# tsnorri/founder-sequences

Hardware: AMD Instinct MI355X
Metric: alignment cells/s (m*n/T) through pBWT+DP (higher is better)
Workload: dtype u32

## Files before the change

### founder-sequences_amd/__init__.py

```python
import ctypes as C
import os

import numpy as np

_HERE = os.path.dirname(os.path.abspath(__file__))
LIB_PATH = os.path.join(_HERE, "libfseq_hip.so")

FSEQ_OK, FSEQ_E_ARG, FSEQ_E_NO_REDUCTION, FSEQ_E_HIP, FSEQ_E_OOM, FSEQ_E_UNSUPPORTED = range(6)


class FseqError(RuntimeError):
    def __init__(self, code, msg):
        super().__init__("fseq error %d: %s" % (code, msg))
        self.code = code


class NoReduction(FseqError):
    """generate_context.cc:192-200: max segment size equals the number of input sequences."""


class Params(C.Structure):
    _fields_ = [("m", C.c_uint32), ("n", C.c_uint64), ("segment_length", C.c_uint64),
                ("pbwt_sample_rate", C.c_uint64), ("block_len", C.c_uint32), ("list_cap", C.c_uint32),
                ("device", C.c_int32)]


class SynthSpec(C.Structure):
    _fields_ = [("seed", C.c_uint64), ("n_founders", C.c_uint32), ("block_len", C.c_uint32),
                ("mut_threshold", C.c_uint64), ("kind", C.c_uint32)]


class Segment(C.Structure):
    _fields_ = [("lb", C.c_uint64), ("rb", C.c_uint64), ("segment_size", C.c_uint32), ("reserved", C.c_uint32)]


class DpArg(C.Structure):
    _fields_ = [("lb", C.c_uint64), ("rb", C.c_uint64), ("segment_max_size", C.c_uint32), ("segment_size", C.c_uint32)]


class Result(C.Structure):
    _fields_ = [("max_segment_size", C.c_uint32), ("short_path", C.c_uint32),
                ("dp_segment_count", C.c_uint64), ("segment_count", C.c_uint64)]


class Timings(C.Structure):
    _fields_ = [("ms_total", C.c_double), ("ms_phase_a", C.c_double), ("ms_phase_b", C.c_double),
                ("ms_phase_c", C.c_double), ("ms_dp", C.c_double), ("ms_pass2", C.c_double), ("ms_host", C.c_double),
                ("ms_colstep_kernels", C.c_double), ("colstep_launches", C.c_uint64), ("colstep_cells", C.c_uint64),
                ("pass2_cells", C.c_uint64), ("list_cap_used", C.c_uint32), ("retries", C.c_uint32),
                ("block_len", C.c_uint32), ("n_blocks", C.c_uint32),
                ("dp_chunks", C.c_uint32), ("dp_sweeps", C.c_uint32), ("phase_a_fallbacks", C.c_uint32), ("phase_a_given_up", C.c_uint32), ("phase_a_trie_given_up", C.c_uint32),
                ("reduced_blocks", C.c_uint32), ("reduced_rows_mean", C.c_uint32), ("reduced_redone", C.c_uint32)]


class JoinProfile(C.Structure):
    _fields_ = [("ms_d2h", C.c_double), ("ms_classes", C.c_double), ("ms_edges", C.c_double), ("ms_draw", C.c_double), ("ms_total", C.c_double),
                ("bytes_d2h", C.c_uint64)]


class MatchPiece(C.Structure):
    _fields_ = [("lb", C.c_uint64), ("rb", C.c_uint64), ("row", C.c_uint32), ("n_founders", C.c_uint32)]


class MatchSummary(C.Structure):
    _fields_ = [("pieces", C.c_uint64), ("uncovered_cells", C.c_uint64), ("short_pieces", C.c_uint64), ("max_pieces_per_row", C.c_uint64),
                ("n_founders", C.c_uint32), ("set_words", C.c_uint32), ("ms_device", C.c_double)]


class IdentitySummary(C.Structure):
    _fields_ = [("n", C.c_uint64), ("identity", C.c_uint64), ("kept", C.c_uint64), ("ms_device", C.c_double)]


MATCH_PIECE_DTYPE = np.dtype([("lb", "<u8"), ("rb", "<u8"), ("row", "<u4"), ("n_founders", "<u4")])
MATCH_MAX_FOUNDERS = 2048

SEGMENT_DTYPE = np.dtype([("lb", "<u8"), ("rb", "<u8"), ("segment_size", "<u4"), ("reserved", "<u4")])
DPARG_DTYPE = np.dtype([("lb", "<u8"), ("rb", "<u8"), ("segment_max_size", "<u4"), ("segment_size", "<u4")])

EXPORTS = [
    "fseq_abi_version", "fseq_strerror", "fseq_create", "fseq_destroy", "fseq_last_error",
    "fseq_set_rows", "fseq_set_matrix", "fseq_set_device_columns", "fseq_generate_synthetic", "fseq_get_matrix",
    "fseq_run_segmentation", "fseq_get_traceback", "fseq_get_segments", "fseq_boundary_state",
    "fseq_short_path_runs", "fseq_join_greedy", "fseq_greedy_match_host", "fseq_write_founders", "fseq_write_founders_device", "fseq_debug_dp", "fseq_debug_block_state", "fseq_debug_column_list", "fseq_get_timings",
    "fseq_rowshard_xbuf_words", "fseq_rowshard_rows", "fseq_rowshard_pbwt",
    "fseq_debug_rmq", "fseq_shard_xbuf_words", "fseq_set_shard", "fseq_shard_columns", "fseq_shard_owner",
    "fseq_set_device_columns_packed", "fseq_debug_dp_schedule", "fseq_run_segmentation_batch", "fseq_join_bipartite", "fseq_join_random", "fseq_bipartite_match_host", "fseq_random_join_host", "fseq_write_segments",
    "fseq_set_progress", "fseq_step_max", "fseq_current_step", "fseq_set_memory_budget", "fseq_write_segments_host", "fseq_get_join_profile", "fseq_debug_set_tuning",
    "fseq_shard_abort", "fseq_debug_dp_owned", "fseq_debug_clock", "fseq_debug_ranges",
    "fseq_set_list_memory", "fseq_debug_list_windows",
    "fseq_match_founders", "fseq_match_founder_rows", "fseq_get_match", "fseq_write_match",
    "fseq_identity_columns", "fseq_create_without_identity_columns", "fseq_get_identity_columns", "fseq_write_identity_columns", "fseq_write_founders_restored", "fseq_match_founders_restored",
    "fseq_input_begin", "fseq_input_chunk_columns", "fseq_input_scan", "fseq_input_columns", "fseq_input_end", "fseq_set_rows_streamed", "fseq_debug_device_bytes", "fseq_debug_packed_columns",
    "fseq_debug_join_path", "fseq_debug_pass2_paths", "fseq_debug_class_columns", "fseq_debug_bipartite_path",
    "fseq_debug_pass2_step", "fseq_debug_chain_launch", "fseq_debug_red_plan", "fseq_debug_column_sources", "fseq_debug_red_cls_direct",
    "fseq_write_segments_device", "fseq_random_join_classes_host", "fseq_debug_segments_file", "fseq_debug_random_path",
]
DEBUG_EXPORTS = ["fseq_debug_dp", "fseq_debug_dp_owned", "fseq_debug_clock", "fseq_debug_ranges", "fseq_debug_block_state", "fseq_debug_column_list", "fseq_debug_rmq", "fseq_debug_dp_schedule", "fseq_debug_set_tuning",
                 "fseq_debug_list_windows", "fseq_debug_device_bytes", "fseq_debug_packed_columns", "fseq_debug_join_path", "fseq_debug_pass2_paths",
                 "fseq_debug_class_columns", "fseq_debug_bipartite_path", "fseq_debug_pass2_step", "fseq_debug_chain_launch", "fseq_debug_red_plan", "fseq_debug_column_sources", "fseq_debug_red_cls_direct",
                 "fseq_debug_segments_file", "fseq_debug_random_path"]

FSEQ_E_PEER = 6
P2_RUN_CAP = 8832
STAGE_TRACEBACK, STAGE_MERGE, STAGE_SAMPLES = 0, 1, 2
PROGRESS_FN = C.CFUNCTYPE(None, C.c_void_p, C.c_int, C.c_uint64, C.c_uint64)

JOIN_GREEDY, JOIN_BIPARTITE, JOIN_RANDOM = 0, 1, 2

ALLREDUCE_FN = C.CFUNCTYPE(C.c_int, C.c_void_p, C.c_uint64, C.c_uint64, C.c_int)

_lib = None


def load_library():
    global _lib
    if _lib is not None:
        return _lib
    if not os.path.exists(LIB_PATH):
        raise ImportError("%s is missing: run `python __graft_entry__.py build` (hipcc --offload-arch=gfx950); "
                          "there is no CPU fallback for the segmentation path" % LIB_PATH)
    L = C.CDLL(LIB_PATH)
    vp, u64, sz = C.c_void_p, C.c_uint64, C.c_size_t
    L.fseq_abi_version.restype = C.c_uint32
    L.fseq_strerror.restype = C.c_char_p
    L.fseq_strerror.argtypes = [C.c_int]
    L.fseq_create.argtypes = [C.POINTER(Params), C.POINTER(vp)]
    L.fseq_destroy.argtypes = [vp]
    L.fseq_destroy.restype = None
    L.fseq_last_error.restype = C.c_char_p
    L.fseq_last_error.argtypes = [vp]
    L.fseq_set_rows.argtypes = [vp, C.POINTER(vp)]
    L.fseq_set_matrix.argtypes = [vp, vp, sz, sz]
    L.fseq_set_device_columns.argtypes = [vp, vp, sz, C.c_uint32]
    L.fseq_set_device_columns_packed.argtypes = [vp, vp, sz, C.c_uint32, C.c_uint32]
    L.fseq_generate_synthetic.argtypes = [vp, C.POINTER(SynthSpec)]
    L.fseq_get_matrix.argtypes = [vp, u64, u64, vp, sz, sz]
    L.fseq_run_segmentation.argtypes = [vp, C.POINTER(Result)]
    L.fseq_get_traceback.argtypes = [vp, vp]
    L.fseq_get_segments.argtypes = [vp, vp]
    L.fseq_boundary_state.argtypes = [vp, u64, vp, vp]
    L.fseq_short_path_runs.argtypes = [vp, vp, vp]
    L.fseq_join_greedy.argtypes = [vp, vp]
    L.fseq_greedy_match_host.argtypes = [C.c_uint32, C.c_uint32, u64, vp, vp, vp, vp, vp]
    L.fseq_write_founders.argtypes = [vp, C.POINTER(vp), vp, C.c_char_p]
    L.fseq_write_founders_device.argtypes = [vp, vp, C.c_char_p]
    L.fseq_run_segmentation_batch.argtypes = [vp, sz, vp, vp]
    L.fseq_debug_dp_schedule.argtypes = [u64, u64, u64, vp, vp, vp, vp]
    L.fseq_join_bipartite.argtypes = [vp, vp]
    L.fseq_join_random.argtypes = [vp, C.c_uint32, vp]
    L.fseq_bipartite_match_host.argtypes = [C.c_uint32, C.c_uint32, u64, vp, vp, vp, vp, vp, vp]
    L.fseq_random_join_host.argtypes = [C.c_uint32, C.c_uint32, u64, vp, vp, vp, vp, C.c_uint32, vp]
    L.fseq_write_segments.argtypes = [vp, C.POINTER(vp), C.c_int, C.c_char_p]
    L.fseq_debug_dp.argtypes = [vp, vp, vp, vp]
    L.fseq_debug_block_state.argtypes = [vp, u64, vp, vp]
    L.fseq_debug_column_list.argtypes = [vp, u64, vp, vp, vp, vp, vp]
    L.fseq_get_timings.argtypes = [vp, C.POINTER(Timings)]
    L.fseq_debug_rmq.argtypes = [C.c_int, vp, C.c_uint32, vp, vp, C.c_uint32, vp, vp]
    L.fseq_shard_xbuf_words.restype = u64
    L.fseq_shard_xbuf_words.argtypes = [vp, C.c_uint32]
    L.fseq_set_shard.argtypes = [vp, C.c_uint32, C.c_uint32, vp, u64, ALLREDUCE_FN, vp]
    L.fseq_shard_columns.argtypes = [vp, C.POINTER(u64), C.POINTER(u64)]
    L.fseq_shard_owner.argtypes = [vp, u64, C.POINTER(C.c_uint32)]
    L.fseq_rowshard_xbuf_words.restype = u64
    L.fseq_rowshard_xbuf_words.argtypes = [C.c_uint32, C.c_uint32, C.c_uint32]
    L.fseq_rowshard_rows.argtypes = [C.c_uint32, C.c_uint32, C.c_uint32, C.c_uint32, C.POINTER(C.c_uint32), C.POINTER(C.c_uint32)]
    L.fseq_rowshard_pbwt.argtypes = [vp, vp, vp, C.POINTER(C.c_uint32), C.POINTER(C.c_uint32), C.POINTER(C.c_double), C.POINTER(u64)]
    L.fseq_write_segments_host.argtypes = [vp, C.POINTER(vp), C.c_int, vp, vp, C.c_char_p]
    L.fseq_get_join_profile.argtypes = [vp, C.POINTER(JoinProfile)]
    L.fseq_debug_set_tuning.argtypes = [vp, C.c_char_p, C.c_char_p]
    L.fseq_set_progress.argtypes = [vp, PROGRESS_FN, vp]
    L.fseq_step_max.restype = u64
    L.fseq_step_max.argtypes = [vp]
    L.fseq_current_step.restype = u64
    L.fseq_current_step.argtypes = [vp]
    L.fseq_set_memory_budget.argtypes = [vp, u64]
    L.fseq_set_list_memory.argtypes = [vp, u64]
    L.fseq_debug_list_windows.argtypes = [vp, C.POINTER(u64), C.POINTER(u64), C.POINTER(C.c_uint32), C.POINTER(C.c_uint32)]
    L.fseq_shard_abort.argtypes = [vp, C.c_int]
    L.fseq_debug_dp_owned.argtypes = [vp, C.POINTER(u64), C.POINTER(u64), C.POINTER(C.c_int), C.POINTER(C.c_int)]
    L.fseq_debug_clock.argtypes = [vp, C.POINTER(C.c_double), C.POINTER(C.c_uint32)]
    L.fseq_debug_ranges.argtypes = [C.POINTER(u64), C.POINTER(u64), C.POINTER(C.c_int)]
    L.fseq_match_founders.argtypes = [vp, vp, u64, C.POINTER(MatchSummary)]
    L.fseq_match_founder_rows.argtypes = [vp, C.POINTER(vp), C.c_uint32, u64, C.POINTER(MatchSummary)]
    L.fseq_get_match.argtypes = [vp, vp, vp]
    L.fseq_write_match.argtypes = [vp, C.c_char_p]
    L.fseq_identity_columns.argtypes = [vp, vp, C.POINTER(IdentitySummary)]
    L.fseq_create_without_identity_columns.argtypes = [vp, C.POINTER(Params), C.POINTER(vp), C.POINTER(IdentitySummary)]
    L.fseq_get_identity_columns.argtypes = [vp, vp, vp]
    L.fseq_write_identity_columns.argtypes = [vp, C.c_char_p]
    L.fseq_write_founders_restored.argtypes = [vp, vp, C.c_char_p]
    L.fseq_match_founders_restored.argtypes = [vp, vp, u64, C.POINTER(MatchSummary)]
    L.fseq_input_begin.argtypes = [vp, vp, C.c_uint32, u64]
    L.fseq_input_chunk_columns.restype = u64
    L.fseq_input_chunk_columns.argtypes = [vp]
    L.fseq_input_scan.argtypes = [vp, u64, u64, C.POINTER(vp)]
    L.fseq_input_columns.argtypes = [vp, u64, u64, C.POINTER(vp)]
    L.fseq_input_end.argtypes = [vp]
    L.fseq_set_rows_streamed.argtypes = [vp, C.POINTER(vp), u64]
    L.fseq_debug_device_bytes.argtypes = [vp, C.POINTER(u64), C.POINTER(u64), C.c_int]
    L.fseq_debug_packed_columns.argtypes = [vp, u64, u64, vp, C.POINTER(u64), C.POINTER(C.c_uint32)]
    L.fseq_debug_join_path.argtypes = [vp, C.POINTER(C.c_int)]
    L.fseq_debug_bipartite_path.argtypes = [vp, C.POINTER(C.c_int)]
    L.fseq_debug_pass2_paths.argtypes = [vp] + [C.POINTER(C.c_uint32)] * 4 + [vp]
    L.fseq_debug_class_columns.argtypes = [vp, C.POINTER(C.c_uint32), C.POINTER(C.c_uint32), C.c_uint32, C.POINTER(C.c_uint32), C.POINTER(C.c_uint32), C.POINTER(u64), vp, u64]
    L.fseq_debug_column_sources.argtypes = [vp, C.POINTER(C.c_uint32), C.POINTER(C.c_uint32), C.c_uint32, C.POINTER(C.c_uint32)]
    L.fseq_debug_red_cls_direct.argtypes = [C.c_uint32, C.c_uint32, C.c_uint32, u64, C.c_uint32, C.c_uint32, C.c_uint32, C.POINTER(u64), C.POINTER(u64), C.POINTER(C.c_int)]
    L.fseq_debug_pass2_step.argtypes = [C.c_int, C.c_uint32, C.c_uint32, vp, vp, vp, C.c_uint32, C.c_uint32, vp, vp, vp, vp, C.c_uint32, C.c_uint32, vp, vp, vp]
    L.fseq_debug_chain_launch.argtypes = [C.c_int, C.c_uint32, C.c_uint32, C.c_uint32, u64, vp, vp, vp, C.c_uint32, C.c_uint32, vp, vp, vp, vp, vp, vp, vp]
    L.fseq_debug_red_plan.argtypes = [C.c_uint32, C.c_uint32, C.c_uint32, C.c_int, C.c_uint32, C.c_uint32, C.c_uint32, vp, vp, C.c_int, C.c_int] + [vp] * 11
    L.fseq_write_segments_device.argtypes = [vp, C.c_int, C.c_char_p]
    L.fseq_random_join_classes_host.argtypes = [C.c_uint32, C.c_uint32, u64, vp, vp, vp, C.c_uint32, vp]
    L.fseq_debug_segments_file.argtypes = [vp] + [C.POINTER(u64)] * 4
    L.fseq_debug_random_path.argtypes = [vp, C.POINTER(C.c_int)]
    _lib = L
    return L


def synth_threshold(mu):
    if mu <= 0.0:
        return 0
    if mu >= 1.0:
        return 0xFFFFFFFFFFFFFFFF
    return int(mu * 18446744073709551616.0)


def greedy_match_host(m, max_segment_size, lb, rb, a, d):
    L = load_library()
    lb = np.ascontiguousarray(lb, dtype=np.uint64)
    rb = np.ascontiguousarray(rb, dtype=np.uint64)
    a = np.ascontiguousarray(a, dtype=np.uint32)
    d = np.ascontiguousarray(d, dtype=np.uint32)
    perm = np.zeros((len(lb), max_segment_size), dtype=np.uint32)
    rc = L.fseq_greedy_match_host(m, max_segment_size, len(lb), lb.ctypes.data, rb.ctypes.data, a.ctypes.data, d.ctypes.data, perm.ctypes.data)
    if rc != FSEQ_OK:
        raise FseqError(rc, L.fseq_strerror(rc).decode())
    return perm


def debug_ranges():
    a, b, w = C.c_uint64(), C.c_uint64(), C.c_int()
    load_library().fseq_debug_ranges(C.byref(a), C.byref(b), C.byref(w))
    return a.value, b.value, bool(w.value)


def debug_rmq(keys, beg, end, device=0):
    L = load_library()
    keys = np.ascontiguousarray(keys, dtype=np.uint32)
    beg = np.ascontiguousarray(beg, dtype=np.uint32)
    end = np.ascontiguousarray(end, dtype=np.uint32)
    a = np.zeros(len(beg), dtype=np.uint32)
    b = np.zeros(len(beg), dtype=np.uint32)
    rc = L.fseq_debug_rmq(device, keys.ctypes.data, len(keys), beg.ctypes.data, end.ctypes.data, len(beg), a.ctypes.data, b.ctypes.data)
    if rc != FSEQ_OK:
        raise FseqError(rc, L.fseq_strerror(rc).decode())
    return a, b


P2_STATS = 23
NOT_WRITTEN = 0xFFFFFFFF


def pass2_step(a0, d0, rank, task_blk, cls, headd, ncls, run_cap=P2_RUN_CAP, workgroups=1, device=0):
    L = load_library()
    a0 = np.ascontiguousarray(np.atleast_2d(a0), dtype=np.uint32)
    d0 = np.ascontiguousarray(np.atleast_2d(d0), dtype=np.uint32)
    rank = np.ascontiguousarray(np.atleast_2d(rank), dtype=np.uint32)
    task_blk = np.ascontiguousarray(task_blk, dtype=np.uint32)
    ncls = np.ascontiguousarray(ncls, dtype=np.uint32)
    cls = np.ascontiguousarray(np.atleast_2d(cls), dtype=np.uint32)
    headd = np.ascontiguousarray(np.atleast_2d(headd), dtype=np.uint32)
    nblocks, m = a0.shape
    ntasks, cap = cls.shape
    if d0.shape != a0.shape or rank.shape != a0.shape or headd.shape != cls.shape or task_blk.shape != (ntasks,) or ncls.shape != (ntasks,):
        raise FseqError(FSEQ_E_ARG, "pass2_step: shapes disagree")
    snap_a = np.zeros((ntasks, m), dtype=np.uint32)
    snap_d = np.zeros((ntasks, m), dtype=np.uint32)
    stats = np.zeros(P2_STATS, dtype=np.uint32)
    rc = L.fseq_debug_pass2_step(device, m, nblocks, a0.ctypes.data, d0.ctypes.data, rank.ctypes.data, cap, ntasks, task_blk.ctypes.data, cls.ctypes.data,
                                 headd.ctypes.data, ncls.ctypes.data, run_cap, workgroups, snap_a.ctypes.data, snap_d.ctypes.data, stats.ctypes.data)
    if rc != FSEQ_OK:
        raise FseqError(rc, L.fseq_strerror(rc).decode())
    return snap_a, snap_d, stats


def chain_launch(rank, keyd, nkeys, G, cols_per_block, first_chain=0, chains=None, start_a=None, start_d=None, states=True, keys=False, device=0):
    L = load_library()
    rank = np.ascontiguousarray(np.atleast_2d(rank), dtype=np.uint32)
    keyd = np.ascontiguousarray(np.atleast_2d(keyd), dtype=np.uint32)
    nkeys = np.ascontiguousarray(nkeys, dtype=np.uint32)
    nb_total, m = rank.shape
    if keyd.shape != rank.shape or nkeys.shape != (nb_total,):
        raise FseqError(FSEQ_E_ARG, "chain_launch: shapes disagree")
    if chains is None:
        chains = max(0, (nb_total + G - 1) // G - first_chain) if G else 0
    if (start_a is None) != (start_d is None):
        raise FseqError(FSEQ_E_ARG, "chain_launch: start_a and start_d go together")
    if start_a is not None:
        start_a = np.ascontiguousarray(np.atleast_2d(start_a), dtype=np.uint32)
        start_d = np.ascontiguousarray(np.atleast_2d(start_d), dtype=np.uint32)
        if start_a.shape != (chains, m) or start_d.shape != (chains, m):
            raise FseqError(FSEQ_E_ARG, "chain_launch: start states are [chains][m]")
    out = {}
    if states:
        out["state_a"] = np.zeros((nb_total + 1, m), dtype=np.uint32)
        out["state_d"] = np.zeros((nb_total + 1, m), dtype=np.uint32)
    if keys:
        out["rank"] = np.zeros((chains, m), dtype=np.uint32)
        out["keyd"] = np.zeros((chains, m), dtype=np.uint32)
        out["nkeys"] = np.zeros(chains, dtype=np.uint32)
    ptr = lambda name: out[name].ctypes.data if name in out else None
    rc = L.fseq_debug_chain_launch(device, m, nb_total, G, cols_per_block, rank.ctypes.data, keyd.ctypes.data, nkeys.ctypes.data, first_chain, chains,
                                   None if start_a is None else start_a.ctypes.data, None if start_a is None else start_d.ctypes.data,
                                   ptr("state_a"), ptr("state_d"), ptr("rank"), ptr("keyd"), ptr("nkeys"))
    if rc != FSEQ_OK:
        raise FseqError(rc, L.fseq_strerror(rc).decode())
    return out


RED_NONE = 0xFFFFFFFF
RED_FORCE_FULL, RED_FORCE_WIDE = 1, 2
RED_USE, RED_DECLINED, RED_NO_BLOCK_LIST = 0, 1, 2
RED_CONFIGS_MAX = 64


def red_cls_direct_host(m, B, bits, cls_ld, config, resident_rows, resident_cls):
    a, b, d = C.c_uint64(), C.c_uint64(), C.c_int()
    rc = load_library().fseq_debug_red_cls_direct(m, B, bits, cls_ld, config, resident_rows, resident_cls, C.byref(a), C.byref(b), C.byref(d))
    if rc != FSEQ_OK:
        raise FseqError(rc, "red_cls_direct_host")
    return a.value, b.value, bool(d.value)


def red_plan_host(m, B, bits, direct, cnt, force=None, b_lo=0, b_hi=None, reduced_always=False, no_block_list=False):
    L = load_library()
    cnt = np.ascontiguousarray(cnt, dtype=np.uint32)
    if cnt.ndim != 1:
        raise FseqError(FSEQ_E_ARG, "red_plan_host: cnt is one count per block")
    nb = len(cnt)
    if force is not None:
        force = np.ascontiguousarray(force, dtype=np.uint8)
        if force.shape != cnt.shape:
            raise FseqError(FSEQ_E_ARG, "red_plan_host: one force mark per block")
    configs = np.zeros((RED_CONFIGS_MAX, 6), dtype=np.uint32)
    full = np.zeros(nb, dtype=np.uint8)
    config_of = np.zeros(nb, dtype=np.int32)
    config_snap_of = np.zeros(nb, dtype=np.int32)
    blocks = np.zeros(3 * nb, dtype=np.uint32)
    bins = np.zeros((RED_CONFIGS_MAX, 3), dtype=np.uint32)
    summary = np.zeros(6, dtype=np.uint32)
    n_configs, n_blocks, n_bins, verdict = C.c_uint32(), C.c_uint32(), C.c_uint32(), C.c_int()
    rc = L.fseq_debug_red_plan(m, B, bits, int(bool(direct)), nb, b_lo, nb if b_hi is None else b_hi, cnt.ctypes.data,
                               None if force is None else force.ctypes.data, int(bool(reduced_always)), int(bool(no_block_list)),
                               configs.ctypes.data, C.addressof(n_configs), C.addressof(verdict), full.ctypes.data, config_of.ctypes.data,
                               config_snap_of.ctypes.data, blocks.ctypes.data, C.addressof(n_blocks), bins.ctypes.data, C.addressof(n_bins),
                               summary.ctypes.data)
    if rc != FSEQ_OK:
        raise FseqError(rc, L.fseq_strerror(rc).decode())
    out = dict(zip(("full_at", "nfull", "listed", "max_rows", "reduced_blocks", "rows_mean"), (int(x) for x in summary)))
    out.update(verdict=verdict.value, full=full, config_of=config_of, config_snap_of=config_snap_of, blocks=blocks[:n_blocks.value],
               bins=[tuple(int(x) for x in row) for row in bins[:n_bins.value]],
               configs=[(int(r), int(v), int(T), int(E), bool(ew), bool(fits)) for r, v, T, E, ew, fits in configs[:n_configs.value]])
    return out


class RowShard(C.Structure):
    _fields_ = [("device", C.c_int32), ("rank", C.c_uint32), ("world", C.c_uint32), ("m", C.c_uint32), ("sigma", C.c_uint32),
                ("bits", C.c_uint32), ("ncols", C.c_uint64), ("d_cols", C.c_void_p), ("ld", C.c_size_t), ("xbuf", C.c_void_p),
                ("xbuf_words", C.c_uint64), ("fn", ALLREDUCE_FN), ("user", C.c_void_p)]


def pack_columns(msa_codes, bits):
    m, n = msa_codes.shape
    per = 8 // bits
    ld = ((m + per - 1) // per + 15) // 16 * 16
    cols = np.zeros((n, ld * per), dtype=np.uint8)
    cols[:, :m] = msa_codes.T
    out = np.zeros((n, ld), dtype=np.uint8)
    for j in range(per):
        out |= (cols[:, j::per] << (bits * j)).astype(np.uint8)
    return out, ld


def rowshard_xbuf_words(m, bits, world):
    return int(load_library().fseq_rowshard_xbuf_words(m, bits, world))


def rowshard_rows(m, bits, rank, world):
    lo, hi = C.c_uint32(), C.c_uint32()
    rc = load_library().fseq_rowshard_rows(m, bits, rank, world, C.byref(lo), C.byref(hi))
    if rc != FSEQ_OK:
        raise FseqError(rc, load_library().fseq_strerror(rc).decode())
    return lo.value, hi.value


def rowshard_pbwt(d_cols_ptr, ld, m, sigma, bits, ncols, rank, world, xbuf_ptr, xbuf_words, allreduce=None, device=0):
    L = load_library()

    def _cb(_user, off, cnt, op):
        try:
            return int(allreduce(int(off), int(cnt), int(op)) or 0)
        except Exception:
            import traceback
            traceback.print_exc()
            return 1
    cb = ALLREDUCE_FN(_cb) if allreduce is not None else ALLREDUCE_FN()
    args = RowShard(device, rank, world, m, sigma, bits, ncols, d_cols_ptr, ld, xbuf_ptr, xbuf_words, cb, None)
    a = np.zeros(m, dtype=np.uint32)
    d = np.zeros(m, dtype=np.uint32)
    lo, hi, ms, nex = C.c_uint32(), C.c_uint32(), C.c_double(), C.c_uint64()
    rc = L.fseq_rowshard_pbwt(C.byref(args), a.ctypes.data, d.ctypes.data, C.byref(lo), C.byref(hi), C.byref(ms), C.byref(nex))
    if rc != FSEQ_OK:
        raise FseqError(rc, L.fseq_strerror(rc).decode())
    return a, d, lo.value, hi.value, ms.value, nex.value


def dp_schedule(segment_length, n, col_hi):
    L = load_library()
    a, b, c_, d = C.c_uint32(), C.c_uint32(), C.c_uint32(), C.c_int()
    rc = L.fseq_debug_dp_schedule(segment_length, n, col_hi, C.byref(a), C.byref(b), C.byref(c_), C.byref(d))
    if rc != FSEQ_OK:
        raise FseqError(rc, L.fseq_strerror(rc).decode())
    return a.value, b.value, c_.value, bool(d.value)


def run_batch(contexts):
    L = load_library()
    n = len(contexts)
    handles = (C.c_void_p * n)(*[c.h for c in contexts])
    results = (Result * n)()
    rcs = (C.c_int * n)()
    rc = L.fseq_run_segmentation_batch(handles, n, results, rcs)
    if rc != FSEQ_OK:
        raise FseqError(rc, L.fseq_strerror(rc).decode())
    for i, c in enumerate(contexts):
        r = Result()
        C.memmove(C.byref(r), C.byref(results[i]), C.sizeof(Result))
        c.result = r
    return list(rcs)


def bipartite_match_host(m, max_segment_size, lb, rb, a, d):
    L = load_library()
    lb = np.ascontiguousarray(lb, dtype=np.uint64)
    rb = np.ascontiguousarray(rb, dtype=np.uint64)
    a = np.ascontiguousarray(a, dtype=np.uint32)
    d = np.ascontiguousarray(d, dtype=np.uint32)
    perm = np.zeros((len(lb), max_segment_size), dtype=np.uint32)
    weights = np.zeros(max(1, len(lb) - 1), dtype=np.int64)
    rc = L.fseq_bipartite_match_host(m, max_segment_size, len(lb), lb.ctypes.data, rb.ctypes.data, a.ctypes.data, d.ctypes.data,
                                     perm.ctypes.data, weights.ctypes.data)
    if rc != FSEQ_OK:
        raise FseqError(rc, L.fseq_strerror(rc).decode())
    return perm, weights[:len(lb) - 1]


def random_join_host(m, max_segment_size, lb, rb, a, d, seed):
    L = load_library()
    lb = np.ascontiguousarray(lb, dtype=np.uint64)
    rb = np.ascontiguousarray(rb, dtype=np.uint64)
    a = np.ascontiguousarray(a, dtype=np.uint32)
    d = np.ascontiguousarray(d, dtype=np.uint32)
    perm = np.zeros((len(lb), max_segment_size), dtype=np.uint32)
    rc = L.fseq_random_join_host(m, max_segment_size, len(lb), lb.ctypes.data, rb.ctypes.data, a.ctypes.data, d.ctypes.data, seed, perm.ctypes.data)
    if rc != FSEQ_OK:
        raise FseqError(rc, L.fseq_strerror(rc).decode())
    return perm
# ... 231 lines not shown
        self._check(self.L.fseq_debug_segments_file(self.h, *[C.byref(x) for x in v]))
        return dict(zip(("batches", "bytes", "longest_line", "lines"), (x.value for x in v)))

    def random_path(self):
        path = C.c_int()
        self._check(self.L.fseq_debug_random_path(self.h, C.byref(path)))
        return path.value

    def write_founders_device(self, permutations, path):
        perm = np.ascontiguousarray(permutations, dtype=np.uint32)
        self._check(self.L.fseq_write_founders_device(self.h, perm.ctypes.data, path.encode() if path else None))

    def write_founders(self, msa, permutations, path):
        assert msa.dtype == np.uint8 and msa.flags["C_CONTIGUOUS"] and msa.shape == (self.m, self.n)
        rows = (C.c_void_p * self.m)(*[msa.ctypes.data + r * msa.strides[0] for r in range(self.m)])
        perm = np.ascontiguousarray(permutations, dtype=np.uint32)
        self._check(self.L.fseq_write_founders(self.h, rows, perm.ctypes.data, path.encode() if path else None))

    def match_founders(self, permutations=None, founders=None, min_segment_length=0):
        if (permutations is None) == (founders is None):
            raise ValueError("match_founders: give either permutations or founders")
        sm = MatchSummary()
        if permutations is not None:
            perm = np.ascontiguousarray(permutations, dtype=np.uint32)
            self._check(self.L.fseq_match_founders(self.h, perm.ctypes.data, int(min_segment_length), C.byref(sm)))
        else:
            if not isinstance(founders, np.ndarray):
                founders = np.array([np.frombuffer(bytes(f), dtype=np.uint8) for f in founders], dtype=np.uint8).reshape(len(founders), -1)
            founders = np.ascontiguousarray(founders, dtype=np.uint8)
            if founders.ndim != 2 or founders.shape[1] != self.n:
                raise ValueError("match_founders: founders must be K rows of n = %d bytes" % self.n)
            K = founders.shape[0]
            rows = (C.c_void_p * max(K, 1))(*[founders.ctypes.data + r * founders.strides[0] for r in range(K)])
            self._check(self.L.fseq_match_founder_rows(self.h, rows, K, int(min_segment_length), C.byref(sm)))
        self._match = sm
        return {k: getattr(sm, k) for k, _ in MatchSummary._fields_}

    def match_pieces(self):
        sm = getattr(self, "_match", None)
        n_pieces, words = (sm.pieces, sm.set_words) if sm is not None else (0, 1)
        pieces = np.zeros(n_pieces, dtype=MATCH_PIECE_DTYPE)
        sets = np.zeros((n_pieces, words), dtype=np.uint32)
        self._check(self.L.fseq_get_match(self.h, pieces.ctypes.data, sets.ctypes.data))
        return pieces, sets

    def write_match(self, path):
        self._check(self.L.fseq_write_match(self.h, path.encode() if path else None))

    def identity_columns(self):
        mask = np.zeros(self.n, dtype=np.uint8)
        sm = IdentitySummary()
        self._check(self.L.fseq_identity_columns(self.h, mask.ctypes.data, C.byref(sm)))
        return mask.astype(bool), {k: getattr(sm, k) for k, _ in IdentitySummary._fields_}

    def without_identity_columns(self, segment_length, block_len=0, list_cap=0, list_memory=0):
        p = Params(0, 0, int(segment_length), 0, int(block_len), int(list_cap), int(self._device))
        h = C.c_void_p()
        sm = IdentitySummary()
        self._check(self.L.fseq_create_without_identity_columns(self.h, C.byref(p), C.byref(h), C.byref(sm)))
        new = SegmentationContext.__new__(SegmentationContext)
        new.L, new.h = self.L, h
        new.m, new.n, new.segment_length, new._device = self.m, int(sm.kept), int(segment_length), self._device
        new.result, new._keep = None, None
        new.source_n = int(sm.n)
        new.identity_summary = {k: getattr(sm, k) for k, _ in IdentitySummary._fields_}
        if list_memory:
            new.set_list_memory(list_memory)
        return new

    def identity_mask(self):
        mask = np.zeros(getattr(self, "source_n", 0), dtype=np.uint8)
        self._check(self.L.fseq_get_identity_columns(self.h, mask.ctypes.data, None))
        return mask.astype(bool)

    def kept_columns(self):
        kept = np.zeros(self.n, dtype=np.uint64)
        self._check(self.L.fseq_get_identity_columns(self.h, None, kept.ctypes.data))
        return kept

    def write_identity_columns(self, path):
        self._check(self.L.fseq_write_identity_columns(self.h, path.encode() if path else None))

    def write_founders_restored(self, permutations, path):
        perm = np.ascontiguousarray(permutations, dtype=np.uint32)
        self._check(self.L.fseq_write_founders_restored(self.h, perm.ctypes.data, path.encode() if path else None))

    def match_founders_restored(self, permutations, min_segment_length=0):
        perm = np.ascontiguousarray(permutations, dtype=np.uint32)
        sm = MatchSummary()
        self._check(self.L.fseq_match_founders_restored(self.h, perm.ctypes.data, int(min_segment_length), C.byref(sm)))
        self._match = sm
        return {k: getattr(sm, k) for k, _ in MatchSummary._fields_}

    def debug_dp(self):
        k = self.n - self.segment_length + 1
        lb = np.zeros(k, dtype=np.uint32)
        mx = np.zeros(k, dtype=np.uint32)
        sz = np.zeros(k, dtype=np.uint32)
        self._check(self.L.fseq_debug_dp(self.h, lb.ctypes.data, mx.ctypes.data, sz.ctypes.data))
        return lb, mx, sz

    def debug_dp_owned(self):
        a, b = C.c_uint64(), C.c_uint64()
        f, w = C.c_int(), C.c_int()
        self._check(self.L.fseq_debug_dp_owned(self.h, C.byref(a), C.byref(b), C.byref(f), C.byref(w)))
        return a.value, b.value, bool(f.value), bool(w.value)

    def debug_clock(self):
        g, n = C.c_double(), C.c_uint32()
        self._check(self.L.fseq_debug_clock(self.h, C.byref(g), C.byref(n)))
        return g.value, n.value

    def debug_block_state(self, b):
        a = np.zeros(self.m, dtype=np.uint32)
        d = np.zeros(self.m, dtype=np.uint32)
        self._check(self.L.fseq_debug_block_state(self.h, b, a.ctypes.data, d.ctypes.data))
        return a, d

    def debug_column_list(self, col):
        cap = self.m + 2
        v = np.zeros(cap, dtype=np.uint32)
        c = np.zeros(cap, dtype=np.uint32)
        ne, c0, comp = C.c_uint32(), C.c_uint32(), C.c_uint32()
        self._check(self.L.fseq_debug_column_list(self.h, col, v.ctypes.data, c.ctypes.data,
                                                  C.byref(ne), C.byref(c0), C.byref(comp)))
        return v[:ne.value].copy(), c[:ne.value].copy(), c0.value, bool(comp.value)

    def set_tuning(self, name, value="1"):
        self._check(self.L.fseq_debug_set_tuning(self.h, name.encode(), None if value is None else str(value).encode()))

    def join_profile(self):
        jp = JoinProfile()
        self._check(self.L.fseq_get_join_profile(self.h, C.byref(jp)))
        return {k: getattr(jp, k) for k, _ in JoinProfile._fields_}

    def join_path(self):
        path = C.c_int()
        self._check(self.L.fseq_debug_join_path(self.h, C.byref(path)))
        return path.value

    def bipartite_path(self):
        path = C.c_int()
        self._check(self.L.fseq_debug_bipartite_path(self.h, C.byref(path)))
        return path.value

    def pass2_paths(self):
        v = [C.c_uint32() for _ in range(4)]
        hist = np.zeros(19, dtype=np.uint32)
        self._check(self.L.fseq_debug_pass2_paths(self.h, *[C.byref(x) for x in v], hist.ctypes.data))
        out = dict(zip(("by_runs", "by_sort", "copies", "max_runs"), (x.value for x in v)))
        out["runs_hist"] = [int(x) for x in hist]
        return out

    def class_column_sources(self):
        a, b = C.c_uint32(), C.c_uint32()
        self._check(self.L.fseq_debug_class_columns(self.h, C.byref(a), C.byref(b), 0xFFFFFFFF, None, None, None, None, 0))
        return {"from_classes": a.value, "from_alignment": b.value}

    def column_sources(self, block=None):
        a, b, s = C.c_uint32(), C.c_uint32(), C.c_uint32()
        self._check(self.L.fseq_debug_column_sources(self.h, C.byref(a), C.byref(b), 0xFFFFFFFF if block is None else block, C.byref(s)))
        out = {"staged": a.value, "gathered": b.value}
        if block is not None:
            out["block_staged"] = bool(s.value)
        return out

    def class_columns(self, block):
        have, nkeys, ldc = C.c_uint32(), C.c_uint32(), C.c_uint64()
        self._check(self.L.fseq_debug_class_columns(self.h, None, None, block, C.byref(have), C.byref(nkeys), C.byref(ldc), None, 0))
        if not have.value:
            return None, ldc.value, nkeys.value
        t = self.timings()
        cols = min(t["block_len"], self.n - block * t["block_len"])
        out = np.zeros((cols, ldc.value), dtype=np.uint8)
        self._check(self.L.fseq_debug_class_columns(self.h, None, None, block, C.byref(have), C.byref(nkeys), C.byref(ldc), out.ctypes.data, out.nbytes))
        return out, ldc.value, nkeys.value

    def timings(self):
        t = Timings()
        self._check(self.L.fseq_get_timings(self.h, C.byref(t)))
        return {k: getattr(t, k) for k, _ in Timings._fields_}
```

### founder-sequences_amd/csrc/fseq_api_debug.hip

```cpp
#include "fseq_path.hpp"
#include "fseq_dp.hpp"
#include "fseq_rowshard.hpp"

using namespace fseq;

extern "C" {

int fseq_debug_set_tuning(fseq_ctx *c, char const *name, char const *value)
{
	if (!c || !name) return FSEQ_E_ARG;
	if (c->sh.on && c->have_input) return fail(c, FSEQ_E_ARG, "sharded run: set tuning knobs before the input is set (identically on every rank)");
	if (!c->tune.set(name, value)) return fail(c, FSEQ_E_ARG, "unknown tuning knob");
	(void) hipSetDevice(c->p.device);
	if (c->stream) (void) hipStreamSynchronize(c->stream);
	free_work(c);
	forget_run_history(c);
	return FSEQ_OK;
}

int fseq_debug_pass2_paths(fseq_ctx *c, uint32_t *by_runs, uint32_t *by_sort, uint32_t *copies, uint32_t *max_runs, uint32_t *runs_hist)
{
	if (!c) return FSEQ_E_ARG;
	if (int const rc = need_result(c)) return rc;
	uint32_t const none[P2_STATS] = {};
	uint32_t const *s = c->p2_stats_have ? c->p2_stats : none;
	if (by_runs) *by_runs = s[0];
	if (by_sort) *by_sort = s[1];
	if (copies) *copies = s[2];
	if (max_runs) *max_runs = s[3];
	if (runs_hist) std::copy(s + 4, s + 4 + P2_HIST, runs_hist);
	return FSEQ_OK;
}

int fseq_debug_class_columns(fseq_ctx *c, uint32_t *from_classes, uint32_t *from_alignment, uint32_t block, uint32_t *have, uint32_t *nkeys, uint64_t *ldc,
                             uint8_t *out, uint64_t out_bytes)
{
	if (!c) return FSEQ_E_ARG;
	if (int const rc = need_result(c)) return rc;
	(void) hipSetDevice(c->p.device);
	uint32_t const b_lo = c->sh.on ? c->sh.b_lo : 0u, b_hi = c->sh.on ? c->sh.b_hi : c->nblocks;
	std::vector<uint32_t> flags;
	if (c->cls_read)
	{
		flags.assign(c->nblocks, 0u);
		if (b_hi > b_lo) HIP_TRY(c, hipMemcpy(flags.data() + b_lo, c->d_cls_have + b_lo, (size_t) (b_hi - b_lo) * 4, hipMemcpyDeviceToHost));
	}
	uint32_t n_cls = 0, n_msa = 0;
	if (c->red_active && !c->red_direct && c->red.plan.cnt.size() == c->nblocks)
		for (uint32_t b = b_lo; b < b_hi; ++b)
			if (c->red.plan.cnt[b] != RED_NONE) ++(c->cls_read && flags[b] ? n_cls : n_msa);
	if (from_classes) *from_classes = n_cls;
	if (from_alignment) *from_alignment = n_msa;
	if (block == UINT32_MAX) return FSEQ_OK;
	if (block < b_lo || block >= b_hi) return fail(c, FSEQ_E_ARG, "fseq_debug_class_columns: not a block of this context");
	uint32_t h = 0;
	if (c->cls_on && c->d_cls && c->d_cls_have) HIP_TRY(c, hipMemcpy(&h, c->d_cls_have + block, 4, hipMemcpyDeviceToHost));
	if (have) *have = h;
	if (nkeys) { *nkeys = 0; if (c->d_nkeys) HIP_TRY(c, hipMemcpy(nkeys, c->d_nkeys + block, 4, hipMemcpyDeviceToHost)); }
	if (ldc) *ldc = c->cls_on ? c->cls_ld : 0;
	if (out && h)
	{
		uint64_t const k0 = (uint64_t) block * c->B, k1 = std::min<uint64_t>(c->p.n, k0 + c->B);
		if (out_bytes < (k1 - k0) * c->cls_ld) return fail(c, FSEQ_E_ARG, "fseq_debug_class_columns: the buffer is smaller than the block's class columns");
		HIP_TRY(c, hipMemcpy(out, c->d_cls + (size_t) k0 * c->cls_ld, (size_t) (k1 - k0) * c->cls_ld, hipMemcpyDeviceToHost));
	}
	return FSEQ_OK;
}

int fseq_debug_column_sources(fseq_ctx *c, uint32_t *staged, uint32_t *gathered, uint32_t block, uint32_t *block_staged)
{
	if (!c) return FSEQ_E_ARG;
	if (int const rc = need_result(c)) return rc;
	(void) hipSetDevice(c->p.device);
	uint32_t const b_lo = c->sh.on ? c->sh.b_lo : 0u, b_hi = c->sh.on ? c->sh.b_hi : c->nblocks;
	uint32_t n_staged = 0, n_gathered = 0, mine = 0;
	RedPlan const &P = c->red.plan;
	if (c->red_active && !c->red_direct && P.cnt.size() == c->nblocks)
	{
		std::vector<uint32_t> have(c->nblocks, 0u);
		if (c->cls_staged && b_hi > b_lo) HIP_TRY(c, hipMemcpy(have.data() + b_lo, c->d_cls_have + b_lo, (size_t) (b_hi - b_lo) * 4, hipMemcpyDeviceToHost));
		for (uint32_t b = b_lo; b < b_hi; ++b)
		{
			if (P.cnt[b] == RED_NONE) continue;
			bool const st = c->cls_staged && P.from_cls[b] && have[b];
			++(st ? n_staged : n_gathered);
			if (b == block) mine = st ? 1u : 0u;
		}
	}
	if (staged) *staged = n_staged;
	if (gathered) *gathered = n_gathered;
	if (block_staged) *block_staged = mine;
	return FSEQ_OK;
}

int fseq_debug_dp(fseq_ctx *c, uint32_t *lb, uint32_t *max_size, uint32_t *size)
{
	if (!c) return FSEQ_E_ARG;
	if (int const rc = need_result(c)) return rc;
	(void) hipSetDevice(c->p.device);
	if (lb) HIP_TRY(c, hipMemcpy(lb, c->dp.LB, c->dp_size * 4, hipMemcpyDeviceToHost));
	if (max_size) HIP_TRY(c, hipMemcpy(max_size, c->dp.M, c->dp_size * 4, hipMemcpyDeviceToHost));
	if (size) HIP_TRY(c, hipMemcpy(size, c->dp.SZ, c->dp_size * 4, hipMemcpyDeviceToHost));
	return FSEQ_OK;
}

int fseq_debug_dp_owned(fseq_ctx *c, uint64_t *first, uint64_t *last, int *final_cell, int *whole_arrays)
{
	if (!c || !c->have_result || c->res.short_path) return FSEQ_E_ARG;
	uint64_t lo = 0, hi = c->dp_size;
	int fin = 1, whole = 1;
	if (c->sh.on)
	{
		Shard const &sh = c->sh;
		bool const have = sh.rank < sh.active && sh.rank < c->own_lo.size();
		lo = have ? c->own_lo[sh.rank] : 0; hi = have ? c->own_hi[sh.rank] : 0;
		fin = have && sh.rank + 1u == sh.active ? 1 : 0;
		whole = c->dp_window_mode ? 0 : 1;
	}
	if (first) *first = lo;
	if (last) *last = hi;
	if (final_cell) *final_cell = fin;
	if (whole_arrays) *whole_arrays = whole;
	return FSEQ_OK;
}

int fseq_debug_ranges(uint64_t *pushes, uint64_t *pops, int *with_roctx)
{
	if (pushes) *pushes = g_range_pushes.load(std::memory_order_relaxed);
	if (pops) *pops = g_range_pops.load(std::memory_order_relaxed);
#ifdef FSEQ_WITH_ROCTX
	if (with_roctx) *with_roctx = 1;
#else
	if (with_roctx) *with_roctx = 0;
#endif
	return FSEQ_OK;
}

int fseq_debug_clock(fseq_ctx *c, double *ghz, uint32_t *workgroups)
{
	if (!c || !ghz) return FSEQ_E_ARG;
#ifdef FSEQ_CLOCK_STAMPS
	(void) hipSetDevice(c->p.device);
	std::vector<unsigned long long> st((size_t) FSEQ_CLOCK_SLOTS * 4);
	HIP_TRY(c, hipMemcpyFromSymbol(st.data(), HIP_SYMBOL(g_clock_stamps), st.size() * 8));
	std::vector<double> f;
	for (uint32_t i = 0; i < FSEQ_CLOCK_SLOTS; ++i)
	{
		unsigned long long const t0 = st[4 * i], r0 = st[4 * i + 1], t1 = st[4 * i + 2], r1 = st[4 * i + 3];
		if (t1 > t0 && r1 > r0) f.push_back((double) (t1 - t0) / (double) (r1 - r0) * 0.1);
	}
	if (f.empty()) return fail(c, FSEQ_E_ARG, "no clock stamps: run a long-path segmentation first");
	std::nth_element(f.begin(), f.begin() + f.size() / 2, f.end());
	*ghz = f[f.size() / 2];
	if (workgroups) *workgroups = (uint32_t) f.size();
	return FSEQ_OK;
#else
	(void) workgroups;
	*ghz = 0.0;
	return fail(c, FSEQ_E_UNSUPPORTED, "built without -DFSEQ_CLOCK_STAMPS (the product kernels execute no stamp)");
#endif
}

int fseq_debug_block_state(fseq_ctx *c, uint64_t block_idx, uint32_t *a_out, uint32_t *d_out)
{
	if (!c || !c->have_result || c->res.short_path || block_idx > c->nblocks) return FSEQ_E_ARG;
	if (c->sh.on && (block_idx < c->sh.b_lo || block_idx > c->sh.b_hi)) return fail(c, FSEQ_E_ARG, "block state held by another rank");
	(void) hipSetDevice(c->p.device);
	size_t const m = c->p.m;
	if (a_out) HIP_TRY(c, hipMemcpy(a_out, c->d_bstate_a + block_idx * m, m * 4, hipMemcpyDeviceToHost));
	if (d_out) HIP_TRY(c, hipMemcpy(d_out, c->d_bstate_d + block_idx * m, m * 4, hipMemcpyDeviceToHost));
	return FSEQ_OK;
}

int fseq_debug_column_list(fseq_ctx *c, uint64_t col, uint32_t *values, uint32_t *counts,
                           uint32_t *n_entries, uint32_t *cnt0, uint32_t *complete)
{
	if (!c || !c->have_result || c->res.short_path || col >= c->p.n) return FSEQ_E_ARG;
	if (c->lw.on && (col < c->lw.col_lo || col >= c->lw.col_hi)) return fail(c, FSEQ_E_ARG, "the list of this column is not held: the run kept its lists in windows (fseq_set_list_memory)");
	(void) hipSetDevice(c->p.device);
	uint4 h;
	HIP_TRY(c, hipMemcpy(&h, c->d_hdr + col, sizeof(h), hipMemcpyDeviceToHost));
	std::vector<uint2> e(h.x);
	if (h.x) HIP_TRY(c, hipMemcpy(e.data(), c->d_ent + col * (size_t) c->stride, h.x * sizeof(uint2), hipMemcpyDeviceToHost));
// ... 150 lines not shown
```

### founder-sequences_amd/csrc/fseq_chainsort.hpp

```cpp
#pragma once

#include <type_traits>

#include "fseq_stream.hpp"
#include "fseq_types.hpp"

namespace fseq {

constexpr uint32_t CS_MAX_DIGIT_BITS = 9;
constexpr uint32_t CS_BINS = 1u << CS_MAX_DIGIT_BITS;
constexpr uint32_t CS_LEVELS = 16;

__host__ __device__ inline size_t chainsort_ws_words(uint32_t m)
{
	size_t const nblk = ((size_t) m + 63) / 64;
	return 8 * (size_t) m + CS_LEVELS * nblk + 64;
}

__device__ __forceinline__ uint64_t cs_match(uint32_t dg, bool in, uint32_t nbits)
{
	uint64_t mask = __ballot(in);
#pragma unroll
	for (uint32_t b = 0; b < CS_MAX_DIGIT_BITS; ++b)
		if (b < nbits)
		{
			uint64_t const bal = __ballot(in && ((dg >> b) & 1u));
			mask &= ((dg >> b) & 1u) ? bal : ~bal;
		}
	return mask;
}

__device__ __forceinline__ uint32_t cs_below(uint64_t mask)
{
	return (uint32_t) __builtin_amdgcn_mbcnt_hi((uint32_t) (mask >> 32), __builtin_amdgcn_mbcnt_lo((uint32_t) mask, 0u));
}

constexpr uint32_t P2_CLS_CAP = 11264;

constexpr uint32_t P2_RUN_CAP = 8832;
constexpr uint32_t P2_CLS_BITS = 14;
static_assert(P2_CLS_CAP <= (1u << P2_CLS_BITS), "a class of a reduced block fits a descriptor");

struct Pass2Lds {
	uint32_t scan[ST / WAVE + 1];
	uint32_t grp;
	union {
		struct {
			uint32_t hist[ST / WAVE][CS_BINS];
			uint32_t total[CS_BINS];
			uint16_t cls[P2_CLS_CAP];
		};
		struct {
			uint32_t off[P2_RUN_CAP + 1];
			uint32_t dsc[P2_RUN_CAP];
		};
	};
};

__host__ __device__ inline size_t pass2_lds_bytes() { return carve_bytes(1, sizeof(Pass2Lds)); }

__host__ __device__ inline size_t pass2_ws_r(uint32_t m) { return (((size_t) m + 1) / 2 + 3) & ~size_t(3); }
__host__ __device__ inline size_t pass2_ws_words(uint32_t m)
{
	size_t const nblk = ((size_t) m + 63) / 64;
	return pass2_ws_r(m) + 2 * (size_t) m + 2 * (size_t) m + 4 * (size_t) m + ((CS_LEVELS * nblk + 64 + 3) & ~size_t(3));
}
struct Pass2Ws {
	uint16_t *r;
	uint32_t *bufB, *bufA;
	uint4 *rec;
	uint32_t *tab;
};
__device__ __forceinline__ Pass2Ws pass2_ws(uint32_t *w, uint32_t m)
{
	Pass2Ws W;
	W.r = reinterpret_cast<uint16_t *>(w);
	W.bufB = w + pass2_ws_r(m);
	W.bufA = W.bufB + 2u * (size_t) m;
	W.rec = reinterpret_cast<uint4 *>(W.bufA + 2u * (size_t) m);
	W.tab = W.bufA + 6u * (size_t) m;
	return W;
}

__device__ __forceinline__ void pass2_digits(uint32_t D, uint32_t &npass, uint32_t &db)
{
	uint32_t bits = 1;
	while (bits < 32u && ((D - 1u) >> bits) != 0u) ++bits;
	npass = (bits + CS_MAX_DIGIT_BITS - 1u) / CS_MAX_DIGIT_BITS;
	db = (bits + npass - 1u) / npass;
}

template <typename PairT, typename Load0, typename KeyOf>
__device__ __forceinline__ void pass2_sort(uint32_t cnt, uint32_t npass, uint32_t db, Load0 load0, KeyOf key_of, PairT none, PairT *bufA, PairT *bufB, Pass2Lds &S)
{
	uint32_t const tid = threadIdx.x, lane = lane_id();
	uint32_t const wave = __builtin_amdgcn_readfirstlane(tid >> 6);
	constexpr uint32_t NW = ST / WAVE;
	uint32_t const nbins = 1u << db;
	uint32_t const per = ((cnt + NW - 1u) / NW + 63u) & ~63u;
	uint32_t const c_lo = min(cnt, wave * per), c_hi = min(cnt, c_lo + per);
	for (uint32_t p = 0; p < npass; ++p)
	{
		uint32_t const shift = p * db;
		bool const first = p == 0;
		PairT const *src = ((npass - p) & 1u) ? bufA : bufB;
		PairT *dst = ((npass - p) & 1u) ? bufB : bufA;
		auto load = [&](uint32_t i) -> PairT { return first ? load0(i) : src[i]; };
		for (uint32_t b = lane; b < nbins; b += 64u) S.hist[wave][b] = 0;
		constexpr uint32_t U = 4;
		for (uint32_t i0 = c_lo; i0 < c_hi; i0 += 64u * U)
		{
			PairT pr[U];
#pragma unroll
			for (uint32_t u = 0; u < U; ++u) { uint32_t const i = i0 + u * 64u + lane; pr[u] = i < c_hi ? load(i) : none; }
#pragma unroll
			for (uint32_t u = 0; u < U; ++u)
				if (i0 + u * 64u + lane < c_hi) atomicAdd(&S.hist[wave][(key_of(pr[u]) >> shift) & (nbins - 1u)], 1u);
		}
		__syncthreads();
		uint32_t tot = 0;
		if (tid < nbins)
			for (uint32_t v = 0; v < NW; ++v) { uint32_t const c = S.hist[v][tid]; S.hist[v][tid] = tot; tot += c; }
		uint32_t all;
		uint32_t const start = block_excl_add<ST>(tid < nbins ? tot : 0u, S.scan, &all);
		if (tid < nbins) S.total[tid] = start;
		__syncthreads();
		for (uint32_t b = lane; b < nbins; b += 64u) S.hist[wave][b] += S.total[b];
		for (uint32_t i0 = c_lo; i0 < c_hi; i0 += 64u * U)
		{
			PairT pr[U];
#pragma unroll
			for (uint32_t u = 0; u < U; ++u) { uint32_t const i = i0 + u * 64u + lane; pr[u] = i < c_hi ? load(i) : none; }
#pragma unroll
			for (uint32_t u = 0; u < U; ++u)
			{
				bool const in = i0 + u * 64u + lane < c_hi;
				uint32_t const dg = (key_of(pr[u]) >> shift) & (nbins - 1u);
				uint64_t const same = cs_match(dg, in, db);
				uint32_t const below = cs_below(same);
				uint32_t const base = S.hist[wave][dg];
				if (in) dst[base + below] = pr[u];
				if (in && below == 0u) S.hist[wave][dg] = base + (uint32_t) __popcll(same);
			}
		}
		__syncthreads();
	}
}

__device__ __forceinline__ void pass2_records(uint32_t m, uint32_t const *__restrict__ a0, uint32_t const *__restrict__ d0, uint4 *rec, uint32_t *tab)
{
	uint32_t const tid = threadIdx.x, lane = lane_id();
	uint32_t const wave = __builtin_amdgcn_readfirstlane(tid >> 6);
	constexpr uint32_t NW = ST / WAVE;
	uint32_t const nblk = (m + 63u) / 64u;
	constexpr uint32_t UB = 4;
	for (uint32_t b0 = wave; b0 < nblk; b0 += NW * UB)
	{
		uint32_t v[UB], a[UB];
#pragma unroll
		for (uint32_t u = 0; u < UB; ++u)
		{
			uint32_t const i = (b0 + u * NW) * 64u + lane;
			v[u] = i < m ? d0[i] : 0u;
			a[u] = i < m ? a0[i] : 0u;
		}
#pragma unroll
		for (uint32_t u = 0; u < UB; ++u)
		{
			uint32_t const blk = b0 + u * NW, i = blk * 64u + lane;
			if (blk >= nblk) break;
			uint32_t const pre = wave_incl_max(v[u]);
			uint32_t const rev = (uint32_t) __builtin_amdgcn_ds_bpermute((int) ((63u - lane) << 2), (int) v[u]);
			uint32_t const sufr = wave_incl_max(rev);
			uint32_t const sufn = (uint32_t) __builtin_amdgcn_ds_bpermute((int) ((62u - min(lane, 62u)) << 2), (int) sufr);
			if (i < m) rec[i] = make_uint4(a[u], v[u], pre, lane == 63u ? 0u : sufn);
			if (lane == 63u) tab[blk] = pre;
		}
	}
	__syncthreads();
	for (uint32_t j = tid; j + 1u < nblk; j += ST) rec[j * 64u + 63u].w = tab[j + 1u];
	for (uint32_t k = 1; k < CS_LEVELS && (1u << k) <= nblk; ++k)
	{
		uint32_t const *lo = tab + (size_t) (k - 1u) * nblk;
		uint32_t *hi = tab + (size_t) k * nblk;
		for (uint32_t j = tid; j + (1u << k) <= nblk; j += ST) hi[j] = max(lo[j], lo[j + (1u << (k - 1u))]);
		__syncthreads();
	}
	__syncthreads();
}

__device__ __forceinline__ uint32_t pass2_range_max(uint32_t lo, uint32_t hi, uint4 const *rec, uint32_t const *tab, uint32_t nblk, uint32_t const *__restrict__ d0)
{
	uint32_t const bl = lo >> 6, bh = hi >> 6;
	uint4 const rc = rec[hi], q = rec[lo - 1u];
	uint32_t const pz = q.z, sv = q.w;
	uint32_t dv = max(sv, rc.z);
	if (bh > bl + 1u)
	{
		uint32_t const k = 31u - (uint32_t) __builtin_clz(bh - bl - 1u);
		uint32_t const *t = tab + (size_t) k * nblk;
		dv = max(dv, max(t[bl + 1u], t[bh - (1u << k)]));
	}
	if (bl == bh)
	{
		if ((lo & 63u) == 0u || rc.z > pz) dv = rc.z;
		else if ((hi & 63u) == 63u || sv > rc.w) dv = sv;
		else
		{
			dv = rc.y;
			for (uint32_t i = lo; i < hi; ++i) dv = max(dv, d0[i]);
		}
	}
	return dv;
}

__device__ __forceinline__ bool pass2_runs(
	uint32_t m, uint32_t const *__restrict__ kd, uint32_t D, Pass2Ws const &W, Pass2Lds &S, uint32_t run_cap, uint32_t *nrun,
	uint32_t const *__restrict__ a0, uint32_t const *__restrict__ d0, uint32_t *__restrict__ a1, uint32_t *__restrict__ d1)
{
	uint32_t const tid = threadIdx.x, lane = lane_id();
	uint32_t const wave = __builtin_amdgcn_readfirstlane(tid >> 6);
	constexpr uint32_t NW = ST / WAVE;
	uint16_t const *__restrict__ r = W.r;
	uint32_t pb = 1;
	while (pb < 32u && ((m - 1u) >> pb) != 0u) ++pb;
	uint32_t const pmask = (1u << pb) - 1u;
	uint32_t const nblk = (m + 63u) / 64u;
	uint32_t const per = ((m + NW - 1u) / NW + 63u) & ~63u;
	uint32_t const c_lo = min(m, wave * per), c_hi = min(m, c_lo + per);
	constexpr uint32_t U = 4;

	uint32_t npass, db;
	pass2_digits(D, npass, db);
	uint2 *const bufA = reinterpret_cast<uint2 *>(W.bufA), *const bufB = reinterpret_cast<uint2 *>(W.bufB);
	uint32_t *const pos_order = reinterpret_cast<uint32_t *>((npass & 1u) ? bufA : bufB);
	uint32_t R = 0, wbase = 0;
	for (uint32_t sweep = 0; sweep < 2u; ++sweep)
	{
		uint32_t prev = 0xFFFFFFFFu;
		if (c_lo > 0u && c_lo < c_hi) prev = (uint32_t) S.cls[r[c_lo - 1u]];
		uint32_t k0 = wbase;
		for (uint32_t i0 = c_lo; i0 < c_hi; i0 += 64u * U)
		{
			uint32_t rv[U];
#pragma unroll
			for (uint32_t u = 0; u < U; ++u) { uint32_t const i = i0 + u * 64u + lane; rv[u] = i < c_hi ? (uint32_t) r[i] : 0u; }
// ... 101 lines not shown
	                  reinterpret_cast<PairT *>(W.bufA), reinterpret_cast<PairT *>(W.bufB), S);
	PairT const *perm = reinterpret_cast<PairT const *>(W.bufB);


	{
		constexpr uint32_t U = 4;
		for (uint32_t p0 = tid; p0 < m; p0 += ST * U)
		{
			uint2 me[U], pv[U];
#pragma unroll
			for (uint32_t u = 0; u < U; ++u)
			{
				uint32_t const p = min(p0 + u * ST, m - 1u);
				PairT const pm_ = perm[p], pp_ = perm[p ? p - 1u : 0u];
				me[u] = make_uint2(key_of(pm_), pos_of(pm_));
				pv[u] = make_uint2(key_of(pp_), pos_of(pp_));
			}
			uint4 rc[U];
			uint32_t z0[U], w0[U], kdv[U], t0[U], t1[U];
#pragma unroll
			for (uint32_t u = 0; u < U; ++u)
			{
				uint32_t const p = p0 + u * ST;
				bool const first = p == 0u || pv[u].x != me[u].x;
				uint32_t const lo = pv[u].y + 1u, hi = me[u].y;
				uint32_t const bl = lo >> 6, bh = hi >> 6;
				rc[u] = rec[hi];
				z0[u] = 0u; w0[u] = 0u; kdv[u] = 0u; t0[u] = 0u; t1[u] = 0u;
				if (lane == 0u && !first) { uint4 const q = rec[pv[u].y]; z0[u] = q.z; w0[u] = q.w; }
				if (p < m && first) kdv[u] = kd[me[u].x];
				if (p < m && !first && bh > bl + 1u)
				{
					uint32_t const k = 31u - (uint32_t) __builtin_clz(bh - bl - 1u);
					uint32_t const *t = tab + (size_t) k * nblk;
					t0[u] = t[bl + 1u];
					t1[u] = t[bh - (1u << k)];
				}
			}
#pragma unroll
			for (uint32_t u = 0; u < U; ++u)
			{
				uint32_t const p = p0 + u * ST;
				uint32_t const bz = (uint32_t) __builtin_amdgcn_ds_bpermute((int) ((lane - 1u) << 2), (int) rc[u].z);
				uint32_t const bw = (uint32_t) __builtin_amdgcn_ds_bpermute((int) ((lane - 1u) << 2), (int) rc[u].w);
				if (p < m)
				{
					bool const first = p == 0u || pv[u].x != me[u].x;
					uint32_t const lo = pv[u].y + 1u, hi = me[u].y;
					uint32_t const bl = lo >> 6, bh = hi >> 6;
					uint32_t const pz = lane ? bz : z0[u], sv = lane ? bw : w0[u];
					uint32_t dv = max(sv, rc[u].z);
					if (bh > bl + 1u) dv = max(dv, max(t0[u], t1[u]));
					if (!first && bl == bh)
					{
						if ((lo & 63u) == 0u || rc[u].z > pz) dv = rc[u].z;
						else if ((hi & 63u) == 63u || sv > rc[u].w) dv = sv;
						else
						{
							dv = rc[u].y;
							for (uint32_t i = lo; i < hi; i += 4u)
							{
								uint32_t const x0 = d0[i], x1 = i + 1u < hi ? d0[i + 1u] : 0u;
								uint32_t const x2 = i + 2u < hi ? d0[i + 2u] : 0u, x3 = i + 3u < hi ? d0[i + 3u] : 0u;
								dv = max(dv, max(max(x0, x1), max(x2, x3)));
							}
						}
					}
					a1[p] = rc[u].x;
					d1[p] = first ? kdv[u] : dv;
				}
			}
		}
	}
	__syncthreads();
}

__global__ __launch_bounds__(ST) void k_chain_snap_grouped(
	uint32_t const *__restrict__ bstate_a, uint32_t const *__restrict__ bstate_d, uint32_t const *__restrict__ rank, uint32_t m,
	uint32_t const *__restrict__ task_blk, uint32_t const *__restrict__ cls, uint32_t const *__restrict__ headd, uint32_t const *__restrict__ ncls,
	uint32_t cap, uint2 const *__restrict__ grps, uint32_t ngrp, uint32_t *__restrict__ grp_next, uint32_t *__restrict__ snap_a,
	uint32_t *__restrict__ snap_d, uint32_t *ws, uint32_t run_cap, uint32_t *__restrict__ stats)
{
	extern __shared__ __attribute__((aligned(16))) char smem[];
	Pass2Lds &S = *reinterpret_cast<Pass2Lds *>(smem);
	uint32_t const tid = threadIdx.x;
	Pass2Ws const W = pass2_ws(ws + (size_t) blockIdx.x * pass2_ws_words(m), m);
	uint16_t *const r = W.r;
	uint32_t pbits = 1;
	while (pbits < 32u && ((m - 1u) >> pbits) != 0u) ++pbits;
	for (;;)
	{
		if (tid == 0) S.grp = atomicAdd(grp_next, 1u);
		__syncthreads();
		uint32_t const g = S.grp;
		__syncthreads();
		if (g >= ngrp) break;
		uint2 const gr = grps[g];
		size_t const sb = (size_t) task_blk[gr.x] * m;
		uint32_t const *a0 = bstate_a + sb, *d0 = bstate_d + sb;
		bool have_r = false;
		for (uint32_t task = gr.x; task < gr.x + gr.y; ++task)
		{
			uint32_t const D = ncls[task];
			if (D == 0xFFFFFFFFu) continue;
			size_t const ob = (size_t) task * m;
			if (D == 0u)
			{
				for (uint32_t i = tid; i < m; i += ST) { snap_a[ob + i] = a0[i]; snap_d[ob + i] = d0[i]; }
				if (tid == 0) atomicAdd(stats + 2, 1u);
				continue;
			}
			if (!have_r)
			{
				constexpr uint32_t U = 4;
				for (uint32_t i0 = tid; i0 < m; i0 += ST * U)
				{
					uint32_t rv[U];
#pragma unroll
					for (uint32_t u = 0; u < U; ++u) { uint32_t const i = i0 + u * ST; rv[u] = i < m ? rank[sb + a0[i]] : 0u; }
#pragma unroll
					for (uint32_t u = 0; u < U; ++u) { uint32_t const i = i0 + u * ST; if (i < m) r[i] = (uint16_t) rv[u]; }
				}
				pass2_records(m, a0, d0, W.rec, W.tab);
				have_r = true;
			}
			for (uint32_t j = tid; j < cap; j += ST) S.cls[j] = (uint16_t) cls[(size_t) task * cap + j];
			__syncthreads();
			uint32_t kb = 1;
			while (kb < 32u && ((D - 1u) >> kb) != 0u) ++kb;
			bool const p4 = kb + pbits <= 32u;
			uint32_t const *kd = headd + (size_t) task * cap;
			uint32_t nrun = 0;
			bool const by_runs = run_cap != 0u && P2_CLS_BITS + pbits <= 32u && pass2_runs(m, kd, D, W, S, run_cap, &nrun, a0, d0, snap_a + ob, snap_d + ob);
			if (!by_runs)
			{
				if (p4) pass2_step<true>(m, kd, D, W, S, d0, snap_a + ob, snap_d + ob);
				else pass2_step<false>(m, kd, D, W, S, d0, snap_a + ob, snap_d + ob);
			}
			if (tid == 0)
			{
				atomicAdd(stats + (by_runs ? 0 : 1), 1u);
				if (nrun)
				{
					atomicMax(stats + 3, nrun);
					atomicAdd(stats + 4 + min(P2_HIST - 1u, nrun > 1u ? 32u - (uint32_t) __builtin_clz(nrun - 1u) : 0u), 1u);
				}
			}
		}
	}
}

constexpr uint32_t CM_PART = 1024;
constexpr uint32_t CM_WG = 256;


struct CmWg { uint32_t x, chain; bool ok; };
__device__ __forceinline__ CmWg cm_wg(ChainMultiArgs const &A)
{
	CmWg w;
	uint32_t const nx = gridDim.x, L = blockIdx.y * nx + blockIdx.x;
	uint32_t const xcd = L & 7u, slot = L >> 3;
	w.chain = (slot / nx) * 8u + xcd;
	w.x = slot % nx;
	w.ok = w.chain < A.nchains;
	return w;
}

__host__ __device__ inline uint32_t chainmulti_parts(uint32_t m) { return (m + CM_PART - 1u) / CM_PART; }
__host__ __device__ inline uint32_t chainmulti_passes(uint32_t m)
{
	uint32_t bits = 1;
	while (bits < 32u && ((m - 1u) >> bits) != 0u) ++bits;
	return (bits + CS_MAX_DIGIT_BITS - 1u) / CS_MAX_DIGIT_BITS;
}

struct ChainMultiGeom {
	uint32_t b, npass, db, nbins;
	uint32_t pb;
	bool p4;
	bool active;
	uint32_t *w;
	uint32_t const *a0, *d0;
	uint32_t *a1, *d1;
	uint2 *pairA, *pairB;
	uint32_t *pm, *sm, *tab;
	uint32_t *hist;
};

__device__ __forceinline__ ChainMultiGeom chainmulti_geom(ChainMultiArgs const &A, uint32_t chain)
{
	ChainMultiGeom g;
	uint32_t const grp = chain + A.grp0;
	uint32_t const b0 = grp * A.G, b1 = min(A.nb_total, b0 + A.G);
	g.b = b0 + A.step;
	g.active = g.b < b1 && (A.out_rank != nullptr || g.b + 1u < b1 || g.b + 1u == A.nb_total);
	uint32_t const nk = g.active ? A.nkeys[g.b] : 1u;
	uint32_t bits = 1;
	while (bits < 32u && ((nk - 1u) >> bits) != 0u) ++bits;
	g.npass = (bits + CS_MAX_DIGIT_BITS - 1u) / CS_MAX_DIGIT_BITS;
	g.db = (bits + g.npass - 1u) / g.npass;
	g.nbins = 1u << g.db;
	uint32_t const cur = A.step & 1u, m = A.m;
	g.pb = 1;
	while (g.pb < 32u && ((m - 1u) >> g.pb) != 0u) ++g.pb;
	g.p4 = bits + g.pb <= 32u;
	g.w = A.ws + (size_t) chain * chainsort_ws_words(m);
	g.a0 = g.w + (size_t) cur * 2u * m; g.d0 = g.a0 + m;
	g.a1 = g.w + (size_t) (cur ^ 1u) * 2u * m; g.d1 = g.a1 + m;
	g.pairA = reinterpret_cast<uint2 *>(g.a1);
	g.pairB = reinterpret_cast<uint2 *>(g.w + 4u * (size_t) m);
	g.pm = g.w + 6u * (size_t) m; g.sm = g.w + 7u * (size_t) m; g.tab = g.w + 8u * (size_t) m;
	g.hist = A.hist + (size_t) chain * chainmulti_parts(m) * CS_BINS;
	return g;
}

__device__ __forceinline__ uint2 cm_pack(uint32_t key, uint32_t pos, uint32_t row) { return make_uint2(key | (row << 20), pos | ((row >> 12) << 20)); }
__device__ __forceinline__ uint32_t cm_key(uint2 p) { return p.x & 0xFFFFFu; }
__device__ __forceinline__ uint32_t cm_pos(uint2 p) { return p.y & 0xFFFFFu; }
__device__ __forceinline__ uint32_t cm_row(uint2 p) { return (p.x >> 20) | ((p.y >> 20) << 12); }

template <bool P4>
struct CmPair {
	using T = std::conditional_t<P4, uint32_t, uint2>;
	static __device__ __forceinline__ T pack(ChainMultiGeom const &g, uint32_t key, uint32_t pos, uint32_t row)
	{
		if constexpr (P4) { (void) row; return (key << g.pb) | pos; } else { (void) g; return cm_pack(key, pos, row); }
	}
	static __device__ __forceinline__ T none() { if constexpr (P4) return 0u; else return make_uint2(0u, 0u); }
	static __device__ __forceinline__ uint32_t key(ChainMultiGeom const &g, T p) { if constexpr (P4) return p >> g.pb; else { (void) g; return cm_key(p); } }
	static __device__ __forceinline__ uint32_t pos(ChainMultiGeom const &g, T p) { if constexpr (P4) return p & ((1u << g.pb) - 1u); else { (void) g; return cm_pos(p); } }
	static __device__ __forceinline__ uint32_t row(ChainMultiGeom const &g, T p) { if constexpr (P4) return g.a0[pos(g, p)]; else { (void) g; return cm_row(p); } }
	static __device__ __forceinline__ T *bufA(ChainMultiGeom const &g) { return reinterpret_cast<T *>(g.pairA); }
	static __device__ __forceinline__ T *bufB(ChainMultiGeom const &g) { return reinterpret_cast<T *>(g.pairB); }
	static __device__ __forceinline__ T *stage(ChainMultiGeom const &g) { return (g.npass & 1u) ? bufA(g) : bufB(g); }
	static __device__ __forceinline__ T load(ChainMultiGeom const &g, uint32_t const *rk, uint32_t pass, uint32_t i)
	{
		if (pass == 0u) { uint32_t const r = g.a0[i]; return pack(g, rk[r], i, r); }
		T const *src = ((g.npass - pass) & 1u) ? bufA(g) : bufB(g);
		return src[i];
	}
};


__global__ __launch_bounds__(CM_WG) void k_cm_init(ChainMultiArgs const A)
{
	CmWg const wg = cm_wg(A);
	if (!wg.ok) return;
	uint32_t const chain = wg.chain, grp = chain + A.grp0, m = A.m;
	uint32_t const b0 = grp * A.G;
	if (b0 >= A.nb_total) return;
	uint32_t const kstart = (uint32_t) ((uint64_t) b0 * A.cols_per_block);
	uint32_t *w = A.ws + (size_t) chain * chainsort_ws_words(m);
	uint32_t const i = wg.x * CM_WG + threadIdx.x;
	if (i >= m) return;
	uint32_t const av = A.start_a ? A.start_a[(size_t) grp * m + i] : i;
	uint32_t const dv = A.start_d ? A.start_d[(size_t) grp * m + i] : kstart;
	w[i] = av; w[(size_t) m + i] = dv;
	if (A.out_state_a) { A.out_state_a[(size_t) b0 * m + i] = av; A.out_state_d[(size_t) b0 * m + i] = dv; }
}

__global__ __launch_bounds__(CM_WG) void k_cm_count(ChainMultiArgs const A)
{
	__shared__ uint32_t hist[CM_WG / WAVE][CS_BINS];
	CmWg const wg = cm_wg(A);
	if (!wg.ok) return;
	ChainMultiGeom const g = chainmulti_geom(A, wg.chain);
	if (!g.active || A.pass >= g.npass) return;
	uint32_t const lane = lane_id(), wave = __builtin_amdgcn_readfirstlane(threadIdx.x >> 6);
	uint32_t const part = wg.x * (CM_WG / WAVE) + wave, m = A.m;
	uint32_t const lo = part * CM_PART;
	if (lo >= m) return;
	uint32_t const hi = min(m, lo + CM_PART);
	uint32_t const *rk = A.rank + (size_t) g.b * m;
	uint32_t const shift = A.pass * g.db;
	for (uint32_t b = lane; b < g.nbins; b += 64u) hist[wave][b] = 0;
	auto sweep = [&](auto p4_) {
		using P = CmPair<decltype(p4_)::value>;
		constexpr uint32_t U = 4;
		for (uint32_t i0 = lo; i0 < hi; i0 += 64u * U)
		{
			typename P::T pr[U];
#pragma unroll
			for (uint32_t u = 0; u < U; ++u) { uint32_t const i = i0 + u * 64u + lane; pr[u] = i < hi ? P::load(g, rk, A.pass, i) : P::none(); }
			if (A.pass == 0u)
			{
				typename P::T *const stage = P::stage(g);
#pragma unroll
				for (uint32_t u = 0; u < U; ++u) { uint32_t const i = i0 + u * 64u + lane; if (i < hi) stage[i] = pr[u]; }
			}
#pragma unroll
			for (uint32_t u = 0; u < U; ++u)
				if (i0 + u * 64u + lane < hi) atomicAdd(&hist[wave][(P::key(g, pr[u]) >> shift) & (g.nbins - 1u)], 1u);
		}
	};
	if (g.p4) sweep(std::true_type{}); else sweep(std::false_type{});
	if (A.pass == 0u)
	{
		uint32_t const nblk = (m + 63u) / 64u;
		for (uint32_t i0 = lo; i0 < hi; i0 += 64u)
		{
			uint32_t const i = i0 + lane;
			uint32_t const v = i < m ? g.d0[i] : 0u;
			uint32_t const pre = wave_incl_max(v);
			uint32_t const rev = (uint32_t) __builtin_amdgcn_ds_bpermute((int) ((63u - lane) << 2), (int) v);
			uint32_t const sufr = wave_incl_max(rev);
			uint32_t const suf = (uint32_t) __builtin_amdgcn_ds_bpermute((int) ((63u - lane) << 2), (int) sufr);
			if (i < m) { g.pm[i] = pre; g.sm[i] = suf; }
			if (lane == 63u && (i0 >> 6) < nblk) g.tab[i0 >> 6] = pre;
		}
	}
	uint32_t *out = g.hist + (size_t) part * CS_BINS;
	for (uint32_t b = lane; b < g.nbins; b += 64u) out[b] = hist[wave][b];
}

__global__ __launch_bounds__(ST) void k_cm_offsets(ChainMultiArgs const A)
{
	__shared__ uint32_t scan[ST / WAVE + 1];
	__shared__ uint32_t start_of[CS_BINS];
	ChainMultiGeom const g = chainmulti_geom(A, blockIdx.x);
	if (!g.active || A.pass >= g.npass) return;
	uint32_t const tid = threadIdx.x, m = A.m;
	uint32_t const nparts = chainmulti_parts(m);
	constexpr uint32_t PB = 16;
	uint32_t tot = 0;
	if (tid < g.nbins)
		for (uint32_t p0 = 0; p0 < nparts; p0 += PB)
		{
			uint32_t c[PB];
#pragma unroll
			for (uint32_t q = 0; q < PB; ++q) c[q] = p0 + q < nparts ? g.hist[(size_t) (p0 + q) * CS_BINS + tid] : 0u;
#pragma unroll
			for (uint32_t q = 0; q < PB; ++q) tot += c[q];
		}
	uint32_t all;
	uint32_t const start = block_excl_add<ST>(tid < g.nbins ? tot : 0u, scan, &all);
	(void) start_of;
	if (tid < g.nbins)
	{
		uint32_t run = start;
		for (uint32_t p0 = 0; p0 < nparts; p0 += PB)
		{
			uint32_t c[PB];
#pragma unroll
			for (uint32_t q = 0; q < PB; ++q) c[q] = p0 + q < nparts ? g.hist[(size_t) (p0 + q) * CS_BINS + tid] : 0u;
#pragma unroll
			for (uint32_t q = 0; q < PB; ++q)
			{
				if (p0 + q < nparts) g.hist[(size_t) (p0 + q) * CS_BINS + tid] = run;
				run += c[q];
			}
		}
	}
	if (A.pass == 0u)
	{
		uint32_t const nblk = (m + 63u) / 64u;
		for (uint32_t k = 1; k < CS_LEVELS && (1u << k) <= nblk; ++k)
		{
			__syncthreads();
			uint32_t const *lo = g.tab + (size_t) (k - 1u) * nblk;
			uint32_t *hi = g.tab + (size_t) k * nblk;
			for (uint32_t j = tid; j + (1u << k) <= nblk; j += ST) hi[j] = max(lo[j], lo[j + (1u << (k - 1u))]);
		}
	}
}

__global__ __launch_bounds__(CM_WG) void k_cm_scatter(ChainMultiArgs const A)
{
	__shared__ uint32_t offs[CM_WG / WAVE][CS_BINS];
	CmWg const wg = cm_wg(A);
	if (!wg.ok) return;
	ChainMultiGeom const g = chainmulti_geom(A, wg.chain);
	if (!g.active || A.pass >= g.npass) return;
	uint32_t const lane = lane_id(), wave = __builtin_amdgcn_readfirstlane(threadIdx.x >> 6);
	uint32_t const part = wg.x * (CM_WG / WAVE) + wave, m = A.m;
	uint32_t const lo = part * CM_PART;
	if (lo >= m) return;
	uint32_t const hi = min(m, lo + CM_PART);
	uint32_t const *rk = A.rank + (size_t) g.b * m;
	uint32_t const shift = A.pass * g.db;
	uint32_t const *in_offs = g.hist + (size_t) part * CS_BINS;
	for (uint32_t b = lane; b < g.nbins; b += 64u) offs[wave][b] = in_offs[b];
	auto sweep = [&](auto p4_) {
		using P = CmPair<decltype(p4_)::value>;
		typename P::T *dst = ((g.npass - A.pass) & 1u) ? P::bufB(g) : P::bufA(g);
		constexpr uint32_t U = 4;
		for (uint32_t i0 = lo; i0 < hi; i0 += 64u * U)
		{
			typename P::T pr[U];
#pragma unroll
			for (uint32_t u = 0; u < U; ++u)
			{
				uint32_t const i = i0 + u * 64u + lane;
				pr[u] = i < hi ? (A.pass == 0u ? P::stage(g)[i] : P::load(g, rk, A.pass, i)) : P::none();
			}
#pragma unroll
			for (uint32_t u = 0; u < U; ++u)
			{
				bool const in = i0 + u * 64u + lane < hi;
				uint32_t const dg = (P::key(g, pr[u]) >> shift) & (g.nbins - 1u);
				uint64_t const same = cs_match(dg, in, g.db);
				uint32_t const below = cs_below(same);
				uint32_t const base = offs[wave][dg];
				if (in) dst[base + below] = pr[u];
				if (in && below == 0u) offs[wave][dg] = base + (uint32_t) __popcll(same);
			}
		}
	};
	if (g.p4) sweep(std::true_type{}); else sweep(std::false_type{});
}

__global__ __launch_bounds__(CM_WG) void k_cm_output(ChainMultiArgs const A)
{
	CmWg const wg = cm_wg(A);
	if (!wg.ok) return;
	ChainMultiGeom const g = chainmulti_geom(A, wg.chain);
	if (!g.active) return;
	uint32_t const m = A.m, p = wg.x * CM_WG + threadIdx.x;
	if (p >= m) return;
	uint32_t const nblk = (m + 63u) / 64u;
	uint32_t const *kd = A.keyd + (size_t) g.b * m;
	uint32_t key_me, key_pv, pos_me, pos_pv, row;
	if (g.p4)
	{
		using P = CmPair<true>;
		P::T const me = P::bufB(g)[p], pv = P::bufB(g)[p ? p - 1u : 0u];
		key_me = P::key(g, me); key_pv = P::key(g, pv); pos_me = P::pos(g, me); pos_pv = P::pos(g, pv); row = P::row(g, me);
	}
	else
	{
		using P = CmPair<false>;
		P::T const me = P::bufB(g)[p], pv = P::bufB(g)[p ? p - 1u : 0u];
		key_me = P::key(g, me); key_pv = P::key(g, pv); pos_me = P::pos(g, me); pos_pv = P::pos(g, pv); row = P::row(g, me);
	}
	bool const first = p == 0u || key_pv != key_me;
	uint32_t dv;
	if (first) dv = kd[key_me];
	else
	{
		uint32_t const lo = pos_pv + 1u, hi = pos_me;
		uint32_t const bl = lo >> 6, bh = hi >> 6;
		if (bl == bh)
		{
			dv = g.d0[hi];
			for (uint32_t i = lo; i < hi; ++i) dv = max(dv, g.d0[i]);
		}
		else
		{
			dv = max(g.sm[lo], g.pm[hi]);
			if (bh > bl + 1u)
			{
				uint32_t const k = 31u - (uint32_t) __builtin_clz(bh - bl - 1u);
				uint32_t const *t = g.tab + (size_t) k * nblk;
				dv = max(dv, max(t[bl + 1u], t[bh - (1u << k)]));
			}
		}
	}
	g.a1[p] = row; g.d1[p] = dv;
	uint32_t const grp = wg.chain + A.grp0;
	uint32_t const b1 = min(A.nb_total, grp * A.G + A.G);
	if (A.out_state_a && (g.b + 1u < b1 || g.b + 1u == A.nb_total))
	{
		A.out_state_a[(size_t) (g.b + 1u) * m + p] = row; A.out_state_d[(size_t) (g.b + 1u) * m + p] = dv;
	}
}

__global__ __launch_bounds__(ST) void k_cm_emit(ChainMultiArgs const A, uint32_t steps_done)
{
	extern __shared__ __attribute__((aligned(16))) char smem[];
	Carver cv{smem};
	StreamLds &L = *cv.take<StreamLds>(1);
	uint32_t const chain = blockIdx.x, grp = chain + A.grp0, m = A.m;
	uint32_t const b0 = grp * A.G;
	if (b0 >= A.nb_total) return;
	uint32_t const b1 = min(A.nb_total, b0 + A.G);
	uint32_t const cur = (b1 - b0) & 1u;
	(void) steps_done;
	uint32_t const *w = A.ws + (size_t) chain * chainsort_ws_words(m);
	uint32_t const *a = w + (size_t) cur * 2u * m, *d = a + m;
	uint32_t const kstart = (uint32_t) ((uint64_t) b0 * A.cols_per_block);
	stream_emit_ranks(m, a, d, kstart, A.out_rank + (size_t) grp * m, A.out_keyd + (size_t) grp * m, A.out_nkeys + grp, L);
}

}
```

### founder-sequences_amd/csrc/fseq_ctx.hpp

```cpp
#pragma once

#include "../../include/fseq.h"
#include "../../include/fseq_debug.h"
#include "fseq_types.hpp"

#include <hip/hip_runtime.h>

#include <algorithm>
#include <array>
#include <atomic>
#include <chrono>
#include <climits>
#include <cmath>
#include <cstdio>
#include <cstring>
#include <string>
#include <thread>
#include <unordered_map>
#include <vector>

namespace fseq {

struct KernelSet {
	uint32_t T, E, sigma, cap;
	size_t lds_colblock, lds_snap;
	uint32_t scan_shift;
	void (*rank)(hipStream_t st, uint32_t grid, size_t lds, PhaseAArgs const &keys);
	void (*snap)(hipStream_t st, uint32_t grid, size_t lds, SnapArgs const &tasks);
	size_t (*columns_lds)(uint32_t B);
	void (*columns)(hipStream_t st, uint32_t grid, size_t lds, ColumnsArgs const &cols);
	uint32_t (*columns_resident)(size_t lds);
	size_t lds_chain;
	void (*chain)(hipStream_t st, uint32_t grid, size_t lds, ChainMultiArgs const &chains, uint32_t keyed);
	hipError_t (*prepare)();
	hipError_t (*prepare_columns)(size_t lds_columns);
};

template <typename K>
inline hipError_t allow_lds(K kernel, size_t bytes)
{
	if (bytes <= 64 * 1024) return hipSuccess;
	return hipFuncSetAttribute(reinterpret_cast<void const *>(kernel), hipFuncAttributeMaxDynamicSharedMemorySize, (int) bytes);
}

struct Stream2Config { uint32_t T, E, key_shift; size_t (*lds)(uint32_t colbytes); hipError_t (*prepare)(size_t lds);
	void (*launch)(hipStream_t st, uint32_t grid, size_t lds, ColumnsArgs const &cols);
	uint32_t (*resident)(size_t lds);
	void (*launch_snap)(hipStream_t st, uint32_t grid, size_t lds, SnapArgs const &tasks); };
struct ReducedSet {
	uint32_t T, E, rows, values;
	bool pk, ew;
	size_t (*lds)(uint32_t B, uint32_t symcap);
	hipError_t (*prepare)(size_t lds);
	void (*launch)(hipStream_t st, uint32_t grid, size_t lds, ColumnsArgs const &cols, RedArgs const &red);
	uint32_t (*resident)(size_t lds);
};
int reduced_config_count();
bool reduced_config(int index, ReducedSet *out);
struct ChainSnapSet {
	size_t lds;
	hipError_t (*prepare)();
	void (*launch)(hipStream_t st, uint32_t grid, size_t lds, SnapArgs const &tasks, RedArgs const &red);
};
bool select_chain_snap(uint32_t T, uint32_t E, ChainSnapSet *out);

bool select_kernels(uint32_t m, uint32_t sigma, KernelSet *out);
Stream2Config stream2_config();
void launch_blockkeys(hipStream_t st, uint32_t grid, size_t lds, PhaseAArgs const &keys);
hipError_t prepare_blockkeys(uint32_t T, size_t lds, bool debug);
uint32_t blocktrie_threads(uint32_t m, bool stream);
size_t blocktrie_lds(uint32_t T);
hipError_t launch_blocktrie(hipStream_t st, uint32_t groups, PhaseAArgs const &keys);
hipError_t launch_reduce_prep(hipStream_t, uint32_t grid, RedPrepArgs const &);
void launch_reduce_check(hipStream_t, uint32_t const *cnt, uint32_t const *planned, uint32_t count, uint32_t *flags);
void launch_reduce_msa(hipStream_t st, MsaArgs const &A, ReducedMsaArgs const &red, bool gather_only);
bool launch_reduce_cls(hipStream_t st, MsaArgs const &A, ReducedMsaArgs const &red, ClassColumnArgs const &classes);

inline double now_ms()
{
	using namespace std::chrono;
	return duration<double, std::milli>(steady_clock::now().time_since_epoch()).count();
}


}

struct Tuning {
	bool debug = false;
	bool dp_serial = false;
	int  dp_spec_win = 0, dp_spec_rounds = 0, dp_spec_max_sweeps = 0;
	bool stream_plain_scan = false;
	bool plain_scan = false;
	bool occurrence_keys = false;
	bool phase_a_classic = false;
	int  chain_fan = 0;
	bool blockkeys_wide = false;
	bool blockkeys_single = false;
	bool no_dense_columns = false;
	bool no_blocktrie = false;
	bool blocktrie_always = false;
	int  blockkeys_cap = 0;
	bool ss_unpacked = false;
	bool ss_absolute = false;
	bool poison_lists = false;
	bool join_host = false;
	bool join_wide = false;
	bool join_bip_wide = false;
	int  join_bip_slabs = 0;
	int  segfile_batch = 0;
	bool shard_dp_full = false;
	int  shard_dp_window = 0;
	int  inject_failure_rank = -1;
	std::string sync_phases;
	bool check_phase_a = false;
	bool no_reduced = false;
	int  reduced_margin = -1;
	bool reduced_always = false;
	bool reduced_msa_gather = false;
	int  reduced_cap = 0;
	bool class_gather = false;
	int  class_columns = 1;
	int  p2_run_cap = -1;

	struct Knob {
		char const *name;
		bool Tuning::*flag;
		int Tuning::*num;
		int lo, off;
		std::string Tuning::*str;
	};
	static std::vector<Knob> const &knobs()
	{
		static std::vector<Knob> const table = {
			{"FSEQ_DEBUG", &Tuning::debug, nullptr, 0, 0, nullptr},
			{"FSEQ_DP_SERIAL", &Tuning::dp_serial, nullptr, 0, 0, nullptr},
			{"FSEQ_DP_SPEC_WIN", nullptr, &Tuning::dp_spec_win, 1, 0, nullptr},
			{"FSEQ_DP_SPEC_ROUNDS", nullptr, &Tuning::dp_spec_rounds, 1, 0, nullptr},
			{"FSEQ_DP_SPEC_MAX_SWEEPS", nullptr, &Tuning::dp_spec_max_sweeps, 1, 0, nullptr},
			{"FSEQ_STREAM_PLAIN_SCAN", &Tuning::stream_plain_scan, nullptr, 0, 0, nullptr},
			{"FSEQ_PLAIN_SCAN", &Tuning::plain_scan, nullptr, 0, 0, nullptr},
			{"FSEQ_OCCURRENCE_KEYS", &Tuning::occurrence_keys, nullptr, 0, 0, nullptr},
			{"FSEQ_PHASE_A_CLASSIC", &Tuning::phase_a_classic, nullptr, 0, 0, nullptr},
			{"FSEQ_CHAIN_FAN", nullptr, &Tuning::chain_fan, 2, 0, nullptr},
			{"FSEQ_BLOCKKEYS_WIDE", &Tuning::blockkeys_wide, nullptr, 0, 0, nullptr},
			{"FSEQ_BLOCKKEYS_SINGLE", &Tuning::blockkeys_single, nullptr, 0, 0, nullptr},
			{"FSEQ_NO_DENSE_COLUMNS", &Tuning::no_dense_columns, nullptr, 0, 0, nullptr},
			{"FSEQ_NO_BLOCKTRIE", &Tuning::no_blocktrie, nullptr, 0, 0, nullptr},
			{"FSEQ_BLOCKTRIE_ALWAYS", &Tuning::blocktrie_always, nullptr, 0, 0, nullptr},
			{"FSEQ_BLOCKKEYS_CAP", nullptr, &Tuning::blockkeys_cap, 2048, 0, nullptr},
			{"FSEQ_SS_UNPACKED", &Tuning::ss_unpacked, nullptr, 0, 0, nullptr},
			{"FSEQ_SS_ABSOLUTE", &Tuning::ss_absolute, nullptr, 0, 0, nullptr},
			{"FSEQ_POISON_LISTS", &Tuning::poison_lists, nullptr, 0, 0, nullptr},
			{"FSEQ_JOIN_HOST", &Tuning::join_host, nullptr, 0, 0, nullptr},
			{"FSEQ_JOIN_WIDE", &Tuning::join_wide, nullptr, 0, 0, nullptr},
			{"FSEQ_JOIN_BIP_WIDE", &Tuning::join_bip_wide, nullptr, 0, 0, nullptr},
			{"FSEQ_JOIN_BIP_SLABS", nullptr, &Tuning::join_bip_slabs, 1, 0, nullptr},
			{"FSEQ_SEGFILE_BATCH", nullptr, &Tuning::segfile_batch, 1, 0, nullptr},
			{"FSEQ_SHARD_DP_FULL", &Tuning::shard_dp_full, nullptr, 0, 0, nullptr},
			{"FSEQ_SHARD_DP_WINDOW", nullptr, &Tuning::shard_dp_window, 64, 0, nullptr},
			{"FSEQ_INJECT_FAILURE_RANK", nullptr, &Tuning::inject_failure_rank, INT_MIN, -1, nullptr},
			{"FSEQ_SYNC_PHASES", nullptr, nullptr, 0, 0, &Tuning::sync_phases},
			{"FSEQ_CHECK_PHASE_A", &Tuning::check_phase_a, nullptr, 0, 0, nullptr},
			{"FSEQ_NO_REDUCED", &Tuning::no_reduced, nullptr, 0, 0, nullptr},
			{"FSEQ_REDUCED_MARGIN", nullptr, &Tuning::reduced_margin, 0, -1, nullptr},
			{"FSEQ_REDUCED_ALWAYS", &Tuning::reduced_always, nullptr, 0, 0, nullptr},
			{"FSEQ_REDUCED_MSA_GATHER", &Tuning::reduced_msa_gather, nullptr, 0, 0, nullptr},
			{"FSEQ_REDUCED_CAP", nullptr, &Tuning::reduced_cap, 1, 0, nullptr},
			{"FSEQ_P2_RUN_CAP", nullptr, &Tuning::p2_run_cap, 0, -1, nullptr},
			{"FSEQ_CLASS_COLUMNS", nullptr, &Tuning::class_columns, 0, 1, nullptr},
			{"FSEQ_CLASS_GATHER", &Tuning::class_gather, nullptr, 0, 0, nullptr},
		};
		return table;
	}

	void apply(Knob const &k, char const *value)
	{
		bool const on = value != nullptr;
		if (k.flag) this->*k.flag = on;
		else if (k.num) this->*k.num = on ? std::max(k.lo, atoi(value)) : k.off;
		else this->*k.str = on ? value : "";
	}

	bool set(char const *name, char const *value)
	{
		for (Knob const &k : knobs())
			if (!strcmp(k.name, name)) { apply(k, value); return true; }
		return false;
	}

	void from_environment()
	{
		for (Knob const &k : knobs())
			if (char const *v = getenv(k.name)) apply(k, v);
	}
};

struct fseq_ctx;

namespace fseq {

template <typename T>
struct DevBuf {
	T *base = nullptr;
	size_t cap = 0;
	ptrdiff_t shift = 0;
	operator T *() const { return base ? reinterpret_cast<T *>(reinterpret_cast<char *>(base) - shift) : nullptr; }
	template <typename U> U *as() const { return reinterpret_cast<U *>(static_cast<T *>(*this)); }
	void rebase(ptrdiff_t elements) { shift = elements * (ptrdiff_t) sizeof(T); }
	int alloc(fseq_ctx *c, size_t count);
	bool try_alloc(fseq_ctx *c, size_t count);
	int ensure(fseq_ctx *c, size_t count) { return cap >= count ? FSEQ_OK : alloc(c, count); }
	int alloc_range(fseq_ctx *c, size_t lo, size_t hi, size_t per)
	{
		int const rc = alloc(c, (hi > lo ? hi - lo : 0) * per);
		rebase((ptrdiff_t) (lo * per));
		return rc;
	}
	void release(fseq_ctx *c);
};

template <typename T>
struct DevTemp : DevBuf<T> {
	fseq_ctx *const c;
	explicit DevTemp(fseq_ctx *c_) : c(c_) {}
	DevTemp(DevTemp const &) = delete;
	~DevTemp() { this->release(c); }
	int alloc(size_t count) { return DevBuf<T>::alloc(c, count); }
};

template <typename... B>
inline void release_all(fseq_ctx *c, B &...bufs) { (bufs.release(c), ...); }

}

struct Shard {
	bool on = false;
	uint32_t rank = 0, world = 1;
	uint32_t *xbuf = nullptr;
	uint64_t xwords = 0;
	fseq_allreduce_fn fn = nullptr;
	void *user = nullptr;
	uint32_t bpr = 0;
	uint32_t active = 1;
	uint32_t b_lo = 0, b_hi = 0;
	uint64_t c_lo = 0, c_hi = 0, c_end = 0;
	bool posted = false;
	bool closed = false;
};

struct fseq_ctx {
	fseq_params p{};
	Tuning tune;
	template <typename T> using DevBuf = fseq::DevBuf<T>;
	std::unordered_map<void *, size_t> alloc_sizes;
	size_t alloc_total = 0;
	size_t alloc_peak = 0;
	uint64_t mem_budget = 0;
	struct ListWindows {
		uint64_t budget = 0;
		bool on = false;
		uint32_t wb = 0, H = 0, nwin = 0;
		uint32_t merge_windows = 0;
		uint64_t bytes = 0;
		uint64_t col_lo = 0, col_hi = 0;
		std::vector<hipEvent_t> ev;
	} lw;
	std::atomic<uint64_t> step_max{0}, current_step{0};
	fseq_join_profile jp{};
	int join_path = -1;
	int bip_path = -1;
	int rand_path = -1;
	struct SegFileStats { bool have = false; uint64_t batches = 0, bytes = 0, longest_line = 0, lines = 0; } segfile;
	fseq_progress_fn progress_fn = nullptr;
	void *progress_user = nullptr;
	hipStream_t stream = nullptr;
	std::string err;
	Shard sh;
	DevBuf<uint8_t> d_msa_own;
	DevBuf<uint32_t> d_bkws;
	DevBuf<uint16_t> d_bk;
	size_t bk_per_block = 0;
	uint32_t bk_cap_words = 0;
	uint32_t bk_T = 0;
	DevBuf<uint32_t> d_todo;
	int bk_given_up = -1;
	size_t bk_lds = 0;
	DevBuf<uint32_t> d_colmask;
	bool colmask_ready = false, colmask_use = false;
	DevBuf<uint32_t> d_btws;
	DevBuf<uint32_t> d_only;
	int bt_given_up = -1;
	DevBuf<uint32_t> d_chunk_r0;
	DevBuf<uint2> d_tau;
	std::vector<int64_t> snap_slot;
	std::vector<uint32_t> own_lo, own_hi;
	bool dp_window_mode = false;
	bool shard_dp_full_sticky = false;
	uint64_t dp_exchange_words = 0;

	uint8_t *d_msa = nullptr;
	size_t ld = 0;
	bool have_input = false;
	uint32_t sigma = 0;
	uint8_t code_to_byte[256]{};

	uint32_t B = 0, nblocks = 0, N2 = 0, npass = 1;
	uint32_t auto_B = 0;
	fseq::Stream2Config s2{};
	size_t s2_lds = 0;
	bool stream_staged = false;
	uint32_t bsh = 0;
	fseq::KernelSet ks{};
	bool kernels_ready = false;
	bool use_stream = false;
	size_t tb_guess = 0;
	std::vector<uint2> tau_host;
	DevBuf<uint32_t> d_ws;
	size_t lds_columns = 0;

	DevBuf<uint32_t> d_rank, d_keyd, d_nkeys;
	DevBuf<uint32_t> d_bstate_a, d_bstate_d;
	DevBuf<uint32_t> d_cshist;
	DevBuf<uint32_t> d_hrank, d_hkeyd, d_hnkeys, d_hstate_a, d_hstate_d;
	struct ChainLevel { uint32_t count = 0; uint64_t cols = 0; DevBuf<uint32_t> rank, keyd, nkeys, state_a, state_d; };
	std::vector<ChainLevel> levels;
	uint32_t chain_fan = 0;
	uint32_t shard_k = 0, shard_q = 0;
	uint32_t chain_G = 0, n_super = 0;
	uint32_t chain_G2 = 0, n_hyper = 0;
	DevBuf<uint2> d_ent;
	DevBuf<uint4> d_hdr;
	uint32_t X = 0, stride = 0;
	uint32_t X_hint = 0;
	struct Dp {
		DevBuf<uint32_t> M, LB, SZ, Tb, Tbv;
		DevBuf<unsigned long long> K;
		uint32_t tstride = 0;
		operator fseq::DpArrays() const { return fseq::DpArrays{M, LB, SZ, Tb, Tbv, K, tstride}; }
	} dp;
	DevBuf<uint32_t> d_Mprev;
	DevBuf<uint32_t> d_spec;
	DevBuf<fseq::PathWords> d_flags;
	DevBuf<uint32_t> d_recent;
	uint64_t dp_size = 0;
	DevBuf<uint64_t> d_cols;
	DevBuf<uint2> d_grp;
	DevBuf<uint64_t> d_src;
	uint32_t snap_stride = 16;
	DevBuf<uint32_t> d_ss_a, d_ss_d;
	uint32_t ss_pack = 0;
	bool ss_ids = false;
	DevBuf<uint32_t> d_bs_w;
	DevBuf<uint8_t> d_bs_h;
	DevBuf<uint32_t> d_wgblk;
	DevBuf<uint2> d_wggrp;
	DevBuf<uint32_t> d_snap_a, d_snap_d;

	DevBuf<uint32_t> d_red_cnt, d_red_vmin, d_red_rows, d_red_leaf, d_red_a, d_red_d;
	DevBuf<uint32_t> d_red_invalid, d_red_blocks;
	uint32_t red_cap = 0;
	DevBuf<uint8_t> d_red_msa;
	size_t red_ld = 0;
	DevBuf<uint8_t> d_cls;
	DevBuf<uint32_t> d_cls_have;
	size_t cls_ld = 0;
	bool cls_on = false;
	bool cls_every = false;
	bool cls_read = false;
	DevBuf<uint32_t> d_red_src;
	bool cls_staged = false;
	struct Red {
		fseq::RedPlan plan;
		std::vector<uint8_t> cls_config;
		struct Memory {
			std::vector<uint8_t> force;
			bool plan_holds = false;
			uint32_t plan_X = 0;
			bool declined = false;
			uint32_t declined_X = 0;
			bool cls_unread = false;
			void forget_plan() { plan_holds = false; }
			void forget_verdicts() { plan_holds = false; declined = false; cls_unread = false; }
			void forget_input() { forget_verdicts(); force.clear(); }
		} memory;
	} red;
	bool red_active = false;
	DevBuf<uint32_t> d_red_cls, d_red_headd, d_red_ncls, d_red_taskblk, d_red_wgtasks;
	DevBuf<uint32_t> d_red_p2grp;
	uint32_t p2_stats[fseq::P2_STATS]{};
	bool p2_stats_have = false;
	DevBuf<uint32_t> d_red_ss_a, d_red_ss_d;
	uint32_t red_ss_stride = 0, red_ss_cap = 0;
	uint32_t *h_red_pin = nullptr;
	size_t red_pin_words = 0;
	bool red_direct = false;
	DevBuf<uint32_t> d_red_cnt_plan;
	hipStream_t red_st[2]{};
	struct RedEvents {
		hipEvent_t fork = nullptr;
		hipEvent_t join_stream2 = nullptr, join_side0 = nullptr, join_side1 = nullptr;
		std::array<hipEvent_t *, 3> joins() { return {&join_stream2, &join_side0, &join_side1}; }
		std::array<hipEvent_t *, 4> all() { return {&fork, &join_stream2, &join_side0, &join_side1}; }
	} red_ev;
	uint8_t *h_red_pin2 = nullptr;
	size_t red_pin2_bytes = 0;

	bool have_result = false;
	fseq_result res{};
	DevBuf<uint4> d_tb;
	std::vector<fseq_dp_arg> traceback;
	std::vector<fseq_segment> segments;
	std::vector<uint32_t> sp_first, sp_len;
	fseq_timings tm{};
	struct PathEvents {
		hipEvent_t a_begin = nullptr, a_end_b_begin = nullptr, b_end = nullptr;
		hipEvent_t c_begin = nullptr, c_end = nullptr, dp_begin = nullptr, dp_end = nullptr;
		hipEvent_t pass2_begin = nullptr, pass2_end = nullptr;
		hipEvent_t dp_reset = nullptr;
		std::array<hipEvent_t *, 9> timed() { return {&a_begin, &a_end_b_begin, &b_end, &c_begin, &c_end, &dp_begin, &dp_end, &pass2_begin, &pass2_end}; }
	} ev;
	hipStream_t stream2 = nullptr;
	uint8_t *h_pin = nullptr;
	size_t pin_cap = 0, pin_used = 0;

	struct Match {
		DevBuf<uint8_t> fcols;
		DevBuf<uint32_t> cnt;
		DevBuf<uint64_t> off;
		DevBuf<fseq_match_piece> pieces;
		DevBuf<uint32_t> sets;
		bool have = false;
		fseq_match_summary sum{};
		hipEvent_t ev[4]{};
	} match;
	void free_match()
	{
		fseq::release_all(this, match.fcols, match.cnt, match.off, match.pieces, match.sets);
		for (auto &e : match.ev) if (e) { (void) hipEventDestroy(e); e = nullptr; }
		match.have = false;
	}

	struct Identity {
		bool have = false;
		uint64_t n_src = 0, identity = 0;
		DevBuf<uint8_t> mask;
		DevBuf<uint32_t> kept;
		DevBuf<uint8_t> ref;
	} idn;
	void free_identity()
	{
		fseq::release_all(this, idn.mask, idn.kept, idn.ref);
		idn.have = false;
	}

	struct Input {
		bool open = false;
		bool given = false;
		bool table_ready = false;
		uint64_t half_bytes = 0, chunk_cols = 0;
		uint64_t scanned = 0, encoded = 0;
		uint64_t calls = 0;
		uint32_t present[8]{};
		DevBuf<uint8_t> stage;
		DevBuf<uint32_t> words;
		DevBuf<uint8_t> table;
		hipEvent_t copied[2]{}, used[2]{};
	} in;
	void free_input()
	{
		fseq::release_all(this, in.stage, in.words, in.table);
		for (auto &e : in.copied) if (e) { (void) hipEventDestroy(e); e = nullptr; }
		for (auto &e : in.used) if (e) { (void) hipEventDestroy(e); e = nullptr; }
		in.open = false;
	}
};
// ... 96 lines not shown
```

### founder-sequences_amd/csrc/fseq_path_pass1.hip

```cpp
#include "fseq_path.hpp"
#include "fseq_kernels.hpp"
#include "fseq_stream.hpp"
#include "fseq_stream2.hpp"
#include "fseq_chainsort.hpp"
#include "fseq_blockkeys.hpp"
#include "fseq_blocktrie.hpp"

namespace fseq {

std::atomic<uint64_t> g_range_pushes{0}, g_range_pops{0};

uint32_t scan_keyed(fseq_ctx const *c)
{
	if (c->use_stream || c->tune.plain_scan) return 0u;
	return (c->p.n < (1ull << c->ks.scan_shift) && !c->tune.occurrence_keys) ? 1u : c->p.n < (1ull << 25) ? 2u : 0u;
}

namespace {

bool stream_keyed(fseq_ctx const *c) { return c->p.n < (1ull << 25) && !c->tune.plain_scan; }

template <int MODE>
void launch_colblock_stream(fseq_ctx *c, uint32_t grid, MsaArgs const &A, PhaseAArgs const &K, SnapArgs const &S)
{
	hipLaunchKernelGGL((stream_keyed(c) ? k_colblock_stream<MODE, true> : k_colblock_stream<MODE, false>), dim3(grid), dim3(ST), stream_lds_bytes(sym_bytes(A.m, A.bsh), c->stream_staged), c->stream,
	                   A.msa, A.ld, A.m, A.n, A.B, A.nblocks, A.npass, A.bsh, c->d_ws.base, (uint32_t) c->stream_staged, K.rank, K.keyd, K.nkeys, MODE == MODE_RANK ? K.only : S.bstate_a, S.bstate_d,
	                   S.task_rb, S.task_grp, S.snap_a, S.snap_d, S.task_src, S.ss.snap_stride, (uint32_t const *) S.ss.ss_a, (uint32_t const *) S.ss.ss_d, K.col0, S.ss.ss_pack);
}

void launch_rank(fseq_ctx *c, PhaseAArgs const &K)
{
	if (!K.nblk) return;
	if (c->use_stream) launch_colblock_stream<MODE_RANK>(c, K.nblk, K.A, K, SnapArgs{});
	else c->ks.rank(c->stream, K.nblk, c->ks.lds_colblock, K);
}

void launch_blockkeys_stream(fseq_ctx *c, uint32_t groups, PhaseAArgs const &K)
{
	MsaArgs const &A = K.A;
	hipLaunchKernelGGL(k_blockkeys_stream, dim3(groups), dim3(1024), c->bk_lds, c->stream, A.msa, A.ld, A.m, A.n, A.B, A.bsh, K.nblk, K.rank, K.keyd, K.nkeys, K.col0,
	                   static_cast<uint32_t *>(K.work), K.work_per, K.cap_words, K.counters, K.wide, K.todo, K.only);
}

}

void launch_replay_stream(fseq_ctx *c, size_t groups, SnapArgs const &tasks)
{
	size_t const cap = std::max<size_t>(1, c->d_ws.cap / (4 * (size_t) c->p.m));
	SnapArgs S = tasks;
	for (size_t g0 = 0; g0 < groups; g0 += cap)
	{
		S.task_grp = tasks.task_grp + g0; S.task_src = tasks.task_src + g0;
		launch_colblock_stream<MODE_SNAP>(c, (uint32_t) std::min(cap, groups - g0), S.A, PhaseAArgs{}, S);
	}
}

namespace {

void launch_chain_stream(hipStream_t st, uint32_t grid, ChainMultiArgs A)
{
	uint32_t const m = A.m, nparts = chainmulti_parts(m), npass = chainmulti_passes(m);
	A.step = 0; A.pass = 0;
	A.nchains = grid;
	uint32_t const grid_y = (grid + 7u) & ~7u;
	dim3 const by_row((m + CM_WG - 1u) / CM_WG, grid_y), by_part((nparts + CM_WG / WAVE - 1u) / (CM_WG / WAVE), grid_y);
	hipLaunchKernelGGL(k_cm_init, by_row, dim3(CM_WG), 0, st, A);
	for (uint32_t s_ = 0; s_ < A.G; ++s_)
	{
		A.step = s_;
		for (uint32_t ps = 0; ps < npass; ++ps)
		{
			A.pass = ps;
			hipLaunchKernelGGL(k_cm_count, by_part, dim3(CM_WG), 0, st, A);
			hipLaunchKernelGGL(k_cm_offsets, dim3(grid), dim3(ST), 0, st, A);
			hipLaunchKernelGGL(k_cm_scatter, by_part, dim3(CM_WG), 0, st, A);
		}
		hipLaunchKernelGGL(k_cm_output, by_row, dim3(CM_WG), 0, st, A);
	}
	if (A.out_rank) hipLaunchKernelGGL(k_cm_emit, dim3(grid), dim3(ST), stream_lds_bytes(0, false), st, A, A.G);
}

void launch_chain(fseq_ctx *c, uint32_t grid, ChainMultiArgs A)
{
	if (!grid) return;
	A.m = c->p.m;
	if (c->use_stream)
	{
		A.ws = c->d_ws.base; A.hist = c->d_cshist;
		launch_chain_stream(c->stream, grid, A);
	}
	else
		c->ks.chain(c->stream, grid, c->ks.lds_chain, A, scan_keyed(c));
}

}

int prepare_stream_kernels(fseq_ctx *c, size_t lds)
{
	HIP_TRY(c, allow_lds(k_colblock_stream<MODE_RANK>, lds));
	HIP_TRY(c, allow_lds(k_colblock_stream<MODE_SNAP>, lds));
	HIP_TRY(c, allow_lds(k_colblock_stream<MODE_RANK, true>, lds));
	HIP_TRY(c, allow_lds(k_colblock_stream<MODE_SNAP, true>, lds));
	HIP_TRY(c, allow_lds(k_columns_stream<19>, lds));
	HIP_TRY(c, allow_lds(k_columns_stream<0>, lds));
	HIP_TRY(c, allow_lds(k_chain_snap_grouped, pass2_lds_bytes()));
	HIP_TRY(c, allow_lds(k_cm_emit, stream_lds_bytes(0, false)));
	return FSEQ_OK;
}
int prepare_stream2_prologue(fseq_ctx *c)
{
	HIP_TRY(c, allow_lds(k_columns_stream2_prologue, stream_lds_bytes(0, true)));
	return FSEQ_OK;
}
int prepare_blockkeys_stream(fseq_ctx *c)
{
	HIP_TRY(c, allow_lds(k_blockkeys_stream, c->bk_lds));
	return FSEQ_OK;
}
size_t chain_hist_words(uint32_t m) { return (size_t) chainmulti_parts(m) * CS_BINS; }

uint32_t pass2_run_cap(fseq_ctx const *c)
{
	return c->tune.p2_run_cap < 0 ? P2_RUN_CAP : std::min<uint32_t>((uint32_t) c->tune.p2_run_cap, P2_RUN_CAP);
}

int launch_chain_snap_grouped(fseq_ctx *c, uint32_t ngrp, uint32_t *stats)
{
	uint32_t const m = c->p.m;
	hipStream_t st = c->stream;
	if (c->red_cap > P2_CLS_CAP) return fail(c, FSEQ_E_UNSUPPORTED, "pass 2: more representatives a block than the class table in LDS holds");
	int ncu = 0;
	(void) hipDeviceGetAttribute(&ncu, hipDeviceAttributeMultiprocessorCount, c->p.device);
	size_t const fit = c->d_ws.cap / pass2_ws_words(m);
	uint32_t const grid = (uint32_t) std::min<size_t>(std::min<size_t>(ngrp, fit), (size_t) std::max(ncu, 1) * 2u);
	if (!grid) return fail(c, FSEQ_E_OOM, "pass 2: the workspace holds no chain step");
	if (c->tune.debug)
	{
		int resident = 0;
		(void) hipOccupancyMaxActiveBlocksPerMultiprocessor(&resident, k_chain_snap_grouped, (int) ST, pass2_lds_bytes());
		fprintf(stderr, "[fseq] pass 2 chain steps: %u groups on %u workgroups (the workspace holds %zu, a CU %d), %zu bytes of LDS, at most %u runs\n", ngrp, grid, fit,
		        resident, pass2_lds_bytes(), pass2_run_cap(c));
	}
	hipLaunchKernelGGL(k_chain_snap_grouped, dim3(grid), dim3(ST), pass2_lds_bytes(), st, c->d_bstate_a, c->d_bstate_d, c->d_rank, m, c->d_red_taskblk, c->d_red_cls,
	                   c->d_red_headd, c->d_red_ncls, c->red_cap, c->d_red_p2grp.as<uint2 const>(), ngrp, c->d_red_p2grp + 2 * (size_t) ngrp,
	                   c->d_snap_a, c->d_snap_d, c->d_ws.base, pass2_run_cap(c), stats);
	return FSEQ_OK;
}

int long_phase_a(fseq_ctx *c, LongRun &R)
{
	FSEQ_LONG_LOCALS(c);
	if (c->bsh == 1u && c->npass == 2u && !c->use_stream && !c->tune.no_dense_columns && !c->colmask_ready && held_hi(c) > held_lo(c)
	    && c->d_msa_own && (c->ld & 3u) == 0)
	{
		uint64_t const lo = held_lo(c), hi = held_hi(c);
		if ((rc = c->d_colmask.alloc_range(c, (size_t) lo, (size_t) hi, 1))) return rc;
		HIP_TRY(c, hipMemsetAsync(&path_words(c)->dense_columns, 0, 4, st));
		hipLaunchKernelGGL(k_column_presence, dim3((uint32_t) std::min<uint64_t>(hi - lo, 8192)), dim3(256), 0, st, c->d_msa, c->ld, sym_bytes(m, c->bsh), lo, hi, c->d_colmask,
		                   &path_words(c)->dense_columns);
		uint32_t n_dense = 0;
		HIP_TRY(c, hipMemcpyAsync(&n_dense, &path_words(c)->dense_columns, 4, hipMemcpyDeviceToHost, st));
		HIP_TRY(c, hipStreamSynchronize(st));
		c->colmask_use = (uint64_t) n_dense * 20u >= hi - lo;
		c->colmask_ready = true;
	}
	HIP_TRY(c, hipEventRecord(c->ev.a_begin, st));
	progress(c, FSEQ_STAGE_TRACEBACK, 0, n);
	FSEQ_RANGE_PUSH("fseq pass 1: phases A + B (block keys, boundary states)");
	R.range_ab_open = true;
	bool const keyspace = R.keyspace = c->bk_cap_words && my_blocks && !c->tune.phase_a_classic;
	bool const limited = keyspace && !c->tune.blockkeys_cap;
	bool const tree = keyspace && !(limited && c->bk_given_up >= 0 && 2u * (uint32_t) c->bk_given_up > my_blocks);
	bool const sweep_after = limited && !(tree && c->bk_given_up == 0);
	R.tree_alone = tree && limited && !sweep_after;
	R.tree_ran = tree;
	uint32_t *todo = nullptr;
	if (limited)
	{
		if ((rc = c->d_todo.ensure(c, my_blocks))) return rc;
		todo = c->d_todo;
		HIP_TRY(c, hipMemsetAsync(todo, tree ? 0 : 0x01, (size_t) my_blocks * 4, st));
	}
	if (keyspace) HIP_TRY(c, hipMemsetAsync(&path_words(c)->phase_a, 0, sizeof(PhaseACounters), st));
	uint32_t const bt_bits = 8u >> c->bsh, bt_T = blocktrie_threads(m, c->use_stream);
	bool const trie = tree && limited && (uint64_t) m <= (uint64_t) (32u / bt_bits) * bt_T * 32u && c->B < 65536u && !c->tune.no_blocktrie
	                  && (c->use_stream || m > 12u * 512u || c->tune.blocktrie_always)
	                  && (c->ld & 3u) == 0 && (reinterpret_cast<uintptr_t>(c->d_msa) & 3u) == 0
	                  && !(c->bt_given_up >= 0 && 2u * (uint32_t) c->bt_given_up > my_blocks);
	bool const tree_after = tree && !(trie && c->bt_given_up == 0);
	c->cls_on = c->cls_every = c->cls_read = c->cls_staged = false;
	R.trie_ran = trie;
	R.trie_alone = trie && !tree_after;
	PhaseAArgs keys;
	keys.A = msa_args(c);
	keys.rank = c->d_rank + (size_t) b_lo * m; keys.keyd = c->d_keyd + (size_t) b_lo * m; keys.nkeys = c->d_nkeys + b_lo;
	keys.col0 = (uint64_t) b_lo * c->B; keys.nblk = my_blocks;
	keys.T = c->bk_T; keys.cap_words = c->bk_cap_words; keys.counters = &path_words(c)->phase_a.tree_sliced; keys.todo = todo;
	keys.wide = (c->tune.blockkeys_wide ? 1u : 0u) | (c->tune.blockkeys_single ? 2u : 0u);
	if (trie)
	{
		int ncu = 0;
		(void) hipDeviceGetAttribute(&ncu, hipDeviceAttributeMultiprocessorCount, c->p.device);
		uint32_t const per_cu = (uint32_t) std::max<size_t>(1, std::min<size_t>(2048u / bt_T, (160u * 1024u) / blocktrie_lds(bt_T)));
		uint32_t const groups = std::min<uint32_t>(my_blocks, (uint32_t) std::max(1, ncu) * per_cu);
		size_t const per = (blocktrie_ws_words(m, c->B, bt_bits, bt_T) + 15) & ~size_t(15);
		if ((rc = c->d_btws.ensure(c, per * groups))) return rc;
		if ((rc = c->d_only.ensure(c, my_blocks))) return rc;
		HIP_TRY(c, hipMemsetAsync(c->d_only, 0, (size_t) my_blocks * 4, st));
		PhaseAArgs T = keys;
		T.T = bt_T; T.work = c->d_btws; T.work_per = per; T.counters = &path_words(c)->phase_a.trie_given_up; T.todo = c->d_only;
		if (c->use_stream && c->tune.class_columns && !c->tune.no_reduced && n >= 2 * L && !(c->red.memory.declined && !c->tune.reduced_always) && !c->red.memory.cls_unread)
		{
			size_t const ldc = ((size_t) sym_bytes((uint32_t) BT_PER * bt_T, c->bsh) + 15) & ~size_t(15);
			uint64_t const k_lo = (uint64_t) b_lo * c->B, k_hi = std::min<uint64_t>(n, (uint64_t) b_hi * c->B);
			size_t const need = (size_t) (k_hi - k_lo) * ldc + 64;
			bool ok = c->d_cls.cap >= need;
			if (!ok)
			{
				size_t const held = c->d_cls.base ? c->d_cls.cap : 0;
				size_t free_b = 0, total_b = 0;
				bool fits = hipMemGetInfo(&free_b, &total_b) == hipSuccess && need <= (free_b + held) / 4;
				if (c->mem_budget && c->alloc_total - std::min(c->alloc_total, held) + need > c->mem_budget) fits = false;
				if (fits) ok = c->d_cls.try_alloc(c, need);
				else if (c->d_cls.base) c->d_cls.release(c);
				if (c->tune.debug && !ok) fprintf(stderr, "[fseq] phase A: no room for %zu bytes of class columns: the reduced alignment from the alignment\n", need);
			}
			if (ok && (rc = c->d_cls_have.ensure(c, c->nblocks))) return rc;
			if (ok)
			{
				c->cls_ld = ldc;
				c->d_cls.rebase((ptrdiff_t) ((size_t) k_lo * ldc));
				HIP_TRY(c, hipMemsetAsync(c->d_cls_have + b_lo, 0, (size_t) my_blocks * 4, st));
				T.cls = c->d_cls; T.ldc = ldc; T.cls_have = c->d_cls_have + b_lo;
				c->cls_on = true; c->cls_every = !tree_after;
			}
		}
		HIP_TRY(c, launch_blocktrie(st, groups, T));
		keys.only = c->d_only;
	}
	if (tree_after && c->use_stream)
	{
		int ncu = 0;
		(void) hipDeviceGetAttribute(&ncu, hipDeviceAttributeMultiprocessorCount, c->p.device);
		uint32_t const groups = std::min<uint32_t>(my_blocks, (uint32_t) std::max(1, ncu));
		size_t const per = (blockkeys_stream_ws_words(m, c->B, c->bsh) + 15) & ~size_t(15);
		if ((rc = c->d_bkws.ensure(c, per * groups))) return rc;
		keys.work = c->d_bkws; keys.work_per = per;
		launch_blockkeys_stream(c, groups, keys);
	}
	else if (tree_after)
	{
		size_t const per = (blockkeys_scratch_halfwords(m, c->B, c->bsh) + 7) & ~size_t(7);
		if (c->bk_per_block != per) c->d_bk.release(c);
		if ((rc = c->d_bk.ensure(c, per * my_blocks))) return rc;
		c->bk_per_block = per;
		keys.work = c->d_bk; keys.work_per = per;
		launch_blockkeys(st, my_blocks, c->bk_lds, keys);
	}
	if (!keyspace || sweep_after)
	{
		keys.only = keyspace && tree ? todo : nullptr;
		launch_rank(c, keys);
	}
	HIP_TRY(c, hipEventRecord(c->ev.a_end_b_begin, st));
	if (sharded && c->tune.inject_failure_rank >= 0 && (uint32_t) c->tune.inject_failure_rank == sh.rank)
		return fail(c, FSEQ_E_OOM, "injected failure (FSEQ_INJECT_FAILURE_RANK)");
	if (sync_at(c, 'A')) { fprintf(stderr, "[fseq] phase A queued\n"); HIP_TRY(c, hipStreamSynchronize(st)); fprintf(stderr, "[fseq] phase A done\n"); }
	if (c->tune.check_phase_a)
	{
		HIP_TRY(c, hipStreamSynchronize(st));
		std::vector<uint32_t> rk(m), kd(m);
		for (uint32_t b = b_lo; b < b_hi; ++b)
		{
			uint32_t nk = 0;
			HIP_TRY(c, hipMemcpy(&nk, c->d_nkeys + b, 4, hipMemcpyDeviceToHost));
			HIP_TRY(c, hipMemcpy(rk.data(), c->d_rank + (size_t) b * m, (size_t) m * 4, hipMemcpyDeviceToHost));
			HIP_TRY(c, hipMemcpy(kd.data(), c->d_keyd + (size_t) b * m, (size_t) m * 4, hipMemcpyDeviceToHost));
			uint64_t const k0 = (uint64_t) b * c->B, k1 = std::min<uint64_t>(n, k0 + c->B);
			uint32_t bad_r = 0, bad_k = 0;
			for (uint32_t i = 0; i < m; ++i) if (rk[i] >= nk) ++bad_r;
			for (uint32_t j = 0; j < nk && j < m; ++j) if (kd[j] <= k0 || kd[j] > k1) ++bad_k;
			if (nk == 0 || nk > m || bad_r || bad_k)
			{
				char what[200];
				snprintf(what, sizeof(what), "phase A check: block %u has %u keys (m = %u), %u ranks out of range, %u key divergences outside (%llu, %llu]",
				         b, nk, m, bad_r, bad_k, (unsigned long long) k0, (unsigned long long) k1);
				return fail(c, FSEQ_E_HIP, what);
			}
		}
	}
	return FSEQ_OK;
}

int phase_a_take_counts(fseq_ctx *c, LongRun const &R, PhaseACounters counts)
{
	FSEQ_LONG_LOCALS(c);
	if (!R.keyspace) return FSEQ_OK;
	if (!R.tree_ran) counts.tree_given_up = my_blocks;
	c->tm.phase_a_fallbacks = counts.tree_sliced;
	c->tm.phase_a_given_up = counts.tree_given_up;
	if (R.tree_alone && counts.tree_given_up != 0u) return fail(c, FSEQ_E_HIP, "internal: the key-space tree gave up blocks it ranked in the run before");
	c->bk_given_up = (int) counts.tree_given_up;
	if (R.trie_ran)
	{
		if (R.trie_alone && counts.trie_given_up != 0u) return fail(c, FSEQ_E_HIP, "internal: the block trie gave up blocks it ranked in the run before");
		c->bt_given_up = (int) counts.trie_given_up;
		c->tm.phase_a_trie_given_up = counts.trie_given_up;
	}
	return FSEQ_OK;
}

int short_phase_a(fseq_ctx *c, uint32_t *d_rank, uint32_t *d_keyd, uint32_t *d_nkeys)
{
	fseq_params const &p = c->p;
	uint32_t const m = p.m;
	int rc;
	PhaseAArgs keys;
	keys.A = msa_args(c, p.n, (uint32_t) p.n, 1);
	keys.rank = d_rank; keys.keyd = d_keyd; keys.nkeys = d_nkeys; keys.nblk = 1;
	keys.T = c->bk_T; keys.cap_words = c->bk_cap_words;
	keys.wide = (c->tune.blockkeys_wide ? 1u : 0u) | (c->tune.blockkeys_single ? 2u : 0u);
	if (c->bk_cap_words && !c->tune.phase_a_classic)
	{
		if (c->use_stream)
		{
			size_t const per = (blockkeys_stream_ws_words(m, (uint32_t) p.n, c->bsh) + 15) & ~size_t(15);
			if ((rc = c->d_bkws.ensure(c, per))) return rc;
			keys.work = c->d_bkws; keys.work_per = per;
			launch_blockkeys_stream(c, 1, keys);
		}
		else
		{
			size_t const per = (blockkeys_scratch_halfwords(m, (uint32_t) p.n, c->bsh) + 7) & ~size_t(7);
			if (c->bk_per_block != per) c->d_bk.release(c);
			if ((rc = c->d_bk.ensure(c, per))) return rc;
			c->bk_per_block = per;
			keys.work = c->d_bk; keys.work_per = per;
			launch_blockkeys(c->stream, 1, c->bk_lds, keys);
		}
	}
	else
	{
		if (!c->use_stream && c->ks.cap > 7168u && p.n > 65535u)
			return fail(c, FSEQ_E_UNSUPPORTED, "short path by column sweep: more than 65535 columns with 16-bit LDS state (unset FSEQ_PHASE_A_CLASSIC)");
		launch_rank(c, keys);
	}
	return FSEQ_OK;
}

int long_phase_b(fseq_ctx *c, LongRun &R)
{
	FSEQ_LONG_LOCALS(c);
	(void) R;
	auto rank_of = [&](size_t i) { return i ? c->levels[i - 1].rank : c->d_rank; };
	auto keyd_of = [&](size_t i) { return i ? c->levels[i - 1].keyd : c->d_keyd; };
	auto nkeys_of = [&](size_t i) { return i ? c->levels[i - 1].nkeys : c->d_nkeys; };
	auto sa_of = [&](size_t i) { return i ? c->levels[i - 1].state_a : c->d_bstate_a; };
	auto sd_of = [&](size_t i) { return i ? c->levels[i - 1].state_d : c->d_bstate_d; };
	auto count_of = [&](size_t i) { return i ? c->levels[i - 1].count : c->nblocks; };
	auto chains_of = [&](size_t i, uint32_t G, uint32_t grp0) {
		ChainMultiArgs A{};
		A.rank = rank_of(i); A.keyd = keyd_of(i); A.nkeys = nkeys_of(i); A.nb_total = count_of(i); A.G = G;
		A.cols_per_block = i ? c->levels[i - 1].cols : (uint64_t) c->B; A.grp0 = grp0;
		return A;
	};
	auto compose = [&](size_t i, uint32_t G, uint32_t grp0 = 0) {
		ChainMultiArgs A = chains_of(i, G, grp0);
		A.out_rank = rank_of(i + 1); A.out_keyd = keyd_of(i + 1); A.out_nkeys = nkeys_of(i + 1);
		return A;
	};
	auto expand = [&](size_t i, uint32_t G, uint32_t grp0 = 0) {
		ChainMultiArgs A = chains_of(i, G, grp0);
		if (i < c->levels.size()) { A.start_a = sa_of(i + 1); A.start_d = sd_of(i + 1); }
		A.out_state_a = sa_of(i); A.out_state_d = sd_of(i);
		return A;
	};
	if (!sharded)
	{
		uint32_t const G = c->chain_fan;
		size_t const top = c->levels.size();
		for (size_t i = 0; i < top; ++i) launch_chain(c, count_of(i + 1), compose(i, G));
		launch_chain(c, 1, expand(top, count_of(top)));
		for (size_t i = top; i-- > 0;) launch_chain(c, count_of(i + 1), expand(i, G));
	}
	else
	{
		uint32_t const F = c->chain_fan, NH = c->n_hyper, K = c->shard_k, Q = c->shard_q;
		bool const have = sh.rank < NH;
		std::vector<uint32_t> lo(K + 1), hi(K + 1);
		lo[0] = b_lo; hi[0] = b_hi;
		for (uint32_t i = 1; i <= K; ++i) { lo[i] = lo[i - 1] / F; hi[i] = (hi[i - 1] + F - 1) / F; }
		ChainMultiArgs mine = chains_of(K, Q, sh.rank), hyper{};
		mine.out_rank = c->d_hrank; mine.out_keyd = c->d_hkeyd; mine.out_nkeys = c->d_hnkeys;
		hyper.rank = c->d_hrank; hyper.keyd = c->d_hkeyd; hyper.nkeys = c->d_hnkeys; hyper.nb_total = hyper.G = NH; hyper.cols_per_block = (uint64_t) sh.bpr * c->B;
		hyper.out_state_a = c->d_hstate_a; hyper.out_state_d = c->d_hstate_d;
		for (uint32_t i = 0; have && i < K; ++i) launch_chain(c, hi[i + 1] - lo[i + 1], compose(i, F, lo[i + 1]));
		if (have) launch_chain(c, 1, mine);
		{
			size_t const w = (size_t) NH * m;
			HIP_TRY(c, hipMemsetAsync(sh.xbuf, 0, (2 * w + NH) * 4, st));
			if (have)
			{
				HIP_TRY(c, hipMemcpyAsync(sh.xbuf + (size_t) sh.rank * m, c->d_hrank + (size_t) sh.rank * m, (size_t) m * 4, hipMemcpyDeviceToDevice, st));
				HIP_TRY(c, hipMemcpyAsync(sh.xbuf + w + (size_t) sh.rank * m, c->d_hkeyd + (size_t) sh.rank * m, (size_t) m * 4, hipMemcpyDeviceToDevice, st));
				HIP_TRY(c, hipMemcpyAsync(sh.xbuf + 2 * w + sh.rank, c->d_hnkeys + sh.rank, 4, hipMemcpyDeviceToDevice, st));
			}
			if ((rc = shard_exchange(c, 2 * w + NH, 0))) return rc;
			HIP_TRY(c, hipMemcpyAsync(c->d_hrank, sh.xbuf, w * 4, hipMemcpyDeviceToDevice, st));
			HIP_TRY(c, hipMemcpyAsync(c->d_hkeyd, sh.xbuf + w, w * 4, hipMemcpyDeviceToDevice, st));
			HIP_TRY(c, hipMemcpyAsync(c->d_hnkeys, sh.xbuf + 2 * w, (size_t) NH * 4, hipMemcpyDeviceToDevice, st));
		}
		launch_chain(c, 1, hyper);
		if (have)
		{
			ChainMultiArgs top = expand(K, Q, sh.rank);
			top.start_a = c->d_hstate_a; top.start_d = c->d_hstate_d;
			launch_chain(c, 1, top);
			for (uint32_t i = K; i-- > 0;) launch_chain(c, hi[i + 1] - lo[i + 1], expand(i, F, lo[i + 1]));
			if (b_hi < c->nblocks)
			{
				HIP_TRY(c, hipMemcpyAsync(c->d_bstate_a + (size_t) b_hi * m, c->d_hstate_a + (size_t) (sh.rank + 1u) * m, (size_t) m * 4, hipMemcpyDeviceToDevice, st));
				HIP_TRY(c, hipMemcpyAsync(c->d_bstate_d + (size_t) b_hi * m, c->d_hstate_d + (size_t) (sh.rank + 1u) * m, (size_t) m * 4, hipMemcpyDeviceToDevice, st));
			}
		}
	}
	HIP_TRY(c, hipEventRecord(c->ev.b_end, st));
	HIP_TRY(c, hipGetLastError());
	FSEQ_RANGE_POP();
	R.range_ab_open = false;
	progress(c, FSEQ_STAGE_TRACEBACK, n / 5, n);
	if (sync_at(c, 'B')) { fprintf(stderr, "[fseq] phase B queued\n"); HIP_TRY(c, hipStreamSynchronize(st)); fprintf(stderr, "[fseq] phase B done\n"); }
	return FSEQ_OK;
}

int long_list_capacity(fseq_ctx *c, LongRun &R)
{
	FSEQ_LONG_LOCALS(c);
	uint32_t &X = R.X;
	if (!p.list_cap && !c->X_hint)
	{
		std::vector<uint32_t> recent(my_blocks ? my_blocks + 1 : 0);
		if (my_blocks)
		{
			hipLaunchKernelGGL(k_boundary_recent, dim3(my_blocks + 1), dim3(256), 0, st, c->d_bstate_d, m, n, c->B, (uint32_t) L, c->d_recent, b_lo);
			HIP_TRY(c, hipMemcpyAsync(recent.data(), c->d_recent, recent.size() * 4, hipMemcpyDeviceToHost, st));
		}
		HIP_TRY(c, hipStreamSynchronize(st));
		recent.erase(std::remove(recent.begin(), recent.end(), 0xFFFFFFFFu), recent.end());
		if (!recent.empty())
		{
			std::nth_element(recent.begin(), recent.begin() + recent.size() / 2, recent.end());
			uint64_t const med = recent[recent.size() / 2];
			uint64_t const want = med + med / 4;
			if (X < want) X = (uint32_t) (((want + 63) & ~63ull) - 1);
			if (c->tune.debug)
				fprintf(stderr, "[fseq] list capacity estimate: %zu boundaries, median recent count %llu -> X = %u\n",
				        recent.size(), (unsigned long long) med, X);
		}
	}
	if (sharded)
	{
		HIP_TRY(c, hipMemcpyAsync(sh.xbuf, &X, 4, hipMemcpyHostToDevice, st));
		if ((rc = shard_exchange(c, 1, 1))) return rc;
		HIP_TRY(c, hipMemcpy(&X, sh.xbuf, 4, hipMemcpyDeviceToHost));
	}
	if (X >= m) X = m;

	return FSEQ_OK;
}

namespace {

template <int KS>
void launch_columns_stream(fseq_ctx *c, uint32_t grid, ColumnsArgs const &C)
{
	MsaArgs const &A = C.A;
	hipLaunchKernelGGL(k_columns_stream<KS>, dim3(grid), dim3(ST), stream_lds_bytes(sym_bytes(A.m, A.bsh), c->stream_staged), c->stream, A.msa, A.ld, A.m, A.n, A.B, A.npass, A.bsh, C.ws, (uint32_t) c->stream_staged,
	                   C.bstate_a, C.bstate_d, C.lists.L, C.lists.X, C.lists.stride, C.lists.ent, C.lists.hdr, C.ss.snap_stride, C.ss.ss_a, C.ss.ss_d, C.block0, C.done_host, C.epoch, C.ss.ss_pack);
}

}

void launch_columns(fseq_ctx *c, uint32_t b0, uint32_t nb, uint32_t const *list)
{
	FSEQ_LONG_LOCALS(c);
	ColumnsArgs C;
	C.A = msa_args(c, sharded ? sh.c_end : n, c->B, c->nblocks);
	C.bstate_a = c->d_bstate_a; C.bstate_d = c->d_bstate_d; C.lists = list_args(c); C.ss = stride_states(c); C.ws = c->d_ws;
	C.block0 = b0; C.blocklist = list;
	if (c->colmask_ready && c->colmask_use) C.colmask = c->d_colmask;
	if (c->use_stream && c->s2.T)
	{
		uint32_t pack_abits = 1;
		while ((1u << pack_abits) < m) ++pack_abits;
		hipLaunchKernelGGL(k_columns_stream2_prologue, dim3(nb), dim3(ST), stream_lds_bytes(0, true), st, m, C.A.n, C.A.B, C.ws, C.bstate_a, C.bstate_d, b0, pack_abits,
		                   c->ss_ids ? c->d_bs_w : (uint32_t *) nullptr, c->ss_ids ? c->d_bs_h : (uint8_t *) nullptr, list);
		c->s2.launch(st, nb, c->s2_lds, C);
	}
	else if (c->use_stream && (uint64_t) m + c->B < (1u << 19) && !c->tune.stream_plain_scan) launch_columns_stream<19>(c, nb, C);
	else if (c->use_stream) launch_columns_stream<0>(c, nb, C);
	else ks.columns(st, nb, c->lds_columns, C);
}

}

using namespace fseq;

namespace {

struct DebugBuffers {
	std::vector<void *> held;
	~DebugBuffers() { for (void *p : held) (void) hipFree(p); }
	uint32_t *words(size_t words, int fill)
	{
		void *p = nullptr;
		if (hipMalloc(&p, std::max<size_t>(1, words) * 4) != hipSuccess) return nullptr;
		held.push_back(p);
		if (hipMemset(p, fill, std::max<size_t>(1, words) * 4) != hipSuccess) return nullptr;
		return static_cast<uint32_t *>(p);
	}
	uint32_t *copy(uint32_t const *src, size_t n, size_t at = 0, size_t total = 0)
	{
		uint32_t *p = words(std::max(total, at + n), 0);
		if (p && n && hipMemcpy(p + at, src, n * 4, hipMemcpyHostToDevice) != hipSuccess) return nullptr;
		return p;
	}
};

constexpr uint32_t DEBUG_M_MIN = 11265, DEBUG_M_MAX = 589824;

bool rows_are_permutations(uint32_t const *a, size_t count, uint32_t m)
{
	std::vector<uint8_t> seen(m);
	for (size_t b = 0; b < count; ++b)
	{
		std::fill(seen.begin(), seen.end(), 0);
		for (uint32_t i = 0; i < m; ++i)
		{
			uint32_t const v = a[b * m + i];
			if (v >= m || seen[v]) return false;
			seen[v] = 1;
		}
	}
	return true;
}

}

extern "C" {

int fseq_debug_pass2_step(int device, uint32_t m, uint32_t nblocks, uint32_t const *a0, uint32_t const *d0, uint32_t const *rank, uint32_t cap,
                          uint32_t ntasks, uint32_t const *task_blk, uint32_t const *cls, uint32_t const *headd, uint32_t const *ncls,
                          uint32_t run_cap, uint32_t workgroups, uint32_t *snap_a, uint32_t *snap_d, uint32_t *stats)
{
	if (!a0 || !d0 || !rank || !task_blk || !cls || !headd || !ncls || !snap_a || !snap_d || !stats) return FSEQ_E_ARG;
	if (m < DEBUG_M_MIN || m > DEBUG_M_MAX || !nblocks || nblocks > 4096u || !ntasks || ntasks > 4096u) return FSEQ_E_ARG;
	if (!cap || cap > P2_CLS_CAP || run_cap > P2_RUN_CAP || !workgroups || workgroups > 1024u) return FSEQ_E_ARG;
	if (!rows_are_permutations(a0, nblocks, m)) return FSEQ_E_ARG;
	for (size_t i = 0; i < (size_t) nblocks * m; ++i)
		if (rank[i] >= cap) return FSEQ_E_ARG;
	std::vector<uint2> groups;
	{
		std::vector<uint8_t> block_seen(nblocks);
		for (uint32_t t = 0; t < ntasks; ++t)
		{
			if (task_blk[t] >= nblocks) return FSEQ_E_ARG;
			if (t && task_blk[t] == task_blk[t - 1]) { ++groups.back().y; continue; }
			if (block_seen[task_blk[t]]) return FSEQ_E_ARG;
			block_seen[task_blk[t]] = 1;
			groups.push_back(make_uint2(t, 1u));
		}
	}
	for (uint32_t t = 0; t < ntasks; ++t)
	{
		uint32_t const D = ncls[t];
		if (D == 0u || D == 0xFFFFFFFFu) continue;
		if (D > cap) return FSEQ_E_ARG;
		for (uint32_t j = 0; j < cap; ++j)
			if (cls[(size_t) t * cap + j] >= D) return FSEQ_E_ARG;
	}
	std::stable_sort(groups.begin(), groups.end(), [](uint2 x, uint2 y) { return x.y > y.y; });
	uint32_t const ngrp = (uint32_t) groups.size();
	std::vector<uint32_t> grp_words(2 * (size_t) ngrp + 1, 0u);
	for (uint32_t g = 0; g < ngrp; ++g) { grp_words[2 * g] = groups[g].x; grp_words[2 * g + 1] = groups[g].y; }

	if (hipSetDevice(device) != hipSuccess) return FSEQ_E_HIP;
	DebugBuffers B;
	size_t const states = (size_t) nblocks * m, outs = (size_t) ntasks * m, tables = (size_t) ntasks * cap;
	uint32_t *d_a0 = B.copy(a0, states), *d_d0 = B.copy(d0, states), *d_rank = B.copy(rank, states);
	uint32_t *d_blk = B.copy(task_blk, ntasks), *d_cls = B.copy(cls, tables), *d_headd = B.copy(headd, tables), *d_ncls = B.copy(ncls, ntasks);
	uint32_t *d_grp = B.copy(grp_words.data(), grp_words.size());
	uint32_t *d_sa = B.words(outs, 0xFF), *d_sd = B.words(outs, 0xFF), *d_stats = B.words(P2_STATS, 0);
	uint32_t *d_ws = B.words((size_t) workgroups * pass2_ws_words(m), 0);
	if (!d_a0 || !d_d0 || !d_rank || !d_blk || !d_cls || !d_headd || !d_ncls || !d_grp || !d_sa || !d_sd || !d_stats || !d_ws) return FSEQ_E_OOM;
	if (allow_lds(k_chain_snap_grouped, pass2_lds_bytes()) != hipSuccess) return FSEQ_E_HIP;
	hipLaunchKernelGGL(k_chain_snap_grouped, dim3(workgroups), dim3(ST), pass2_lds_bytes(), 0, d_a0, d_d0, d_rank, m, d_blk, d_cls, d_headd, d_ncls, cap,
	                   reinterpret_cast<uint2 const *>(d_grp), ngrp, d_grp + 2 * (size_t) ngrp, d_sa, d_sd, d_ws, run_cap, d_stats);
	if (hipGetLastError() != hipSuccess || hipDeviceSynchronize() != hipSuccess) return FSEQ_E_HIP;
	if (hipMemcpy(snap_a, d_sa, outs * 4, hipMemcpyDeviceToHost) != hipSuccess || hipMemcpy(snap_d, d_sd, outs * 4, hipMemcpyDeviceToHost) != hipSuccess
	    || hipMemcpy(stats, d_stats, P2_STATS * 4, hipMemcpyDeviceToHost) != hipSuccess)
		return FSEQ_E_HIP;
	return FSEQ_OK;
}

int fseq_debug_chain_launch(int device, uint32_t m, uint32_t nb_total, uint32_t G, uint64_t cols_per_block, uint32_t const *rank, uint32_t const *keyd,
                            uint32_t const *nkeys, uint32_t first_chain, uint32_t chains, uint32_t const *start_a, uint32_t const *start_d,
                            uint32_t *out_state_a, uint32_t *out_state_d, uint32_t *out_rank, uint32_t *out_keyd, uint32_t *out_nkeys)
{
	bool const want_states = out_state_a != nullptr, want_keys = out_rank != nullptr;
	if (!rank || !keyd || !nkeys || (!want_states && !want_keys)) return FSEQ_E_ARG;
	if (want_states != (out_state_d != nullptr) || want_keys != (out_keyd != nullptr) || want_keys != (out_nkeys != nullptr)) return FSEQ_E_ARG;
	if ((start_a != nullptr) != (start_d != nullptr)) return FSEQ_E_ARG;
	if (m < DEBUG_M_MIN || m > DEBUG_M_MAX || !nb_total || nb_total > 4096u) return FSEQ_E_ARG;
	if (!G || G > nb_total) return FSEQ_E_ARG;
	uint32_t const nchains_all = (nb_total + G - 1u) / G;
	if (!chains || first_chain >= nchains_all || chains > nchains_all - first_chain) return FSEQ_E_ARG;
	for (uint32_t b = 0; b < nb_total; ++b)
	{
		if (!nkeys[b] || nkeys[b] > m) return FSEQ_E_ARG;
		for (uint32_t i = 0; i < m; ++i)
			if (rank[(size_t) b * m + i] >= nkeys[b]) return FSEQ_E_ARG;
	}
	if (start_a && !rows_are_permutations(start_a, chains, m)) return FSEQ_E_ARG;

	if (hipSetDevice(device) != hipSuccess) return FSEQ_E_HIP;
	DebugBuffers B;
	size_t const blocks = (size_t) nb_total * m, per_chain = (size_t) (first_chain + chains) * m, at = (size_t) first_chain * m;
	ChainMultiArgs A{};
	A.m = m; A.nb_total = nb_total; A.G = G; A.cols_per_block = cols_per_block; A.grp0 = first_chain;
	A.rank = B.copy(rank, blocks); A.keyd = B.copy(keyd, blocks); A.nkeys = B.copy(nkeys, nb_total);
	A.ws = B.words((size_t) chains * chainsort_ws_words(m), 0);
	A.hist = B.words((size_t) chains * chainmulti_parts(m) * CS_BINS, 0);
	if (!A.rank || !A.keyd || !A.nkeys || !A.ws || !A.hist) return FSEQ_E_OOM;
	if (start_a)
	{
		A.start_a = B.copy(start_a, (size_t) chains * m, at); A.start_d = B.copy(start_d, (size_t) chains * m, at);
		if (!A.start_a || !A.start_d) return FSEQ_E_OOM;
	}
	if (want_states)
	{
		A.out_state_a = B.words(blocks + m, 0xFF); A.out_state_d = B.words(blocks + m, 0xFF);
		if (!A.out_state_a || !A.out_state_d) return FSEQ_E_OOM;
	}
	if (want_keys)
	{
		A.out_rank = B.words(per_chain, 0xFF); A.out_keyd = B.words(per_chain, 0xFF); A.out_nkeys = B.words(first_chain + chains, 0xFF);
		if (!A.out_rank || !A.out_keyd || !A.out_nkeys) return FSEQ_E_OOM;
		if (allow_lds(k_cm_emit, stream_lds_bytes(0, false)) != hipSuccess) return FSEQ_E_HIP;
	}
	launch_chain_stream(0, chains, A);
	if (hipGetLastError() != hipSuccess || hipDeviceSynchronize() != hipSuccess) return FSEQ_E_HIP;
	if (want_states && (hipMemcpy(out_state_a, A.out_state_a, (blocks + m) * 4, hipMemcpyDeviceToHost) != hipSuccess
	                    || hipMemcpy(out_state_d, A.out_state_d, (blocks + m) * 4, hipMemcpyDeviceToHost) != hipSuccess))
		return FSEQ_E_HIP;
	if (want_keys && (hipMemcpy(out_rank, A.out_rank + at, (size_t) chains * m * 4, hipMemcpyDeviceToHost) != hipSuccess
	                  || hipMemcpy(out_keyd, A.out_keyd + at, (size_t) chains * m * 4, hipMemcpyDeviceToHost) != hipSuccess
	                  || hipMemcpy(out_nkeys, A.out_nkeys + first_chain, (size_t) chains * 4, hipMemcpyDeviceToHost) != hipSuccess))
		return FSEQ_E_HIP;
	return FSEQ_OK;
}

}
```

### founder-sequences_amd/csrc/fseq_path_setup.hip

```cpp
#include "fseq_path.hpp"
#include "fseq_kernels.hpp"
#include "fseq_dp.hpp"
#include "fseq_stream.hpp"
#include "fseq_blockkeys.hpp"

namespace fseq {

int pin_reserve(fseq_ctx *c, size_t bytes)
{
	c->pin_used = 0;
	if (c->pin_cap >= bytes) return FSEQ_OK;
	if (c->h_pin) (void) hipHostFree(c->h_pin);
	c->h_pin = nullptr; c->pin_cap = 0;
	size_t const cap = std::max<size_t>((bytes + 4095) & ~size_t(4095), size_t(1) << 20);
	hipError_t const e = hipHostMalloc(reinterpret_cast<void **>(&c->h_pin), cap, hipHostMallocDefault);
	if (e != hipSuccess) { c->h_pin = nullptr; return fail(c, FSEQ_E_OOM, "hipHostMalloc of the staging buffer", e); }
	c->pin_cap = cap;
	return FSEQ_OK;
}

void free_msa(fseq_ctx *c)
{
	c->d_msa_own.release(c);
	c->d_msa = nullptr;
// ... 168 lines not shown
			                           (unsigned long long) rounds, (unsigned long long) b);
			if (b >= 256 && b < c->B)
			{
				c->auto_B = (uint32_t) b;
				block_geometry(c);
			}
		}
		c->bk_cap_words = 12288;
		if (c->tune.blockkeys_cap) c->bk_cap_words = (uint32_t) c->tune.blockkeys_cap;
		c->bk_lds = blockkeys_stream_lds_bytes(c->bk_cap_words, 1024);
		if (c->bk_lds <= LDS_LIMIT && (uint64_t) p.m <= (uint64_t) c->bk_cap_words * 32u)
		{
			if (int const rc = prepare_blockkeys_stream(c)) return rc;
		}
		else c->bk_cap_words = 0;
	}
	else
	{
		c->lds_columns = c->ks.columns_lds(c->B);
		if (c->lds_columns > LDS_LIMIT || c->ks.lds_chain > LDS_LIMIT || c->ks.lds_colblock > LDS_LIMIT || c->ks.lds_snap > LDS_LIMIT)
			return fail(c, FSEQ_E_UNSUPPORTED, "block state does not fit the 160 KiB LDS of one CU");
		if ((uint64_t) p.m + c->B > 65535u) return fail(c, FSEQ_E_UNSUPPORTED, "block length too large for the 16-bit value ids of phase C");
		HIP_TRY(c, c->ks.prepare());
		HIP_TRY(c, c->ks.prepare_columns(c->lds_columns));
		if (!p.block_len && !c->sh.on && !c->auto_B)
		{
			int ncu = 0;
			(void) hipDeviceGetAttribute(&ncu, hipDeviceAttributeMultiprocessorCount, p.device);
			uint64_t const slots = (uint64_t) std::max(ncu, 1) * c->ks.columns_resident(c->lds_columns);
			if (c->tune.debug) fprintf(stderr, "[fseq] phase C: %u blocks of %u columns on %llu workgroup slots (%zu bytes of LDS each)\n", c->nblocks, c->B, (unsigned long long) slots, c->lds_columns);
			if (c->nblocks > slots && c->nblocks < 3 * slots)
			{
				uint64_t const rounds = (c->nblocks + slots / 2) / slots;
				uint64_t const b = (p.n + rounds * slots - 1) / (rounds * slots);
				if (b >= 16 && b <= 4096 && b != c->B && p.m + b <= 65535u)
				{
					c->auto_B = (uint32_t) b;
					block_geometry(c);
					c->lds_columns = c->ks.columns_lds(c->B);
					if (c->lds_columns > LDS_LIMIT || (uint64_t) std::max(ncu, 1) * c->ks.columns_resident(c->lds_columns) != slots)
					{
						c->auto_B = 0;
						block_geometry(c);
						c->lds_columns = c->ks.columns_lds(c->B);
					}
					HIP_TRY(c, c->ks.prepare_columns(c->lds_columns));
				}
			}
		}
		{
			c->bk_T = blockkeys_threads(p.m);
			size_t const arrays = blockkeys_lds_bytes(p.m, 0, (int) c->bk_T, c->ld, c->bsh);
			size_t budget = 76 * 1024;
			if (arrays + 16 * 2560 > budget) budget = LDS_LIMIT - 1024;
			size_t cap = budget > arrays ? (budget - arrays) / 16 : 0;
			cap = std::min<size_t>(cap & ~size_t(63), 32768);
			if (c->tune.blockkeys_cap) cap = (size_t) c->tune.blockkeys_cap;
			c->bk_cap_words = (uint32_t) cap;
			c->bk_lds = blockkeys_lds_bytes(p.m, c->bk_cap_words, (int) c->bk_T, c->ld, c->bsh);
			if (cap >= 2048 && c->bk_lds <= LDS_LIMIT && (size_t) (8u >> (2u - c->bsh)) * c->ld <= (size_t) c->bk_T * 32) HIP_TRY(c, prepare_blockkeys(c->bk_T, c->bk_lds, c->tune.debug));
			else c->bk_cap_words = 0;
		}
	}
	if (int const rc = prepare_dp_kernels(c)) return rc;
	c->kernels_ready = true;
	return FSEQ_OK;
}

namespace {

void release_levels(fseq_ctx *c)
{
	for (auto &lv : c->levels) release_all(c, lv.rank, lv.keyd, lv.nkeys, lv.state_a, lv.state_d);
	c->levels.clear();
}

int alloc_geometry_buffers(fseq_ctx *c)
{
	fseq_params const &p = c->p;
	size_t const m = p.m;
	int rc;
	size_t const bl = c->sh.on ? c->sh.b_lo : 0, bh = c->sh.on ? std::max(c->sh.b_hi, c->sh.b_lo) : c->nblocks;
	if ((rc = c->d_rank.alloc_range(c, bl, bh, m))) return rc;
	if ((rc = c->d_keyd.alloc_range(c, bl, bh, m))) return rc;
	if ((rc = c->d_nkeys.alloc_range(c, bl, bh, 1))) return rc;
	if ((rc = c->d_bstate_a.alloc_range(c, bl, bh + 1, m))) return rc;
	if ((rc = c->d_bstate_d.alloc_range(c, bl, bh + 1, m))) return rc;
	{
		uint32_t cnt = c->nblocks;
		uint64_t cols = c->B;
		size_t lo = bl, hi = bh;
		for (uint32_t i = 0; c->sh.on ? i < c->shard_k : cnt > c->chain_fan; ++i)
		{
			fseq_ctx::ChainLevel lv;
			lv.count = (cnt + c->chain_fan - 1) / c->chain_fan;
			lv.cols = cols * c->chain_fan;
			lo = lo / c->chain_fan; hi = (hi + c->chain_fan - 1) / c->chain_fan;
			c->levels.push_back(lv);
			fseq_ctx::ChainLevel &L = c->levels.back();
			if ((rc = L.rank.alloc_range(c, lo, hi, m))) return rc;
			if ((rc = L.keyd.alloc_range(c, lo, hi, m))) return rc;
			if ((rc = L.nkeys.alloc_range(c, lo, hi, 1))) return rc;
			if ((rc = L.state_a.alloc_range(c, lo, hi + 1, m))) return rc;
			if ((rc = L.state_d.alloc_range(c, lo, hi + 1, m))) return rc;
			cnt = L.count; cols = L.cols;
		}
	}
	if (c->sh.on && c->n_hyper)
	{
		if ((rc = c->d_hrank.alloc(c, (size_t) c->n_hyper * m))) return rc;
		if ((rc = c->d_hkeyd.alloc(c, (size_t) c->n_hyper * m))) return rc;
		if ((rc = c->d_hnkeys.alloc(c, c->n_hyper))) return rc;
		if ((rc = c->d_hstate_a.alloc(c, ((size_t) c->n_hyper + 1) * m))) return rc;
		if ((rc = c->d_hstate_d.alloc(c, ((size_t) c->n_hyper + 1) * m))) return rc;
	}
	if ((rc = c->d_hdr.alloc(c, p.n))) return rc;
	if ((rc = c->d_flags.alloc(c, 1))) return rc;
	if ((rc = c->d_recent.alloc(c, c->nblocks + 1))) return rc;
	if (p.n >= 2 * p.segment_length)
	{
		c->dp_size = p.n - p.segment_length + 1;
		c->dp.tstride = (uint32_t) (c->dp_size / 64 + 2);
		if ((rc = c->dp.M.alloc(c, c->dp_size))) return rc;
		if ((rc = c->dp.LB.alloc(c, c->dp_size))) return rc;
		if ((rc = c->dp.SZ.alloc(c, c->dp_size))) return rc;
		if ((rc = c->dp.K.alloc(c, c->dp_size + 64))) return rc;
		if ((rc = c->dp.Tb.alloc(c, (size_t) 32 * c->dp.tstride))) return rc;
		if ((rc = c->dp.Tbv.alloc(c, (size_t) 32 * c->dp.tstride))) return rc;
		if ((rc = c->d_Mprev.alloc(c, c->dp_size))) return rc;
	}
	return FSEQ_OK;
}

}

int ensure_work_buffers(fseq_ctx *c, uint32_t X, bool want_ss)
{
	fseq_params const &p = c->p;
	size_t const m = p.m;
	int rc;
	if (!c->d_rank && (rc = alloc_geometry_buffers(c)))
	{
		release_levels(c);
		c->d_rank.release(c);
		return rc;
	}
	if (c->use_stream && !c->d_ws)
	{
		size_t const per_block = std::max<size_t>(columns_stream_ws_words(p.m, c->B), (size_t) 4 * m);
		size_t const bl = c->sh.on ? c->sh.b_lo : 0, bh = c->sh.on ? std::min<size_t>(c->nblocks, (size_t) std::max(c->sh.b_hi, c->sh.b_lo) + 1) : c->nblocks;
		if ((rc = c->d_ws.alloc(c, per_block * std::max<size_t>(bh - bl, 1)))) return rc;
		c->d_ws.rebase((ptrdiff_t) (bl * columns_stream_ws_words(p.m, c->B)));
		size_t const chains = std::max<size_t>(1, (bh - bl + std::max(2u, c->chain_fan) - 1) / std::max(2u, c->chain_fan) + 1);
		if ((rc = c->d_cshist.alloc(c, chains * chain_hist_words(p.m)))) { c->d_ws.release(c); return rc; }
	}
	uint64_t const k_lo = held_lo(c), k_cnt = held_hi(c) - k_lo;
	size_t const ent_count = c->lw.on ? ((size_t) c->lw.H + (size_t) c->lw.wb * c->B) * ((X + 3) & ~1u) + 256 : (size_t) k_cnt * ((X + 3) & ~1u) + 256;
	if (X && (!c->d_ent || c->X != X || c->d_ent.cap != ent_count))
	{
		c->X = X;
		c->stride = (X + 3) & ~1u;
		rc = c->d_ent.alloc(c, ent_count);
		if (rc == FSEQ_E_OOM && c->d_ss_a)
		{
			release_all(c, c->d_ss_a, c->d_ss_d);
			rc = c->d_ent.alloc(c, ent_count);
		}
		if (rc) return rc;
		c->d_ent.rebase((ptrdiff_t) ((size_t) k_lo * c->stride));
	}
	if (X && want_ss && !c->d_ss_a && p.n >= 2 * p.segment_length)
	{
		c->ss_pack = 0;
		c->ss_ids = false;
		if (c->use_stream && !c->tune.ss_unpacked)
		{
			uint32_t abits = 1, dbits = 1;
			while ((1ull << abits) < m) ++abits;
			while ((1ull << dbits) <= p.n) ++dbits;
			if (abits + dbits <= 40 && abits < 32) c->ss_pack = abits;
			if (c->s2.T && !c->tune.ss_absolute) { c->ss_pack = abits; c->ss_ids = true; }
		}
		if (c->ss_ids && !c->d_bs_w)
		{
			size_t const bl = c->sh.on ? c->sh.b_lo : 0, bh = c->sh.on ? std::min<size_t>(c->nblocks, (size_t) std::max(c->sh.b_hi, c->sh.b_lo) + 1) : c->nblocks;
			if ((rc = c->d_bs_w.alloc_range(c, bl, std::max(bh, bl + 1), m))) return rc;
			if ((rc = c->d_bs_h.alloc_range(c, bl, std::max(bh, bl + 1), ss_high_stride(p.m)))) { c->d_bs_w.release(c); return rc; }
		}
		uint64_t budget = 4ull << 30;
		{
			size_t free_b = 0, total_b = 0;
			if (hipMemGetInfo(&free_b, &total_b) == hipSuccess)
			{
				uint64_t const reserve = (k_cnt / p.segment_length + 1) * (uint64_t) m * 8ull + (2ull << 30);
				uint64_t mine = free_b;
				if (c->mem_budget) mine = std::min<uint64_t>(mine, c->mem_budget > c->alloc_total ? c->mem_budget - c->alloc_total : 0);
				uint64_t const avail = mine > reserve ? mine - reserve : 0;
				budget = std::max<uint64_t>(budget, std::min<uint64_t>(avail, 160ull << 30));
			}
		}
		uint64_t const state_bytes = c->ss_pack ? (uint64_t) m * 4ull + ss_high_stride(p.m) : (uint64_t) m * 8ull;
		uint64_t st_ = (c->npass >= 2 && !c->use_stream) ? 8 : 16;
		if ((k_cnt / st_ + 2) * state_bytes > budget) st_ = std::max<uint64_t>(st_, (k_cnt * state_bytes + budget - 1) / std::max<uint64_t>(1, budget - 2 * state_bytes));
		while ((k_cnt / st_ + 2) * state_bytes > budget) ++st_;
		c->snap_stride = (uint32_t) st_;
		if (c->tune.debug) fprintf(stderr, "[fseq] stride states every %llu columns (budget %.1f GiB, %llu bytes per state)\n", (unsigned long long) st_, budget / 1073741824.0, (unsigned long long) state_bytes);
		uint64_t const q_lo = k_lo / st_, q_hi = held_hi(c) / st_;
		size_t const hs = ss_high_stride(p.m);
		if ((rc = c->d_ss_a.alloc_range(c, q_lo, q_hi + 1, m))) return rc;
		if (c->ss_pack) { rc = c->d_ss_d.alloc(c, ((size_t) (q_hi - q_lo + 1) * hs + 3) / 4); c->d_ss_d.shift = (ptrdiff_t) ((size_t) q_lo * hs); }
		else rc = c->d_ss_d.alloc_range(c, q_lo, q_hi + 1, m);
		if (rc) { c->d_ss_a.release(c); return rc; }
	}
	return FSEQ_OK;
}

void free_work(fseq_ctx *c)
{
	release_all(c, c->d_rank, c->d_keyd, c->d_nkeys, c->d_bstate_a, c->d_bstate_d, c->d_hrank, c->d_hkeyd, c->d_hnkeys, c->d_hstate_a, c->d_hstate_d);
	release_levels(c);
	release_all(c, c->d_ent, c->d_hdr, c->d_flags, c->d_recent, c->d_chunk_r0, c->d_tau, c->d_bk, c->d_bkws, c->d_todo, c->d_colmask, c->d_btws, c->d_only, c->d_tb);
	release_all(c, c->dp.M, c->dp.LB, c->dp.SZ, c->dp.K, c->dp.Tb, c->dp.Tbv, c->d_Mprev, c->d_spec);
	release_all(c, c->d_cols, c->d_grp, c->d_src, c->d_ss_a, c->d_ss_d, c->d_bs_w, c->d_bs_h, c->d_wgblk, c->d_wggrp, c->d_snap_a, c->d_snap_d, c->d_ws, c->d_cshist);
	release_all(c, c->d_red_cnt, c->d_red_cnt_plan, c->d_red_vmin, c->d_red_rows, c->d_red_leaf, c->d_red_a, c->d_red_d, c->d_red_invalid, c->d_red_blocks, c->d_red_msa, c->d_cls, c->d_cls_have, c->d_red_src);
	release_all(c, c->d_red_ss_a, c->d_red_ss_d, c->d_red_cls, c->d_red_headd, c->d_red_ncls, c->d_red_taskblk, c->d_red_wgtasks, c->d_red_p2grp);
	c->lw.col_lo = c->lw.col_hi = 0;
	c->colmask_ready = false;
	c->ss_pack = 0; c->ss_ids = false;
	c->red.memory.forget_verdicts();
	c->red_cap = 0; c->red_ld = 0;
	c->red_active = false;
	c->cls_on = c->cls_every = c->cls_read = c->cls_staged = false; c->cls_ld = 0;
}

namespace {

int upload_rows_device_impl(fseq_ctx *c, uint8_t const *const *rows)
{
	fseq_params const &p = c->p;
	uint64_t const k_lo = held_lo(c), nloc = held_hi(c) - k_lo;
	size_t const total = (size_t) p.m * nloc;
	DevTemp<uint8_t> d_raw(c);
	DevTemp<uint32_t> d_present(c);
	int rc;
	if ((rc = d_raw.alloc(total + 16)) || (rc = d_present.alloc(8))) return rc;
	for (uint32_t r = 0; r < p.m && nloc; ++r)
	{
		hipError_t const e = hipMemcpyAsync(d_raw + (size_t) r * nloc, rows[r] + k_lo, nloc, hipMemcpyHostToDevice, c->stream);
		if (e != hipSuccess) return fail(c, FSEQ_E_HIP, "row upload", e);
	}
	(void) hipMemsetAsync(d_present, 0, 32, c->stream);
	if (total) hipLaunchKernelGGL(k_presence, dim3(1024), dim3(256), 0, c->stream, d_raw, total, d_present);
	uint32_t present[8];
	hipError_t e = hipMemcpyAsync(present, d_present, 32, hipMemcpyDeviceToHost, c->stream);
	if (e == hipSuccess) e = hipStreamSynchronize(c->stream);
	if (e != hipSuccess) return fail(c, FSEQ_E_HIP, "alphabet scan", e);
	if (c->sh.on)
	{
		uint32_t pw[256];
		for (int b = 0; b < 256; ++b) pw[b] = (present[b >> 5] >> (b & 31)) & 1u;
		e = hipMemcpy(c->sh.xbuf, pw, sizeof(pw), hipMemcpyHostToDevice);
		if (e != hipSuccess) return fail(c, FSEQ_E_HIP, "alphabet exchange", e);
		if ((rc = shard_exchange(c, 256, 1))) return rc;
		e = hipMemcpy(pw, c->sh.xbuf, sizeof(pw), hipMemcpyDeviceToHost);
		if (e != hipSuccess) return fail(c, FSEQ_E_HIP, "alphabet exchange", e);
		memset(present, 0, sizeof(present));
		for (int b = 0; b < 256; ++b) if (pw[b]) present[b >> 5] |= 1u << (b & 31);
	}
	CodeTable tab;
	memset(&tab, 0, sizeof(tab));
	uint32_t sigma = 0;
	for (int b = 0; b < 256; ++b)
		if ((present[b >> 5] >> (b & 31)) & 1u) { tab.code_of[b] = (uint8_t) sigma; c->code_to_byte[sigma] = (uint8_t) b; ++sigma; }
	c->sigma = sigma;
	if ((rc = alloc_msa(c))) return rc;
	if (nloc)
	{
		dim3 const grid((uint32_t) ((nloc + 63) / 64), (uint32_t) ((p.m + 63) / 64));
		hipLaunchKernelGGL(k_encode_transpose, grid, dim3(256), 0, c->stream, d_raw, tab, p.m, nloc, c->d_msa_own, c->ld, c->bsh);
	}
	e = hipGetLastError();
	if (e == hipSuccess) e = hipStreamSynchronize(c->stream);
	if (e != hipSuccess) return fail(c, FSEQ_E_HIP, "encode + transpose", e);
	c->have_input = true;
	return FSEQ_OK;
}

}

int upload_rows_device(fseq_ctx *c, uint8_t const *const *rows)
{
	int const rc = upload_rows_device_impl(c, rows);
	shard_post_failure(c, rc);
	return rc;
}

int set_alphabet_and_upload(fseq_ctx *c, uint8_t const *base, size_t rs, size_t cs)
{
	fseq_params const &p = c->p;
	bool present[256] = {false};
	for (uint32_t r = 0; r < p.m; ++r)
	{
		uint8_t const *row = base + (size_t) r * rs;
		for (uint64_t col = 0; col < p.n; ++col) present[row[col * cs]] = true;
	}
	uint8_t code_of[256] = {0};
	uint32_t sigma = 0;
// ... 70 lines not shown
```

### founder-sequences_amd/csrc/fseq_types.hpp

```cpp
#pragma once

#include "fseq_redplan.hpp"

#include <hip/hip_runtime.h>
#include <stddef.h>
#include <stdint.h>

namespace fseq {

struct DpArrays {
	uint32_t *M, *LB, *SZ, *Tb, *Tbv;
	unsigned long long *K;
	uint32_t tstride;
};

struct PhaseACounters {
	uint32_t tree_sliced;
	uint32_t tree_given_up;
	uint32_t trie_given_up;
};
struct PathWords {
	uint32_t dp[4];
	PhaseACounters phase_a;
	uint32_t dense_columns;
	unsigned long long dp_stamps[96];
	uint32_t dp_hist[34];
};
constexpr uint32_t DP_STAMPS_AT = (uint32_t) ((offsetof(PathWords, dp_stamps) - offsetof(PathWords, dp)) / 4);
constexpr uint32_t DP_HIST_AT = (uint32_t) ((offsetof(PathWords, dp_hist) - offsetof(PathWords, dp)) / 4);
static_assert(offsetof(PathWords, dp) + sizeof(PathWords::dp) <= offsetof(PathWords, phase_a)
              && offsetof(PathWords, phase_a) + sizeof(PhaseACounters) <= offsetof(PathWords, dense_columns)
              && offsetof(PathWords, dense_columns) + 4 <= offsetof(PathWords, dp_stamps)
              && offsetof(PathWords, dp_stamps) + sizeof(PathWords::dp_stamps) <= offsetof(PathWords, dp_hist)
              && offsetof(PathWords, dp_hist) + sizeof(PathWords::dp_hist) <= sizeof(PathWords)
              && offsetof(PathWords, dp_stamps) % 8 == 0, "the path's device words: no region overlaps another");

struct RedFlags {
	uint32_t unproven;
	uint32_t plan_stale;
};

struct AttemptWords {
	uint32_t dp[4];
	PhaseACounters phase_a;
	RedFlags red;
};


__host__ __device__ inline uint32_t sym_bytes(uint32_t m, uint32_t bsh) { return (m + (1u << bsh) - 1u) >> bsh; }

struct MsaArgs {
	uint8_t const *msa = nullptr;
	size_t ld = 0;
	uint32_t m = 0;
	uint64_t n = 0;
	uint32_t B = 0, nblocks = 0;
	uint32_t N2 = 0;
	uint32_t npass = 1, bsh = 0;
};

struct ListArgs {
	uint32_t L = 0, X = 0, stride = 0;
	uint2 *ent = nullptr;
	uint4 *hdr = nullptr;
};

struct StrideStates {
	uint32_t snap_stride = 0;
	uint32_t *ss_a = nullptr, *ss_d = nullptr;
	uint32_t ss_pack = 0;
	bool ids = false;
};

struct PhaseAArgs {
	MsaArgs A;
	uint32_t *rank = nullptr, *keyd = nullptr, *nkeys = nullptr;
	uint64_t col0 = 0;
	uint32_t nblk = 0;
	uint32_t const *only = nullptr;
	uint32_t *todo = nullptr;
	uint32_t T = 0;
	void *work = nullptr;
	size_t work_per = 0;
	uint32_t cap_words = 0;
	uint32_t wide = 0;
	uint32_t *counters = nullptr;
	uint8_t *cls = nullptr;
	size_t ldc = 0;
	uint32_t *cls_have = nullptr;
};

struct SnapArgs {
	MsaArgs A;
	uint32_t const *bstate_a = nullptr, *bstate_d = nullptr;
	uint64_t const *task_rb = nullptr;
	uint2 const *task_grp = nullptr;
	uint64_t const *task_src = nullptr;
	uint32_t *snap_a = nullptr, *snap_d = nullptr;
	StrideStates ss;
	uint32_t keyed = 0;
	uint32_t const *task_blk = nullptr;
	uint32_t *ws = nullptr;
	uint32_t const *wg_block = nullptr;
	uint2 const *wg_groups = nullptr;
	uint32_t const *bs_w = nullptr;
	uint8_t const *bs_h = nullptr;
};

struct ColumnsArgs {
	MsaArgs A;
	uint32_t const *bstate_a = nullptr, *bstate_d = nullptr;
	ListArgs lists;
	StrideStates ss;
	uint32_t *ws = nullptr;
	uint32_t block0 = 0;
	uint32_t *done_host = nullptr;
	uint32_t epoch = 0;
	uint32_t const *blocklist = nullptr;
	uint32_t const *colmask = nullptr;
};

struct ChainMultiArgs {
	uint32_t const *rank, *keyd, *nkeys;
	uint32_t m, nb_total, G;
	uint64_t cols_per_block;
	uint32_t *ws;
	uint32_t *hist;
	uint32_t const *start_a, *start_d;
	uint32_t *out_state_a, *out_state_d, *out_rank, *out_keyd, *out_nkeys;
	uint32_t grp0;
	uint32_t step;
	uint32_t pass;
	uint32_t nchains;
};

struct ReducedMsaArgs {
	uint8_t *red = nullptr;
	size_t ldr = 0;
	uint32_t const *cnt = nullptr, *rows = nullptr;
	uint32_t cap = 0;
	uint32_t const *blocks = nullptr;
	uint32_t nlisted = 0, max_rows = 0;
	uint32_t const *flag = nullptr;
	uint32_t want = 0;
	uint32_t const *pad = nullptr;
	size_t pad_per = 0;
	uint32_t const *skip = nullptr;
};

struct ClassColumnArgs {
	uint8_t const *cls = nullptr;
	size_t ldc = 0;
	uint32_t const *have = nullptr, *leaf = nullptr;
	uint32_t const *rank = nullptr;
};

constexpr uint32_t P2_HIST = 19;
constexpr uint32_t P2_STATS = 4 + P2_HIST;
constexpr uint32_t RED_WIDE = 2u;
struct RedArgs {
	uint32_t const *cnt = nullptr;
	uint32_t const *vmin = nullptr;
	uint32_t const *a = nullptr;
	uint32_t const *d = nullptr;
	uint32_t const *leaf = nullptr;
	uint32_t const *blocks = nullptr;
	uint32_t *invalid = nullptr;
	uint32_t cap = 0;
	uint32_t m_true = 0;
	uint32_t direct = 0;
	uint32_t colbytes = 0;
	uint32_t symcap = 0;
	uint32_t const *rank = nullptr;
	uint32_t *any_invalid = nullptr;
	uint32_t const *cls_have = nullptr, *cls_src = nullptr, *nkeys = nullptr;
	uint8_t const *cls_msa = nullptr;
	size_t cls_ld = 0;
	uint32_t const *wg_tasks = nullptr;
	uint32_t *ss_a = nullptr, *ss_d = nullptr;
	uint32_t ss_stride = 0, ss_cap = 0;
	unsigned long long const *task_rb = nullptr;
	uint32_t *cls = nullptr;
	uint32_t *headd = nullptr;
	uint32_t *ncls = nullptr;
};

struct RedPrepArgs {
	uint32_t const *bstate_a, *bstate_d;
	uint32_t const *rank;
	uint32_t const *blocks;
	uint32_t m, B, L, Xp, cap, block0, leaf_only, direct;
	uint32_t *invalid, *flags;
	uint64_t n;
	uint32_t *cnt, *vmin, *rows, *leaf, *a, *d;
};

}
```

### include/fseq_debug.h

```cpp
#ifndef FSEQ_DEBUG_H
#define FSEQ_DEBUG_H

#include "fseq.h"

#ifdef __cplusplus
extern "C" {
#endif

int  fseq_debug_dp_schedule(uint64_t segment_length, uint64_t n, uint64_t col_hi, uint32_t *n_rounds, uint32_t *cells_per_round,
                            uint32_t *rounds_within, int *pipelined);
int  fseq_debug_dp(fseq_ctx *ctx, uint32_t *lb, uint32_t *max_size, uint32_t *size);
int  fseq_debug_dp_owned(fseq_ctx *ctx, uint64_t *first, uint64_t *last, int *final_cell, int *whole_arrays);
int  fseq_debug_block_state(fseq_ctx *ctx, uint64_t block_idx, uint32_t *a_out, uint32_t *d_out);
int  fseq_debug_column_list(fseq_ctx *ctx, uint64_t c, uint32_t *values, uint32_t *counts,
                            uint32_t *n_entries, uint32_t *cnt0, uint32_t *complete);
int  fseq_debug_list_windows(fseq_ctx *ctx, uint64_t *bytes_held, uint64_t *columns_per_window, uint32_t *windows,
                             uint32_t *merge_windows);

int  fseq_debug_rmq(int device, uint32_t const *keys, uint32_t count, uint32_t const *beg, uint32_t const *end, uint32_t n_queries,
                    uint32_t *index_hbm, uint32_t *index_lds);

int  fseq_debug_ranges(uint64_t *pushes, uint64_t *pops, int *with_roctx);

int  fseq_debug_clock(fseq_ctx *ctx, double *ghz, uint32_t *workgroups);

int  fseq_debug_set_tuning(fseq_ctx *ctx, char const *name, char const *value);

int  fseq_debug_join_path(fseq_ctx *ctx, int *path);

int  fseq_debug_bipartite_path(fseq_ctx *ctx, int *path);

int  fseq_debug_device_bytes(fseq_ctx *ctx, uint64_t *now, uint64_t *peak, int reset_peak);

int  fseq_debug_packed_columns(fseq_ctx *ctx, uint64_t c0, uint64_t c1, uint8_t *out, uint64_t *ld, uint32_t *bits);

int  fseq_debug_pass2_paths(fseq_ctx *ctx, uint32_t *by_runs, uint32_t *by_sort, uint32_t *copies, uint32_t *max_runs, uint32_t *runs_hist);

int  fseq_debug_class_columns(fseq_ctx *ctx, uint32_t *from_classes, uint32_t *from_alignment, uint32_t block, uint32_t *have, uint32_t *nkeys,
                              uint64_t *ldc, uint8_t *out, uint64_t out_bytes);

int  fseq_debug_column_sources(fseq_ctx *ctx, uint32_t *staged, uint32_t *gathered, uint32_t block, uint32_t *block_staged);

int  fseq_debug_red_cls_direct(uint32_t m, uint32_t B, uint32_t bits, uint64_t cls_ld, uint32_t config, uint32_t resident_rows, uint32_t resident_cls,
                               uint64_t *lds_rows, uint64_t *lds_cls, int *direct);

int  fseq_debug_random_path(fseq_ctx *ctx, int *path);

int  fseq_debug_segments_file(fseq_ctx *ctx, uint64_t *batches, uint64_t *bytes, uint64_t *longest_line, uint64_t *lines);

int  fseq_debug_pass2_step(int device, uint32_t m, uint32_t nblocks, uint32_t const *a0, uint32_t const *d0, uint32_t const *rank, uint32_t cap,
                           uint32_t ntasks, uint32_t const *task_blk, uint32_t const *cls, uint32_t const *headd, uint32_t const *ncls,
                           uint32_t run_cap, uint32_t workgroups, uint32_t *snap_a, uint32_t *snap_d, uint32_t *stats);

int  fseq_debug_chain_launch(int device, uint32_t m, uint32_t nb_total, uint32_t G, uint64_t cols_per_block, uint32_t const *rank, uint32_t const *keyd,
                             uint32_t const *nkeys, uint32_t first_chain, uint32_t chains, uint32_t const *start_a, uint32_t const *start_d,
                             uint32_t *out_state_a, uint32_t *out_state_d, uint32_t *out_rank, uint32_t *out_keyd, uint32_t *out_nkeys);

#define FSEQ_DEBUG_RED_CONFIGS 64
int  fseq_debug_red_plan(uint32_t m, uint32_t B, uint32_t bits, int direct, uint32_t nblocks, uint32_t b_lo, uint32_t b_hi, uint32_t const *cnt,
                         uint8_t const *force, int reduced_always, int no_block_list, uint32_t *configs, uint32_t *n_configs, int *verdict,
                         uint8_t *full, int32_t *config_of, int32_t *config_snap_of, uint32_t *blocks, uint32_t *n_blocks, uint32_t *bins,
                         uint32_t *n_bins, uint32_t *summary);

#ifdef __cplusplus
}
#endif
#endif
```

Measured before the change: 2041 billion.

## Sort chain-compose keys by runs of equal keys instead of by rows

During the phase-B chain compose/expand, the first histogram pass now also counts run heads (positions where the rank key changes). If the total number of runs is small (at most m/8 by default), it sorts only the run heads and expands the output by binary search over run offsets, with range-max queries for d. Otherwise it falls back to the full multi-pass radix sort over rows. This is meant to cut radix sort passes when keys are highly repetitive. The cost is extra head counting, more workspace, and device-side stats atomics.

Result: no change. 2056 billion (median of 6 runs) (+0.7%).

```diff
diff --git a/founder-sequences_amd/__init__.py b/founder-sequences_amd/__init__.py
--- a/founder-sequences_amd/__init__.py
+++ b/founder-sequences_amd/__init__.py
@@ -94,11 +94,12 @@
     "fseq_debug_join_path", "fseq_debug_pass2_paths", "fseq_debug_class_columns", "fseq_debug_bipartite_path",
     "fseq_debug_pass2_step", "fseq_debug_chain_launch", "fseq_debug_red_plan", "fseq_debug_column_sources", "fseq_debug_red_cls_direct",
     "fseq_write_segments_device", "fseq_random_join_classes_host", "fseq_debug_segments_file", "fseq_debug_random_path",
+    "fseq_debug_phase_b_paths", "fseq_debug_chain_launch_form",
 ]
 DEBUG_EXPORTS = ["fseq_debug_dp", "fseq_debug_dp_owned", "fseq_debug_clock", "fseq_debug_ranges", "fseq_debug_block_state", "fseq_debug_column_list", "fseq_debug_rmq", "fseq_debug_dp_schedule", "fseq_debug_set_tuning",
                  "fseq_debug_list_windows", "fseq_debug_device_bytes", "fseq_debug_packed_columns", "fseq_debug_join_path", "fseq_debug_pass2_paths",
                  "fseq_debug_class_columns", "fseq_debug_bipartite_path", "fseq_debug_pass2_step", "fseq_debug_chain_launch", "fseq_debug_red_plan", "fseq_debug_column_sources", "fseq_debug_red_cls_direct",
-                 "fseq_debug_segments_file", "fseq_debug_random_path"]
+                 "fseq_debug_segments_file", "fseq_debug_random_path", "fseq_debug_phase_b_paths", "fseq_debug_chain_launch_form"]
 
 FSEQ_E_PEER = 6
 P2_RUN_CAP = 8832
@@ -207,6 +208,8 @@
     L.fseq_debug_red_cls_direct.argtypes = [C.c_uint32, C.c_uint32, C.c_uint32, u64, C.c_uint32, C.c_uint32, C.c_uint32, C.POINTER(u64), C.POINTER(u64), C.POINTER(C.c_int)]
     L.fseq_debug_pass2_step.argtypes = [C.c_int, C.c_uint32, C.c_uint32, vp, vp, vp, C.c_uint32, C.c_uint32, vp, vp, vp, vp, C.c_uint32, C.c_uint32, vp, vp, vp]
     L.fseq_debug_chain_launch.argtypes = [C.c_int, C.c_uint32, C.c_uint32, C.c_uint32, u64, vp, vp, vp, C.c_uint32, C.c_uint32, vp, vp, vp, vp, vp, vp, vp]
+    L.fseq_debug_chain_launch_form.argtypes = L.fseq_debug_chain_launch.argtypes + [C.c_uint32, C.c_uint32, vp, C.POINTER(C.c_double)]
+    L.fseq_debug_phase_b_paths.argtypes = [vp, vp]
     L.fseq_debug_red_plan.argtypes = [C.c_uint32, C.c_uint32, C.c_uint32, C.c_int, C.c_uint32, C.c_uint32, C.c_uint32, vp, vp, C.c_int, C.c_int] + [vp] * 11
     L.fseq_write_segments_device.argtypes = [vp, C.c_int, C.c_char_p]
     L.fseq_random_join_classes_host.argtypes = [C.c_uint32, C.c_uint32, u64, vp, vp, vp, C.c_uint32, vp]
@@ -283,7 +286,24 @@
     return snap_a, snap_d, stats
 
 
-def chain_launch(rank, keyd, nkeys, G, cols_per_block, first_chain=0, chains=None, start_a=None, start_d=None, states=True, keys=False, device=0):
+PB_STATS, PB_KIND, PB_HIST, PB_STEP_SLOTS = 108, 54, 19, 16
+PB_FORM_ROWS, PB_FORM_RULE, PB_FORM_RUNS = 0, 1, 2
+PB_RUN_DIV = 8
+
+
+def phase_b_stats(words):
+    out = {}
+    for k, name in enumerate(("compose", "expand")):
+        s = [int(x) for x in words[k * PB_KIND:(k + 1) * PB_KIND]]
+        per = s[3 + PB_HIST:]
+        steps = per[0::2]
+        out[name] = dict(by_runs=s[0], by_rows=s[1], max_runs=s[2], runs_hist=s[3:3 + PB_HIST], steps=steps,
+                         runs_per_m=[(q / 1024.0 / n) if n else 0.0 for n, q in zip(steps, per[1::2])])
+    return out
+
+
+def chain_launch(rank, keyd, nkeys, G, cols_per_block, first_chain=0, chains=None, start_a=None, start_d=None, states=True, keys=False, device=0,
+                 form=None, run_max=None):
     L = load_library()
     rank = np.ascontiguousarray(np.atleast_2d(rank), dtype=np.uint32)
     keyd = np.ascontiguousarray(np.atleast_2d(keyd), dtype=np.uint32)
@@ -309,9 +329,16 @@
         out["keyd"] = np.zeros((chains, m), dtype=np.uint32)
         out["nkeys"] = np.zeros(chains, dtype=np.uint32)
     ptr = lambda name: out[name].ctypes.data if name in out else None
-    rc = L.fseq_debug_chain_launch(device, m, nb_total, G, cols_per_block, rank.ctypes.data, keyd.ctypes.data, nkeys.ctypes.data, first_chain, chains,
-                                   None if start_a is None else start_a.ctypes.data, None if start_a is None else start_d.ctypes.data,
-                                   ptr("state_a"), ptr("state_d"), ptr("rank"), ptr("keyd"), ptr("nkeys"))
+    args = (device, m, nb_total, G, cols_per_block, rank.ctypes.data, keyd.ctypes.data, nkeys.ctypes.data, first_chain, chains,
+            None if start_a is None else start_a.ctypes.data, None if start_a is None else start_d.ctypes.data,
+            ptr("state_a"), ptr("state_d"), ptr("rank"), ptr("keyd"), ptr("nkeys"))
+    if form is None and run_max is None:
+        rc = L.fseq_debug_chain_launch(*args)
+    else:
+        stats = np.zeros(PB_STATS, dtype=np.uint32)
+        ms = C.c_double()
+        rc = L.fseq_debug_chain_launch_form(*args, PB_FORM_RULE if form is None else form, m // PB_RUN_DIV if run_max is None else run_max, stats.ctypes.data, C.byref(ms))
+        out["stats"], out["device_ms"] = phase_b_stats(stats), ms.value
     if rc != FSEQ_OK:
         raise FseqError(rc, L.fseq_strerror(rc).decode())
     return out
@@ -849,6 +876,11 @@
         out["runs_hist"] = [int(x) for x in hist]
         return out
 
+    def phase_b_paths(self):
+        words = np.zeros(PB_STATS, dtype=np.uint32)
+        self._check(self.L.fseq_debug_phase_b_paths(self.h, words.ctypes.data))
+        return phase_b_stats(words)
+
     def class_column_sources(self):
         a, b = C.c_uint32(), C.c_uint32()
         self._check(self.L.fseq_debug_class_columns(self.h, C.byref(a), C.byref(b), 0xFFFFFFFF, None, None, None, None, 0))
diff --git a/founder-sequences_amd/csrc/fseq_api_debug.hip b/founder-sequences_amd/csrc/fseq_api_debug.hip
--- a/founder-sequences_amd/csrc/fseq_api_debug.hip
+++ b/founder-sequences_amd/csrc/fseq_api_debug.hip
@@ -29,6 +29,17 @@
 	if (copies) *copies = s[2];
 	if (max_runs) *max_runs = s[3];
 	if (runs_hist) std::copy(s + 4, s + 4 + P2_HIST, runs_hist);
+	return FSEQ_OK;
+}
+
+int fseq_debug_phase_b_paths(fseq_ctx *c, uint32_t *stats)
+{
+	if (!c || !stats) return FSEQ_E_ARG;
+	if (int const rc = need_result(c)) return rc;
+	std::fill(stats, stats + PB_STATS, 0u);
+	if (!c->pb_stats_have || !c->d_cshist) return FSEQ_OK;
+	(void) hipSetDevice(c->p.device);
+	HIP_TRY(c, hipMemcpy(stats, c->d_cshist.base + c->pb_stats_off, PB_STATS * 4, hipMemcpyDeviceToHost));
 	return FSEQ_OK;
 }
 
diff --git a/founder-sequences_amd/csrc/fseq_chainsort.hpp b/founder-sequences_amd/csrc/fseq_chainsort.hpp
--- a/founder-sequences_amd/csrc/fseq_chainsort.hpp
+++ b/founder-sequences_amd/csrc/fseq_chainsort.hpp
@@ -90,8 +90,8 @@
 	db = (bits + npass - 1u) / npass;
 }
 
-template <typename PairT, typename Load0, typename KeyOf>
-__device__ __forceinline__ void pass2_sort(uint32_t cnt, uint32_t npass, uint32_t db, Load0 load0, KeyOf key_of, PairT none, PairT *bufA, PairT *bufB, Pass2Lds &S)
+template <typename PairT, typename Load0, typename KeyOf, typename Lds>
+__device__ __forceinline__ void pass2_sort(uint32_t cnt, uint32_t npass, uint32_t db, Load0 load0, KeyOf key_of, PairT none, PairT *bufA, PairT *bufB, Lds &S)
 {
 	uint32_t const tid = threadIdx.x, lane = lane_id();
 	uint32_t const wave = __builtin_amdgcn_readfirstlane(tid >> 6);
@@ -499,6 +499,8 @@
 
 constexpr uint32_t CM_PART = 1024;
 constexpr uint32_t CM_WG = 256;
+constexpr uint32_t PB_RUN_DIV = 8;
+constexpr uint32_t CM_RUN_WIN = 4 * CM_WG;
 
 
 struct CmWg { uint32_t x, chain; bool ok; };
@@ -519,6 +521,12 @@
 	uint32_t bits = 1;
 	while (bits < 32u && ((m - 1u) >> bits) != 0u) ++bits;
 	return (bits + CS_MAX_DIGIT_BITS - 1u) / CS_MAX_DIGIT_BITS;
+}
+
+__host__ __device__ inline size_t chainmulti_hist_words(uint32_t m)
+{
+	size_t const np = chainmulti_parts(m);
+	return np * CS_BINS + ((np + 2u + 3u) & ~size_t(3));
 }
 
 struct ChainMultiGeom {
@@ -532,6 +540,8 @@
 	uint2 *pairA, *pairB;
 	uint32_t *pm, *sm, *tab;
 	uint32_t *hist;
+	uint32_t *heads;
+	bool count_heads;
 };
 
 __device__ __forceinline__ ChainMultiGeom chainmulti_geom(ChainMultiArgs const &A, uint32_t chain)
@@ -557,8 +567,15 @@
 	g.pairA = reinterpret_cast<uint2 *>(g.a1);
 	g.pairB = reinterpret_cast<uint2 *>(g.w + 4u * (size_t) m);
 	g.pm = g.w + 6u * (size_t) m; g.sm = g.w + 7u * (size_t) m; g.tab = g.w + 8u * (size_t) m;
-	g.hist = A.hist + (size_t) chain * chainmulti_parts(m) * CS_BINS;
+	g.hist = A.hist + (size_t) chain * chainmulti_hist_words(m);
+	g.heads = g.hist + (size_t) chainmulti_parts(m) * CS_BINS;
+	g.count_heads = g.active && g.p4 && (A.run_form != PB_FORM_ROWS || A.stats != nullptr);
 	return g;
+}
+
+__device__ __forceinline__ bool cm_by_runs(ChainMultiArgs const &A, ChainMultiGeom const &g)
+{
+	return A.run_form != PB_FORM_ROWS && g.count_heads && g.heads[chainmulti_parts(A.m) + 1u] != 0u;
 }
 
 __device__ __forceinline__ uint2 cm_pack(uint32_t key, uint32_t pos, uint32_t row) { return make_uint2(key | (row << 20), pos | ((row >> 12) << 20)); }
@@ -588,6 +605,139 @@
 	}
 };
 
+
+struct CmSortLds {
+	uint32_t scan[ST / WAVE + 1];
+	uint32_t hist[ST / WAVE][CS_BINS];
+	uint32_t total[CS_BINS];
+};
+
+__device__ __forceinline__ void cm_run_make(ChainMultiArgs const &A, ChainMultiGeom const &g, uint32_t x)
+{
+	uint32_t const lane = lane_id(), wave = __builtin_amdgcn_readfirstlane(threadIdx.x >> 6);
+	uint32_t const part = x * (CM_WG / WAVE) + wave, m = A.m;
+	uint32_t const lo = part * CM_PART;
+	if (lo >= m) return;
+	uint32_t const hi = min(m, lo + CM_PART);
+	uint32_t const *stage = CmPair<true>::stage(g);
+	uint32_t *const head_words = CmPair<true>::stage(g) + m;
+	uint32_t k0 = g.heads[part];
+	uint32_t prev = lo ? stage[lo - 1u] >> g.pb : 0xFFFFFFFFu;
+	constexpr uint32_t U = 4;
+	for (uint32_t i0 = lo; i0 < hi; i0 += 64u * U)
+	{
+		uint32_t w[U];
+#pragma unroll
+		for (uint32_t u = 0; u < U; ++u) { uint32_t const i = i0 + u * 64u + lane; w[u] = i < hi ? stage[i] : 0u; }
+#pragma unroll
+		for (uint32_t u = 0; u < U; ++u)
+		{
+			if (i0 + u * 64u >= hi) break;
+			uint32_t const key = w[u] >> g.pb, front = dpp_mov<DPP_WAVE_SHR1, 0xF>(prev, key);
+			bool const head = i0 + u * 64u + lane < hi && key != front;
+			uint64_t const hs = __ballot(head);
+			uint32_t const k = k0 + cs_below(hs);
+			if (head && k < m) head_words[k] = w[u];
+			k0 += (uint32_t) __popcll(hs);
+			prev = readlane_u32(key, 63);
+		}
+	}
+}
+
+__device__ __forceinline__ void cm_run_sort(ChainMultiArgs const &A, ChainMultiGeom const &g, CmSortLds &S)
+{
+	uint32_t const tid = threadIdx.x, m = A.m;
+	uint32_t const R = min(g.heads[chainmulti_parts(m)], m);
+	if (!R) return;
+	uint32_t const pmask = (1u << g.pb) - 1u, pb = g.pb;
+	uint32_t const *head_words = CmPair<true>::stage(g) + m;
+	uint2 *const bufA = g.pairA, *const bufB = g.pairB;
+	pass2_sort<uint2>(R, g.npass, g.db, [&](uint32_t i) -> uint2 { return make_uint2(head_words[i], i + 1u < R ? head_words[i + 1u] & pmask : m); },
+	                  [&](uint2 x) -> uint32_t { return x.x >> pb; }, make_uint2(0u, 0u), bufA, bufB, S);
+	uint32_t const q = (R + ST - 1u) / ST, j0 = min(R, tid * q), j1 = min(R, j0 + q);
+	uint32_t sum = 0;
+	for (uint32_t j = j0; j < j1; ++j) { uint2 const x = bufB[j]; sum += x.y - (x.x & pmask); }
+	uint32_t all;
+	uint32_t at = block_excl_add<ST>(sum, S.scan, &all);
+	uint32_t const nwin = (m + CM_RUN_WIN - 1u) / CM_RUN_WIN;
+	for (uint32_t j = j0; j < j1; ++j)
+	{
+		uint2 const x = bufB[j];
+		uint32_t const len = x.y - (x.x & pmask);
+		bufB[j].y = at;
+		if (len <= m && at < m)
+			for (uint32_t w = (at + CM_RUN_WIN - 1u) / CM_RUN_WIN; w < nwin && w * CM_RUN_WIN < at + len; ++w) g.hist[w] = j;
+		at += len;
+	}
+}
+
+__device__ __forceinline__ void cm_run_output(ChainMultiArgs const &A, ChainMultiGeom const &g, CmWg const &wg)
+{
+	__shared__ uint32_t s_x[CM_RUN_WIN + 1], s_off[CM_RUN_WIN + 1];
+	constexpr uint32_t U = CM_RUN_WIN / CM_WG;
+	uint32_t const m = A.m, tid = threadIdx.x, w0 = wg.x * CM_RUN_WIN;
+	if (w0 >= m) return;
+	uint32_t const R = min(g.heads[chainmulti_parts(m)], m);
+	if (!R) return;
+	uint32_t const nblk = (m + 63u) / 64u, pmask = (1u << g.pb) - 1u;
+	uint32_t const *kd = A.keyd + (size_t) g.b * m;
+	uint2 const *dsc = g.pairB;
+	uint32_t const jf = min(g.hist[wg.x], R - 1u);
+	uint32_t const jn = w0 + CM_RUN_WIN < m ? min(g.hist[wg.x + 1u], R - 1u) : R - 1u;
+	uint32_t const cnt = jn >= jf ? min(jn - jf + 1u, CM_RUN_WIN + 1u) : 1u;
+	for (uint32_t t = tid; t < cnt; t += CM_WG) { uint2 const x = dsc[jf + t]; s_x[t] = x.x; s_off[t] = x.y; }
+	__syncthreads();
+	uint32_t tt[U], hi[U], row[U], dv[U];
+#pragma unroll
+	for (uint32_t u = 0; u < U; ++u)
+	{
+		uint32_t const p = min(w0 + u * CM_WG + tid, m - 1u);
+		uint32_t t = 0;
+#pragma unroll
+		for (uint32_t step = CM_RUN_WIN; step; step >>= 1) { uint32_t const t1 = t + step; if (t1 < cnt && s_off[t1] <= p) t = t1; }
+		tt[u] = t;
+		hi[u] = min((s_x[t] & pmask) + (p - s_off[t]), m - 1u);
+	}
+#pragma unroll
+	for (uint32_t u = 0; u < U; ++u) { row[u] = g.a0[hi[u]]; dv[u] = g.d0[hi[u]]; }
+	uint32_t const grp = wg.chain + A.grp0;
+	uint32_t const b1 = min(A.nb_total, grp * A.G + A.G);
+	bool const state = A.out_state_a && (g.b + 1u < b1 || g.b + 1u == A.nb_total);
+#pragma unroll
+	for (uint32_t u = 0; u < U; ++u)
+	{
+		uint32_t const p = w0 + u * CM_WG + tid;
+		if (p >= m) break;
+		uint32_t const t = tt[u], j = jf + t, me = s_x[t], off = s_off[t];
+		if (off == p)
+		{
+			uint2 pv = make_uint2(0u, 0u);
+			if (t) pv = make_uint2(s_x[t - 1u], s_off[t - 1u]); else if (j) pv = dsc[j - 1u];
+			if (j == 0u || (pv.x >> g.pb) != (me >> g.pb)) dv[u] = kd[min(me >> g.pb, m - 1u)];
+			else
+			{
+				uint32_t const h = hi[u], lo = min((pv.x & pmask) + (off - pv.y), h);
+				uint32_t const bl = lo >> 6, bh = h >> 6;
+				if (bl == bh)
+				{
+					for (uint32_t i = lo; i < h; ++i) dv[u] = max(dv[u], g.d0[i]);
+				}
+				else
+				{
+					dv[u] = max(g.sm[lo], g.pm[h]);
+					if (bh > bl + 1u)
+					{
+						uint32_t const k = 31u - (uint32_t) __builtin_clz(bh - bl - 1u);
+						uint32_t const *tb = g.tab + (size_t) k * nblk;
+						dv[u] = max(dv[u], max(tb[bl + 1u], tb[bh - (1u << k)]));
+					}
+				}
+			}
+		}
+		g.a1[p] = row[u]; g.d1[p] = dv[u];
+		if (state) { A.out_state_a[(size_t) (g.b + 1u) * m + p] = row[u]; A.out_state_d[(size_t) (g.b + 1u) * m + p] = dv[u]; }
+	}
+}
 
 __global__ __launch_bounds__(CM_WG) void k_cm_init(ChainMultiArgs const A)
 {
@@ -613,6 +763,7 @@
 	if (!wg.ok) return;
 	ChainMultiGeom const g = chainmulti_geom(A, wg.chain);
 	if (!g.active || A.pass >= g.npass) return;
+	if (A.pass != 0u && cm_by_runs(A, g)) return;
 	uint32_t const lane = lane_id(), wave = __builtin_amdgcn_readfirstlane(threadIdx.x >> 6);
 	uint32_t const part = wg.x * (CM_WG / WAVE) + wave, m = A.m;
 	uint32_t const lo = part * CM_PART;
@@ -621,6 +772,9 @@
 	uint32_t const *rk = A.rank + (size_t) g.b * m;
 	uint32_t const shift = A.pass * g.db;
 	for (uint32_t b = lane; b < g.nbins; b += 64u) hist[wave][b] = 0;
+	bool const heads = A.pass == 0u && g.count_heads;
+	uint32_t nheads = 0, prev = 0xFFFFFFFFu;
+	if (heads && lo > 0u) prev = rk[g.a0[lo - 1u]];
 	auto sweep = [&](auto p4_) {
 		using P = CmPair<decltype(p4_)::value>;
 		constexpr uint32_t U = 4;
@@ -638,9 +792,21 @@
 #pragma unroll
 			for (uint32_t u = 0; u < U; ++u)
 				if (i0 + u * 64u + lane < hi) atomicAdd(&hist[wave][(P::key(g, pr[u]) >> shift) & (g.nbins - 1u)], 1u);
+			if (heads)
+			{
+#pragma unroll
+				for (uint32_t u = 0; u < U; ++u)
+				{
+					if (i0 + u * 64u >= hi) break;
+					uint32_t const key = P::key(g, pr[u]), front = dpp_mov<DPP_WAVE_SHR1, 0xF>(prev, key);
+					nheads += (uint32_t) __popcll(__ballot(i0 + u * 64u + lane < hi && key != front));
+					prev = readlane_u32(key, 63);
+				}
+			}
 		}
 	};
 	if (g.p4) sweep(std::true_type{}); else sweep(std::false_type{});
+	if (heads && lane == 0u) g.heads[part] = nheads;
 	if (A.pass == 0u)
 	{
 		uint32_t const nblk = (m + 63u) / 64u;
@@ -662,15 +828,46 @@
 
 __global__ __launch_bounds__(ST) void k_cm_offsets(ChainMultiArgs const A)
 {
-	__shared__ uint32_t scan[ST / WAVE + 1];
-	__shared__ uint32_t start_of[CS_BINS];
+	__shared__ CmSortLds S;
+	uint32_t *const scan = S.scan;
 	ChainMultiGeom const g = chainmulti_geom(A, blockIdx.x);
-	if (!g.active || A.pass >= g.npass) return;
+	if (!g.active) return;
+	if (A.pass != 0u && cm_by_runs(A, g)) { if (A.pass == 1u) cm_run_sort(A, g, S); return; }
+	if (A.pass >= g.npass) return;
 	uint32_t const tid = threadIdx.x, m = A.m;
 	uint32_t const nparts = chainmulti_parts(m);
+	bool by_runs = false;
+	if (A.pass == 0u && g.count_heads)
+	{
+		uint32_t R = 0;
+		for (uint32_t p0 = 0; p0 < nparts; p0 += ST)
+		{
+			uint32_t const p = p0 + tid;
+			uint32_t const h = p < nparts ? min(g.heads[p], min(m, (p + 1u) * CM_PART) - p * CM_PART) : 0u;
+			uint32_t all;
+			uint32_t const before = block_excl_add<ST>(h, scan, &all);
+			if (p < nparts) g.heads[p] = R + before;
+			R += all;
+		}
+		by_runs = A.run_form == PB_FORM_RUNS || (A.run_form == PB_FORM_RULE && R <= A.run_max);
+		if (tid == 0u)
+		{
+			g.heads[nparts] = R; g.heads[nparts + 1u] = by_runs ? 1u : 0u;
+			if (A.stats)
+			{
+				uint32_t *const s = A.stats + (A.out_rank ? 0u : PB_KIND);
+				atomicAdd(s + (by_runs ? 0 : 1), 1u);
+				if (by_runs) atomicMax(s + 2, R);
+				atomicAdd(s + 3 + min(PB_HIST - 1u, R > 1u ? 32u - (uint32_t) __builtin_clz(R - 1u) : 0u), 1u);
+				uint32_t *const t = s + 3 + PB_HIST + 2u * min(A.step, PB_STEP_SLOTS - 1u);
+				atomicAdd(t, 1u);
+				atomicAdd(t + 1, (uint32_t) (((uint64_t) R << 10) / m));
+			}
+		}
+	}
 	constexpr uint32_t PB = 16;
 	uint32_t tot = 0;
-	if (tid < g.nbins)
+	if (tid < g.nbins && !by_runs)
 		for (uint32_t p0 = 0; p0 < nparts; p0 += PB)
 		{
 			uint32_t c[PB];
@@ -681,8 +878,7 @@
 		}
 	uint32_t all;
 	uint32_t const start = block_excl_add<ST>(tid < g.nbins ? tot : 0u, scan, &all);
-	(void) start_of;
-	if (tid < g.nbins)
+	if (tid < g.nbins && !by_runs)
 	{
 		uint32_t run = start;
 		for (uint32_t p0 = 0; p0 < nparts; p0 += PB)
@@ -717,7 +913,9 @@
 	CmWg const wg = cm_wg(A);
 	if (!wg.ok) return;
 	ChainMultiGeom const g = chainmulti_geom(A, wg.chain);
-	if (!g.active || A.pass >= g.npass) return;
+	if (!g.active) return;
+	if (cm_by_runs(A, g)) { if (A.pass == 0u) cm_run_make(A, g, wg.x); return; }
+	if (A.pass >= g.npass) return;
 	uint32_t const lane = lane_id(), wave = __builtin_amdgcn_readfirstlane(threadIdx.x >> 6);
 	uint32_t const part = wg.x * (CM_WG / WAVE) + wave, m = A.m;
 	uint32_t const lo = part * CM_PART;
@@ -762,6 +960,7 @@
 	if (!wg.ok) return;
 	ChainMultiGeom const g = chainmulti_geom(A, wg.chain);
 	if (!g.active) return;
+	if (cm_by_runs(A, g)) { cm_run_output(A, g, wg); return; }
 	uint32_t const m = A.m, p = wg.x * CM_WG + threadIdx.x;
 	if (p >= m) return;
 	uint32_t const nblk = (m + 63u) / 64u;
diff --git a/founder-sequences_amd/csrc/fseq_ctx.hpp b/founder-sequences_amd/csrc/fseq_ctx.hpp
--- a/founder-sequences_amd/csrc/fseq_ctx.hpp
+++ b/founder-sequences_amd/csrc/fseq_ctx.hpp
@@ -120,6 +120,7 @@
 	int  reduced_cap = 0;
 	bool class_gather = false;
 	int  class_columns = 1;
+	int  pb_runs = -1;
 	int  p2_run_cap = -1;
 
 	struct Knob {
@@ -167,6 +168,7 @@
 			{"FSEQ_REDUCED_MSA_GATHER", &Tuning::reduced_msa_gather, nullptr, 0, 0, nullptr},
 			{"FSEQ_REDUCED_CAP", nullptr, &Tuning::reduced_cap, 1, 0, nullptr},
 			{"FSEQ_P2_RUN_CAP", nullptr, &Tuning::p2_run_cap, 0, -1, nullptr},
+			{"FSEQ_PB_RUNS", nullptr, &Tuning::pb_runs, 0, -1, nullptr},
 			{"FSEQ_CLASS_COLUMNS", nullptr, &Tuning::class_columns, 0, 1, nullptr},
 			{"FSEQ_CLASS_GATHER", &Tuning::class_gather, nullptr, 0, 0, nullptr},
 		};
@@ -321,6 +323,8 @@
 	DevBuf<uint32_t> d_rank, d_keyd, d_nkeys;
 	DevBuf<uint32_t> d_bstate_a, d_bstate_d;
 	DevBuf<uint32_t> d_cshist;
+	size_t pb_stats_off = 0;
+	bool pb_stats_have = false;
 	DevBuf<uint32_t> d_hrank, d_hkeyd, d_hnkeys, d_hstate_a, d_hstate_d;
 	struct ChainLevel { uint32_t count = 0; uint64_t cols = 0; DevBuf<uint32_t> rank, keyd, nkeys, state_a, state_d; };
 	std::vector<ChainLevel> levels;
diff --git a/founder-sequences_amd/csrc/fseq_path_pass1.hip b/founder-sequences_amd/csrc/fseq_path_pass1.hip
--- a/founder-sequences_amd/csrc/fseq_path_pass1.hip
+++ b/founder-sequences_amd/csrc/fseq_path_pass1.hip
@@ -62,6 +62,7 @@
 	uint32_t const m = A.m, nparts = chainmulti_parts(m), npass = chainmulti_passes(m);
 	A.step = 0; A.pass = 0;
 	A.nchains = grid;
+	if (npass < 2u) A.run_form = PB_FORM_ROWS;
 	uint32_t const grid_y = (grid + 7u) & ~7u;
 	dim3 const by_row((m + CM_WG - 1u) / CM_WG, grid_y), by_part((nparts + CM_WG / WAVE - 1u) / (CM_WG / WAVE), grid_y);
 	hipLaunchKernelGGL(k_cm_init, by_row, dim3(CM_WG), 0, st, A);
@@ -117,7 +118,7 @@
 	HIP_TRY(c, allow_lds(k_blockkeys_stream, c->bk_lds));
 	return FSEQ_OK;
 }
-size_t chain_hist_words(uint32_t m) { return (size_t) chainmulti_parts(m) * CS_BINS; }
+size_t chain_hist_words(uint32_t m) { return chainmulti_hist_words(m); }
 
 uint32_t pass2_run_cap(fseq_ctx const *c)
 {
@@ -362,8 +363,16 @@
 		ChainMultiArgs A{};
 		A.rank = rank_of(i); A.keyd = keyd_of(i); A.nkeys = nkeys_of(i); A.nb_total = count_of(i); A.G = G;
 		A.cols_per_block = i ? c->levels[i - 1].cols : (uint64_t) c->B; A.grp0 = grp0;
+		if (i == 0 && c->use_stream)
+		{
+			A.stats = c->d_cshist.base + c->pb_stats_off;
+			A.run_form = c->tune.pb_runs < 0 ? PB_FORM_RULE : c->tune.pb_runs ? PB_FORM_RUNS : PB_FORM_ROWS;
+			A.run_max = m / PB_RUN_DIV;
+		}
 		return A;
 	};
+	c->pb_stats_have = c->use_stream;
+	if (c->use_stream) HIP_TRY(c, hipMemsetAsync(c->d_cshist.base + c->pb_stats_off, 0, PB_STATS * 4, st));
 	auto compose = [&](size_t i, uint32_t G, uint32_t grp0 = 0) {
 		ChainMultiArgs A = chains_of(i, G, grp0);
 		A.out_rank = rank_of(i + 1); A.out_keyd = keyd_of(i + 1); A.out_nkeys = nkeys_of(i + 1);
@@ -607,6 +616,16 @@
                             uint32_t const *nkeys, uint32_t first_chain, uint32_t chains, uint32_t const *start_a, uint32_t const *start_d,
                             uint32_t *out_state_a, uint32_t *out_state_d, uint32_t *out_rank, uint32_t *out_keyd, uint32_t *out_nkeys)
 {
+	return fseq_debug_chain_launch_form(device, m, nb_total, G, cols_per_block, rank, keyd, nkeys, first_chain, chains, start_a, start_d, out_state_a, out_state_d,
+	                                    out_rank, out_keyd, out_nkeys, PB_FORM_RULE, m / PB_RUN_DIV, nullptr, nullptr);
+}
+
+int fseq_debug_chain_launch_form(int device, uint32_t m, uint32_t nb_total, uint32_t G, uint64_t cols_per_block, uint32_t const *rank, uint32_t const *keyd,
+                                 uint32_t const *nkeys, uint32_t first_chain, uint32_t chains, uint32_t const *start_a, uint32_t const *start_d,
+                                 uint32_t *out_state_a, uint32_t *out_state_d, uint32_t *out_rank, uint32_t *out_keyd, uint32_t *out_nkeys,
+                                 uint32_t form, uint32_t run_max, uint32_t *stats, double *device_ms)
+{
+	if (form > PB_FORM_RUNS || run_max > m) return FSEQ_E_ARG;
 	bool const want_states = out_state_a != nullptr, want_keys = out_rank != nullptr;
 	if (!rank || !keyd || !nkeys || (!want_states && !want_keys)) return FSEQ_E_ARG;
 	if (want_states != (out_state_d != nullptr) || want_keys != (out_keyd != nullptr) || want_keys != (out_nkeys != nullptr)) return FSEQ_E_ARG;
@@ -630,8 +649,9 @@
 	A.m = m; A.nb_total = nb_total; A.G = G; A.cols_per_block = cols_per_block; A.grp0 = first_chain;
 	A.rank = B.copy(rank, blocks); A.keyd = B.copy(keyd, blocks); A.nkeys = B.copy(nkeys, nb_total);
 	A.ws = B.words((size_t) chains * chainsort_ws_words(m), 0);
-	A.hist = B.words((size_t) chains * chainmulti_parts(m) * CS_BINS, 0);
-	if (!A.rank || !A.keyd || !A.nkeys || !A.ws || !A.hist) return FSEQ_E_OOM;
+	A.hist = B.words((size_t) chains * chainmulti_hist_words(m), 0);
+	A.run_form = form; A.run_max = run_max; A.stats = B.words(PB_STATS, 0);
+	if (!A.rank || !A.keyd || !A.nkeys || !A.ws || !A.hist || !A.stats) return FSEQ_E_OOM;
 	if (start_a)
 	{
 		A.start_a = B.copy(start_a, (size_t) chains * m, at); A.start_d = B.copy(start_d, (size_t) chains * m, at);
@@ -648,8 +668,20 @@
 		if (!A.out_rank || !A.out_keyd || !A.out_nkeys) return FSEQ_E_OOM;
 		if (allow_lds(k_cm_emit, stream_lds_bytes(0, false)) != hipSuccess) return FSEQ_E_HIP;
 	}
+	hipEvent_t ev[2] = {nullptr, nullptr};
+	if (device_ms && (hipEventCreate(&ev[0]) != hipSuccess || hipEventCreate(&ev[1]) != hipSuccess || hipEventRecord(ev[0], 0) != hipSuccess)) return FSEQ_E_HIP;
 	launch_chain_stream(0, chains, A);
-	if (hipGetLastError() != hipSuccess || hipDeviceSynchronize() != hipSuccess) return FSEQ_E_HIP;
+	bool ok = !device_ms || hipEventRecord(ev[1], 0) == hipSuccess;
+	ok = hipGetLastError() == hipSuccess && hipDeviceSynchronize() == hipSuccess && ok;
+	if (device_ms)
+	{
+		float ms = 0.f;
+		ok = ok && hipEventElapsedTime(&ms, ev[0], ev[1]) == hipSuccess;
+		*device_ms = ms;
+		(void) hipEventDestroy(ev[0]); (void) hipEventDestroy(ev[1]);
+	}
+	if (!ok) return FSEQ_E_HIP;
+	if (stats && hipMemcpy(stats, A.stats, PB_STATS * 4, hipMemcpyDeviceToHost) != hipSuccess) return FSEQ_E_HIP;
 	if (want_states && (hipMemcpy(out_state_a, A.out_state_a, (blocks + m) * 4, hipMemcpyDeviceToHost) != hipSuccess
 	                    || hipMemcpy(out_state_d, A.out_state_d, (blocks + m) * 4, hipMemcpyDeviceToHost) != hipSuccess))
 		return FSEQ_E_HIP;
diff --git a/founder-sequences_amd/csrc/fseq_path_setup.hip b/founder-sequences_amd/csrc/fseq_path_setup.hip
--- a/founder-sequences_amd/csrc/fseq_path_setup.hip
+++ b/founder-sequences_amd/csrc/fseq_path_setup.hip
@@ -344,7 +344,8 @@
 		if ((rc = c->d_ws.alloc(c, per_block * std::max<size_t>(bh - bl, 1)))) return rc;
 		c->d_ws.rebase((ptrdiff_t) (bl * columns_stream_ws_words(p.m, c->B)));
 		size_t const chains = std::max<size_t>(1, (bh - bl + std::max(2u, c->chain_fan) - 1) / std::max(2u, c->chain_fan) + 1);
-		if ((rc = c->d_cshist.alloc(c, chains * chain_hist_words(p.m)))) { c->d_ws.release(c); return rc; }
+		c->pb_stats_off = chains * chain_hist_words(p.m);
+		if ((rc = c->d_cshist.alloc(c, c->pb_stats_off + PB_STATS))) { c->d_ws.release(c); return rc; }
 	}
 	uint64_t const k_lo = held_lo(c), k_cnt = held_hi(c) - k_lo;
 	size_t const ent_count = c->lw.on ? ((size_t) c->lw.H + (size_t) c->lw.wb * c->B) * ((X + 3) & ~1u) + 256 : (size_t) k_cnt * ((X + 3) & ~1u) + 256;
diff --git a/founder-sequences_amd/csrc/fseq_types.hpp b/founder-sequences_amd/csrc/fseq_types.hpp
--- a/founder-sequences_amd/csrc/fseq_types.hpp
+++ b/founder-sequences_amd/csrc/fseq_types.hpp
@@ -132,7 +132,15 @@
 	uint32_t step;
 	uint32_t pass;
 	uint32_t nchains;
-};
+	uint32_t run_form;
+	uint32_t run_max;
+	uint32_t *stats;
+};
+
+constexpr uint32_t PB_FORM_ROWS = 0, PB_FORM_RULE = 1, PB_FORM_RUNS = 2;
+constexpr uint32_t PB_HIST = 19, PB_STEP_SLOTS = 16;
+constexpr uint32_t PB_KIND = 3 + PB_HIST + 2 * PB_STEP_SLOTS;
+constexpr uint32_t PB_STATS = 2 * PB_KIND;
 
 struct ReducedMsaArgs {
 	uint8_t *red = nullptr;
diff --git a/include/fseq_debug.h b/include/fseq_debug.h
--- a/include/fseq_debug.h
+++ b/include/fseq_debug.h
@@ -36,6 +36,9 @@
 
 int  fseq_debug_pass2_paths(fseq_ctx *ctx, uint32_t *by_runs, uint32_t *by_sort, uint32_t *copies, uint32_t *max_runs, uint32_t *runs_hist);
 
+#define FSEQ_DEBUG_PB_STATS 108
+int  fseq_debug_phase_b_paths(fseq_ctx *ctx, uint32_t *stats);
+
 int  fseq_debug_class_columns(fseq_ctx *ctx, uint32_t *from_classes, uint32_t *from_alignment, uint32_t block, uint32_t *have, uint32_t *nkeys,
                               uint64_t *ldc, uint8_t *out, uint64_t out_bytes);
 
@@ -56,6 +59,11 @@
                              uint32_t const *nkeys, uint32_t first_chain, uint32_t chains, uint32_t const *start_a, uint32_t const *start_d,
                              uint32_t *out_state_a, uint32_t *out_state_d, uint32_t *out_rank, uint32_t *out_keyd, uint32_t *out_nkeys);
 
+int  fseq_debug_chain_launch_form(int device, uint32_t m, uint32_t nb_total, uint32_t G, uint64_t cols_per_block, uint32_t const *rank, uint32_t const *keyd,
+                                  uint32_t const *nkeys, uint32_t first_chain, uint32_t chains, uint32_t const *start_a, uint32_t const *start_d,
+                                  uint32_t *out_state_a, uint32_t *out_state_d, uint32_t *out_rank, uint32_t *out_keyd, uint32_t *out_nkeys,
+                                  uint32_t form, uint32_t run_max, uint32_t *stats, double *device_ms);
+
 #define FSEQ_DEBUG_RED_CONFIGS 64
 int  fseq_debug_red_plan(uint32_t m, uint32_t B, uint32_t bits, int direct, uint32_t nblocks, uint32_t b_lo, uint32_t b_hi, uint32_t const *cnt,
                          uint8_t const *force, int reduced_always, int no_block_list, uint32_t *configs, uint32_t *n_configs, int *verdict,
```
